# sumitsk/algp

Hardware: AMD Instinct MI355X
Metric: GP-fit+MI-score throughput (N train x M candidates) (higher is better)
Workload: dtype f64

## Files before the change

### algp_amd/csrc/api.hip

```cpp
#include "api_impl.h"

using namespace algp;

namespace algp {

int fail(algp_ctx* c, int code, const std::string& msg) {
    if (c) c->err = msg;
    return code;
}

int ensure(algp_ctx* c, DevBuf& b, size_t bytes) {
    if (bytes <= b.cap && b.p) return ALGP_OK;
    if (bytes == 0) bytes = 256;
    if (b.p) {
        hipStreamSynchronize(c->stream);
        hipFree(b.p);
        c->dev_bytes -= (int64_t)b.cap;
        b.p = nullptr;
        b.cap = 0;
    }
    const size_t want = (bytes + 255) / 256 * 256;
    hipError_t e = hipMalloc(&b.p, want);
    if (e != hipSuccess) {
        b.p = nullptr;
        (void)hipGetLastError();
        return fail(c, ALGP_ERR_OOM, std::string("hipMalloc(") + std::to_string(want) + "): " + hipGetErrorString(e));
    }
    b.cap = want;
    c->dev_bytes += (int64_t)want;
    return ALGP_OK;
}

void release(algp_ctx* c, DevBuf& b) {
    if (b.p) {
        hipFree(b.p);
        c->dev_bytes -= (int64_t)b.cap;
    }
    b.p = nullptr;
    b.cap = 0;
}

static hipEvent_t get_event(algp_ctx* c) {
    if (!c->event_pool.empty()) {
        hipEvent_t e = c->event_pool.back();
        c->event_pool.pop_back();
        return e;
    }
    hipEvent_t e;
    hipEventCreate(&e);
    return e;
}

static thread_local int prof_depth = 0;
void prof_begin(algp_ctx* c, int klass, double flops, double bytes) {
    if (!c->prof_on) return;
    if (prof_depth++ > 0) return;
    PendingEvent pe;
    pe.a = get_event(c);
    pe.b = get_event(c);
    pe.klass = klass;
    c->prof[klass].flops += flops;
    c->prof[klass].bytes += bytes;
    c->prof[klass].launches += 1;
    hipEventRecord(pe.a, c->cur);
    c->pending.push_back(pe);
}
void prof_end(algp_ctx* c) {
    if (!c->prof_on) return;
    if (--prof_depth > 0) return;
    hipEventRecord(c->pending.back().b, c->cur);
}
bool prof_launch_events(algp_ctx* c, int klass, double flops, double bytes, hipEvent_t* a, hipEvent_t* b) {
    if (!c->prof_on || prof_depth > 0) return false;
    PendingEvent pe;
    pe.a = get_event(c);
    pe.b = get_event(c);
    pe.klass = klass;
    c->prof[klass].flops += flops;
    c->prof[klass].bytes += bytes;
    c->prof[klass].launches += 1;
    c->pending.push_back(pe);
    *a = pe.a;
    *b = pe.b;
    return true;
}
static thread_local int span_index = -1;
void prof_span_begin(algp_ctx* c, int klass, double flops, double bytes) {
    if (!c->prof_on) return;
    PendingEvent pe;
    pe.a = get_event(c);
    pe.b = get_event(c);
    pe.klass = klass;
    c->prof[klass].flops += flops;
    c->prof[klass].bytes += bytes;
    c->prof[klass].launches += 1;
    hipEventRecord(pe.a, c->stream);
    span_index = (int)c->pending.size();
    c->pending.push_back(pe);
}
void prof_span_end_on(algp_ctx* c, hipStream_t st) {
    if (!c->prof_on || span_index < 0) return;
    hipEventRecord(c->pending[span_index].b, st);
    span_index = -1;
}
void prof_span_end(algp_ctx* c) { prof_span_end_on(c, c->stream); }
static thread_local int span2_index = -1;
void prof_span_begin2(algp_ctx* c, int klass, double flops, double bytes) {
    if (!c->prof_on) return;
    PendingEvent pe;
    pe.a = get_event(c);
    pe.b = get_event(c);
    pe.klass = klass;
    c->prof[klass].flops += flops;
    c->prof[klass].bytes += bytes;
    c->prof[klass].launches += 1;
    hipEventRecord(pe.a, c->cur);
    span2_index = (int)c->pending.size();
    c->pending.push_back(pe);
}
void prof_span_end2(algp_ctx* c) {
    if (!c->prof_on || span2_index < 0) return;
    hipEventRecord(c->pending[span2_index].b, c->stream);
    span2_index = -1;
}
void prof_collect(algp_ctx* c) {
    for (auto& pe : c->pending) {
        hipEventSynchronize(pe.b);
        float ms = 0;
        hipEventElapsedTime(&ms, pe.a, pe.b);
        c->prof[pe.klass].ms += ms;
        c->event_pool.push_back(pe.a);
        c->event_pool.push_back(pe.b);
    }
    c->pending.clear();
}


hipEvent_t sync_event_api(algp_ctx* c, size_t i) {
    while (c->sync_events.size() <= i) {
        hipEvent_t e;
        hipEventCreateWithFlags(&e, hipEventDisableTiming);
        c->sync_events.push_back(e);
    }
    return c->sync_events[i];
}


KmatSrc make_src(algp_ctx* c) {
    KmatSrc s;
    s.Xs = c->Xs.p;
    s.Cp = c->pool_is_cov ? c->Cp.p : nullptr;
    s.n_pool = c->n_pool;
    s.DP = c->hyp.DP;
    s.kernel = c->hyp.kernel;
    s.outputscale = c->hyp.outputscale;
    s.noise = c->hyp.noise;
    return s;
}

int sync(algp_ctx* c) {
    ALGP_HIP(hipStreamSynchronize(c->stream));
    c->n_syncs++;
    return ALGP_OK;
}

int sync_checked(algp_ctx* c, const char* what) {
    int stall = 0;
    int* d = (int*)((double*)c->scal.p + SC_STALL);
    ALGP_HIP(hipMemcpyAsync(&stall, d, sizeof(int), hipMemcpyDeviceToHost, c->stream));
    ALGP_HIP(hipStreamSynchronize(c->stream));
    c->n_syncs++;
    if (stall != 0) {
        hipMemsetAsync(d, 0, sizeof(double), c->stream);
        return fail(c, ALGP_ERR_HIP, std::string(what) + ": a one-launch kernel stalled (a hand-off between its workgroups never "
                                     "arrived within the spin limit); the result is incomplete");
    }
    return ALGP_OK;
}

}


namespace algp {


template <typename T>
int Impl<T>::rescale_pool(algp_ctx* c) {
    if (c->pool_is_cov || c->n_pool == 0 || !c->hyp.set) return ALGP_OK;
    ALGP_TRY(ensure(c, c->Xs, sizeof(T) * c->n_pool * c->hyp.DP));
    return scale_coords_launch<T>(c, (const T*)c->Xraw.p, c->n_pool, p(c->Xs));
}


template <typename T>
int Impl<T>::kernel_matrix(algp_ctx* c, const void* x1, int64_t n1, const void* x2, int64_t n2, const void* diag_add,
                             int add_lik, void* out) {
    const int D = c->hyp.D, DP = c->hyp.DP;
    const bool sym = (x2 == nullptr);
    if (sym) n2 = n1;
    if (n1 == 0 || n2 == 0) return ALGP_OK;
    const int64_t ldo = round_up(n2, 4);
    DevBuf raw1, raw2, s1, s2, dv, o;
    int rc = ALGP_OK;
    auto cleanup = [&]() { release(c, raw1); release(c, raw2); release(c, s1); release(c, s2); release(c, dv); release(c, o); };
#define KM_TRY(x) do { rc = (x); if (rc != ALGP_OK) { cleanup(); return rc; } } while (0)
#define KM_HIP(x) do { hipError_t e_ = (x); if (e_ != hipSuccess) { cleanup(); return fail(c, ALGP_ERR_HIP, hipGetErrorString(e_)); } } while (0)
    KM_TRY(ensure(c, raw1, sizeof(T) * n1 * D));
    KM_TRY(ensure(c, s1, sizeof(T) * n1 * DP));
    KM_HIP(hipMemcpyAsync(raw1.p, x1, sizeof(T) * n1 * D, hipMemcpyHostToDevice, c->stream));
    KM_TRY(scale_coords_launch<T>(c, (const T*)raw1.p, n1, (T*)s1.p));
    if (!sym) {
        KM_TRY(ensure(c, raw2, sizeof(T) * n2 * D));
        KM_TRY(ensure(c, s2, sizeof(T) * n2 * DP));
        KM_HIP(hipMemcpyAsync(raw2.p, x2, sizeof(T) * n2 * D, hipMemcpyHostToDevice, c->stream));
        KM_TRY(scale_coords_launch<T>(c, (const T*)raw2.p, n2, (T*)s2.p));
    }
    if (sym && diag_add) {
        KM_TRY(ensure(c, dv, sizeof(T) * n1));
        KM_HIP(hipMemcpyAsync(dv.p, diag_add, sizeof(T) * n1, hipMemcpyHostToDevice, c->stream));
    }
    KM_TRY(ensure(c, o, sizeof(T) * n1 * ldo));
    KM_TRY(kmat_xy_launch<T>(c, (const T*)s1.p, n1, sym ? nullptr : (const T*)s2.p, n2, sym ? 1 : 0,
                             (sym && diag_add) ? (const T*)dv.p : nullptr, (sym && add_lik) ? c->hyp.noise : 0.0,
                             (T*)o.p, ldo));
    KM_HIP(hipMemcpy2DAsync(out, sizeof(T) * n2, o.p, sizeof(T) * ldo, sizeof(T) * n2, n1, hipMemcpyDeviceToHost,
                            c->stream));
    KM_HIP(hipStreamSynchronize(c->stream));
    cleanup();
#undef KM_TRY
#undef KM_HIP
    return ALGP_OK;
}


template <typename T>
int Impl<T>::set_pool(algp_ctx* c, const void* x, int64_t n) {
    const int D = c->hyp.D;
    ALGP_TRY(ensure(c, c->Xraw, sizeof(T) * n * D));
    ALGP_HIP(hipMemcpyAsync(c->Xraw.p, x, sizeof(T) * n * D, hipMemcpyHostToDevice, c->stream));
    c->n_pool = n;
    c->pool_is_cov = false;
    c->site_hash.assign((size_t)n, 0);
    const unsigned char* bytes = (const unsigned char*)x;
    const size_t stride = sizeof(T) * (size_t)D;
    for (int64_t i = 0; i < n; ++i) {
        uint64_t h = 1469598103934665603ull;
        for (size_t b = 0; b < stride; ++b) h = (h ^ bytes[(size_t)i * stride + b]) * 1099511628211ull;
        c->site_hash[(size_t)i] = h;
    }
    ALGP_TRY(rescale_pool(c));
    return sync(c);
}

template <typename T>
uint64_t Impl<T>::train_sites_hash(const algp_ctx* c, const std::vector<int64_t>& idx) {
    if (c->pool_is_cov || c->site_hash.empty()) return 0;
    uint64_t h = 1469598103934665603ull;
    for (int64_t i : idx) h = (h ^ c->site_hash[(size_t)i]) * 1099511628211ull;
    return h;
}


template <typename T>
int Impl<T>::set_pool_cov(algp_ctx* c, const void* cov, int64_t n) {
    ALGP_TRY(ensure(c, c->Cp, sizeof(T) * n * n));
    ALGP_HIP(hipMemcpyAsync(c->Cp.p, cov, sizeof(T) * n * n, hipMemcpyHostToDevice, c->stream));
    c->n_pool = n;
    c->pool_is_cov = true;
    c->site_hash.clear();
    return sync(c);
}


template <typename T>
int Impl<T>::set_train(algp_ctx* c, const int64_t* idx, int64_t N, const void* y, const void* var) {
    const int64_t Npad = round_up(std::max<int64_t>(N, 1), NB);
    c->N = N;
    c->Npad = Npad;
    c->train_idx.assign(idx, idx + N);
    c->pos_in_train.assign(c->n_pool, -1);
    c->train_has_repeats = false;
    for (int64_t i = 0; i < N; ++i) {
        if (c->pos_in_train[idx[i]] < 0) c->pos_in_train[idx[i]] = i;
        else c->train_has_repeats = true;
    }
    double ybar = 0;
    const T* yt = (const T*)y;
    for (int64_t i = 0; i < N; ++i) ybar += (double)yt[i];
    ybar = N > 0 ? ybar / (double)N : 0.0;
    if (c->mean_override) ybar = c->mean_value;
    c->ybar = ybar;
    std::vector<T> y0(Npad, (T)0), vv(Npad, (T)0);
    for (int64_t i = 0; i < N; ++i) y0[i] = (T)((double)yt[i] - ybar);
    if (var)
        for (int64_t i = 0; i < N; ++i) vv[i] = ((const T*)var)[i];
    ALGP_TRY(ensure(c, c->Aidx, sizeof(int64_t) * Npad));
    ALGP_TRY(ensure(c, c->y0, sizeof(T) * Npad));
    ALGP_TRY(ensure(c, c->varA, sizeof(T) * Npad));
    if (N > 0) ALGP_HIP(hipMemcpyAsync(c->Aidx.p, idx, sizeof(int64_t) * N, hipMemcpyHostToDevice, c->stream));
    ALGP_HIP(hipMemcpyAsync(c->y0.p, y0.data(), sizeof(T) * Npad, hipMemcpyHostToDevice, c->stream));
    std::vector<T> yr(Npad, (T)0);
    for (int64_t i = 0; i < N; ++i) yr[i] = yt[i];
    ALGP_TRY(ensure(c, c->yraw, sizeof(T) * Npad));
    ALGP_HIP(hipMemcpyAsync(c->yraw.p, yr.data(), sizeof(T) * Npad, hipMemcpyHostToDevice, c->stream));
    c->train_y_host.assign(N, 0.0);
    for (int64_t i = 0; i < N; ++i) c->train_y_host[i] = (double)yt[i];
    ALGP_HIP(hipMemcpyAsync(c->varA.p, vv.data(), sizeof(T) * Npad, hipMemcpyHostToDevice, c->stream));
    ALGP_TRY(sync(c));
    c->train_var_host.assign(N, 0.0);
    if (var)
        for (int64_t i = 0; i < N; ++i) c->train_var_host[i] = (double)((const T*)var)[i];
    c->train_dirty = true;
    c->solved = false;
    if (c->comm || c->host_gather) ALGP_TRY(comm_reserve(c));
    return ALGP_OK;
}


template <typename T>
int Impl<T>::build_set_matrix(algp_ctx* c, const int64_t* idx, int64_t m, const void* var, int64_t* mpad_out, T* dst) {
    const int64_t mpad = round_up(std::max<int64_t>(m, 1), NB);
    *mpad_out = mpad;
    if (!dst) ALGP_TRY(ensure(c, c->auxA, sizeof(T) * mpad * mpad));
    ALGP_TRY(ensure(c, c->auxInv, sizeof(T) * mpad * NB));
    ALGP_TRY(ensure(c, c->auxIdx, sizeof(int64_t) * mpad));
    ALGP_TRY(ensure(c, c->auxVar, sizeof(T) * mpad));
    if (m > 0) ALGP_HIP(hipMemcpyAsync(c->auxIdx.p, idx, sizeof(int64_t) * m, hipMemcpyHostToDevice, c->stream));
    if (var && m > 0)
        ALGP_HIP(hipMemcpyAsync(c->auxVar.p, var, sizeof(T) * m, hipMemcpyHostToDevice, c->stream));
    KmatSrc s = make_src(c);
// ... 35 lines not shown
    double ld = 0;
    ALGP_TRY(factor_resident(c, p(c->auxA), m, mpad, p(c->auxInv), SC_AUXLOGDET, SC_AUXINFO, &ld));
    if (H) *H = (double)m * ENT_CONST + 0.5 * ld;
    return inverse_diag_resident(c, m, mpad, diag_out);
}


template <typename T>
int Impl<T>::upload_padded(algp_ctx* c, DevBuf& b, const void* A, int64_t rows, int64_t cols, int64_t rpad,
                             int64_t cpad) {
    ALGP_TRY(ensure(c, b, sizeof(T) * rpad * cpad));
    ALGP_HIP(hipMemsetAsync(b.p, 0, sizeof(T) * rpad * cpad, c->stream));
    if (rows > 0 && cols > 0)
        ALGP_HIP(hipMemcpy2DAsync(b.p, sizeof(T) * cpad, A, sizeof(T) * cols, sizeof(T) * cols, rows,
                                  hipMemcpyHostToDevice, c->stream));
    return ALGP_OK;
}


template <typename T>
int Impl<T>::entropy_from_cov(algp_ctx* c, const void* cov, int64_t k, double* H, void* L_out, double* logdet) {
    if (k == 0) { if (H) *H = 0.0; if (logdet) *logdet = 0.0; return ALGP_OK; }
    const int64_t kpad = round_up(k, NB);
    ALGP_TRY(upload_padded(c, c->auxA, cov, k, k, kpad, kpad));
    ALGP_TRY(pad_identity_launch<T>(c, p(c->auxA), k, kpad, kpad));
    ALGP_TRY(ensure(c, c->auxInv, sizeof(T) * kpad * NB));
    double ld = 0;
    ALGP_TRY(factor_resident(c, p(c->auxA), k, kpad, p(c->auxInv), SC_AUXLOGDET, SC_AUXINFO, &ld));
    if (H) *H = (double)k * ENT_CONST + 0.5 * ld;
    if (logdet) *logdet = ld;
    if (L_out) {
        ALGP_HIP(hipMemcpy2DAsync(L_out, sizeof(T) * k, c->auxA.p, sizeof(T) * kpad, sizeof(T) * k, k,
                                  hipMemcpyDeviceToHost, c->stream));
        ALGP_TRY(sync(c));
        T* Lh = (T*)L_out;
        for (int64_t i = 0; i < k; ++i)
            for (int64_t j = i + 1; j < k; ++j) Lh[i * k + j] = (T)0;
    }
    return ALGP_OK;
}


template <typename T>
int Impl<T>::gemm_host(algp_ctx* c, int64_t m, int64_t n, int64_t k, double alpha, const void* A, const void* B,
                         double beta, const void* C, void* D) {
    const int64_t mp = round_up(std::max<int64_t>(m, 1), NB), np = round_up(std::max<int64_t>(n, 1), NB),
                  kp = round_up(std::max<int64_t>(k, 1), NB);
    DevBuf a, b, cc;
    int rc = upload_padded(c, a, A, m, k, mp, kp);
    if (rc == ALGP_OK) rc = upload_padded(c, b, B, n, k, np, kp);
    if (rc == ALGP_OK) rc = upload_padded(c, cc, (beta != 0.0 && C) ? C : nullptr, (beta != 0.0 && C) ? m : 0, n, mp, np);
    if (rc == ALGP_OK)
        rc = gemm_nt_launch<T>(c, ALGP_PROF_GEMM_OTHER, mp, np, kp, (T)alpha, (const T*)a.p, kp, (const T*)b.p, kp,
                               (T)beta, (const T*)cc.p, np, (T*)cc.p, np, 0);
    if (rc == ALGP_OK) {
        hipError_t e = hipMemcpy2DAsync(D, sizeof(T) * n, cc.p, sizeof(T) * np, sizeof(T) * n, m,
                                        hipMemcpyDeviceToHost, c->stream);
        if (e != hipSuccess) rc = fail(c, ALGP_ERR_HIP, hipGetErrorString(e));
    }
    hipStreamSynchronize(c->stream);
    release(c, a); release(c, b); release(c, cc);
    return rc;
}


template <typename T>
int Impl<T>::trsm_host(algp_ctx* c, const void* L, int64_t n, const void* B, int64_t m, void* X) {
    const int64_t np = round_up(std::max<int64_t>(n, 1), NB), mp = round_up(std::max<int64_t>(m, 1), NB);
    DevBuf l, b, inv;
    int rc = upload_padded(c, l, L, n, n, np, np);
    if (rc == ALGP_OK) rc = pad_identity_launch<T>(c, (T*)l.p, n, np, np);
    if (rc == ALGP_OK) rc = upload_padded(c, b, B, m, n, mp, np);
    if (rc == ALGP_OK) rc = ensure(c, inv, sizeof(T) * np * NB);
    for (int64_t kb = 0; rc == ALGP_OK && kb < np / NB; ++kb)
        rc = trinv_diag_launch<T>(c, (const T*)l.p + kb * NB * np + kb * NB, np, (T*)inv.p + kb * NB * NB);
    if (rc == ALGP_OK) rc = trsm_blocked<T>(c, ALGP_PROF_GEMM_OTHER, (T*)b.p, mp, np, (const T*)l.p, np, np, (const T*)inv.p);
    if (rc == ALGP_OK) {
        hipError_t e = hipMemcpy2DAsync(X, sizeof(T) * n, b.p, sizeof(T) * np, sizeof(T) * n, m,
                                        hipMemcpyDeviceToHost, c->stream);
        if (e != hipSuccess) rc = fail(c, ALGP_ERR_HIP, hipGetErrorString(e));
    }
    hipStreamSynchronize(c->stream);
    release(c, l); release(c, b); release(c, inv);
    return rc;
}

template <typename T>
int Impl<T>::selftest(algp_ctx* c, int* mism) {
    double* sc = (double*)c->scal.p;
    int* d = (int*)(sc + SC_PROBE);
    ALGP_HIP(hipMemsetAsync(d, 0, sizeof(double), c->stream));
    ALGP_TRY(test_mfma_launch<double>(c, d));
    ALGP_TRY(test_mfma_launch<float>(c, d));
    ALGP_HIP(hipMemcpyAsync(mism, d, sizeof(int), hipMemcpyDeviceToHost, c->stream));
    return sync(c);
}

template struct Impl<float>;
template struct Impl<double>;

}

extern "C" {

int algp_version(void) { return 100; }

int algp_device_count(void) {
    int n = 0;
    if (hipGetDeviceCount(&n) != hipSuccess) { (void)hipGetLastError(); return 0; }
    return n;
}

int algp_create(int device_id, int dtype, algp_ctx** out) {
    if (!out || (dtype != ALGP_F32 && dtype != ALGP_F64)) return ALGP_ERR_BAD_ARG;
    *out = nullptr;
    setenv("GPU_MAX_HW_QUEUES", "8", 0);
    int n = 0;
    if (hipGetDeviceCount(&n) != hipSuccess || n <= 0) { (void)hipGetLastError(); return ALGP_ERR_NO_DEVICE; }
    if (device_id < 0 || device_id >= n) return ALGP_ERR_BAD_ARG;
    if (hipSetDevice(device_id) != hipSuccess) return ALGP_ERR_HIP;
    algp_ctx* c = new algp_ctx();
    c->device = device_id;
    c->dtype = dtype;
    c->es = dtype == ALGP_F64 ? 8 : 4;
    if (hipStreamCreateWithFlags(&c->stream, hipStreamNonBlocking) != hipSuccess) { delete c; return ALGP_ERR_HIP; }
    if (hipStreamCreateWithFlags(&c->stream2, hipStreamNonBlocking) != hipSuccess) { hipStreamDestroy(c->stream); delete c; return ALGP_ERR_HIP; }
    if (hipStreamCreateWithFlags(&c->stream3, hipStreamNonBlocking) != hipSuccess) c->stream3 = nullptr;
    if (hipStreamCreateWithFlags(&c->stream4, hipStreamNonBlocking) != hipSuccess) c->stream4 = nullptr;
    c->trsm_chunks = env_int("ALGP_TRSM_CHUNKS", c->trsm_chunks);
    c->trsm_chunks_explicit = env_int("ALGP_TRSM_CHUNKS", 0) != 0;
    if (hipDeviceGetAttribute(&c->cu_count, hipDeviceAttributeMultiprocessorCount, device_id) != hipSuccess) { (void)hipGetLastError(); c->cu_count = 0; }
    c->cur = c->stream;
    if (ensure(c, c->scal, sizeof(double) * SC_COUNT) != ALGP_OK) { hipStreamDestroy(c->stream); delete c; return ALGP_ERR_OOM; }
    hipMemsetAsync(c->scal.p, 0, sizeof(double) * SC_COUNT, c->stream);
    hipStreamSynchronize(c->stream);
    *out = c;
    return ALGP_OK;
}

void algp_destroy(algp_ctx* c) {
    if (!c) return;
    hipSetDevice(c->device);
    hipStreamSynchronize(c->stream);
    prof_collect(c);
    DevBuf* bufs[] = {&c->Xs, &c->Xraw, &c->Cp, &c->Aidx, &c->yA, &c->varA, &c->y0, &c->L, &c->invD, &c->z, &c->alpha,
                      &c->scal, &c->Cidx, &c->ckind, &c->cextra, &c->Vt, &c->dstat, &c->mu, &c->alive, &c->scores,
                      &c->lrow, &c->remote, &c->commbuf, &c->tvec, &c->amax, &c->prevrows, &c->fresh, &c->lazypicks, &c->yraw, &c->uvec, &c->wvec, &c->acc3, &c->rowstat, &c->inv512, &c->inv512_scr, &c->trsm_tmp, &c->gemm_part, &c->rhs_rx, &c->rhs_cx, &c->rhs_rk, &c->splitk, &c->dag_state, &c->dag_stats, &c->trsv_ctrl, &c->auxA, &c->auxInv, &c->auxW, &c->auxIdx,
                      &c->auxVar, &c->auxD, &c->hostStage, &c->rowx, &c->tailE, &c->tailPart, &c->ldpart, &c->tw, &c->smp, &c->grp};
    for (DevBuf* b : bufs) release(c, *b);
    release(c, c->mi);
    release(c, c->vr);
    dag_release(c);
    comm_destroy(c);
    for (hipEvent_t e : c->event_pool) hipEventDestroy(e);
    for (hipEvent_t e : c->sync_events) hipEventDestroy(e);
    hipStreamSynchronize(c->stream2);
    hipStreamDestroy(c->stream2);
    if (c->stream3) { hipStreamSynchronize(c->stream3); hipStreamDestroy(c->stream3); }
    if (c->stream4) { hipStreamSynchronize(c->stream4); hipStreamDestroy(c->stream4); }
    hipStreamDestroy(c->stream);
    delete c;
}

const char* algp_last_error(const algp_ctx* c) { return c ? c->err.c_str() : "null context"; }

int64_t algp_last_pivot(const algp_ctx* c) { return c ? c->pivot : 0; }

double algp_last_jitter(const algp_ctx* c) { return c ? c->last_jitter : 0.0; }

int algp_dtype(const algp_ctx* c) { return c ? c->dtype : -1; }

int algp_set_hypers(algp_ctx* c, int kernel, int D, const double* log_ls, double log_os, double log_noise) {
    CHECK_CTX(c);
    if (D < 1 || D > MAXD || !log_ls) return fail(c, ALGP_ERR_BAD_ARG, "set_hypers: 1 <= D <= 8 required");
    if (kernel < ALGP_KERNEL_RBF || kernel > ALGP_KERNEL_MATERN25) return fail(c, ALGP_ERR_BAD_ARG, "set_hypers: unknown kernel");
    if (c->hyp.set && c->hyp.D != D && c->n_pool > 0 && !c->pool_is_cov) {
        c->n_pool = 0;
        c->N = 0;
        c->pos_in_train.clear();
    }
    c->hyp.kernel = kernel;
    c->hyp.D = D;
    c->hyp.DP = D <= 2 ? 2 : (D <= 4 ? 4 : 8);
    for (int d = 0; d < MAXD; ++d) c->hyp.inv_ls[d] = d < D ? exp(-log_ls[d]) : 0.0;
    c->hyp.outputscale = exp(log_os);
    c->hyp.noise = exp(log_noise);
    c->hyp.set = true;
    c->hyp_stamp++;
    c->factored = false;
    c->solved = false;
    FINISH(c, DISPATCH(c, rescale_pool(c)));
}

int algp_kernel_matrix(algp_ctx* c, const void* x1, int64_t n1, const void* x2, int64_t n2, const void* diag_add,
                       int add_lik, void* out) {
    CHECK_CTX(c);
    NEED_HYPERS(c);
    if (!x1 || n1 < 0 || n2 < 0 || !out) return fail(c, ALGP_ERR_BAD_ARG, "kernel_matrix: bad arguments");
    FINISH(c, DISPATCH(c, kernel_matrix(c, x1, n1, x2, n2, diag_add, add_lik, out)));
}

int algp_set_pool(algp_ctx* c, const void* x, int64_t n) {
    CHECK_CTX(c);
    NEED_HYPERS(c);
    if (!x || n <= 0) return fail(c, ALGP_ERR_BAD_ARG, "set_pool: bad arguments");
    c->factored = c->solved = false;
    c->hyp_stamp++;
    c->pos_in_train.clear();
    c->N = 0;
    c->site_owner.clear();
    c->site_owner_hash = 0;
    c->has_tw = false;
    c->vr.drop();
    FINISH(c, DISPATCH(c, set_pool(c, x, n)));
}

int algp_set_pool_cov(algp_ctx* c, const void* cov, int64_t n) {
    CHECK_CTX(c);
    NEED_HYPERS(c);
    if (!cov || n <= 0) return fail(c, ALGP_ERR_BAD_ARG, "set_pool_cov: bad arguments");
    c->factored = c->solved = false;
    c->hyp_stamp++;
    c->pos_in_train.clear();
    c->N = 0;
    c->site_owner.clear();
    c->site_owner_hash = 0;
    c->has_tw = false;
    c->vr.drop();
    FINISH(c, DISPATCH(c, set_pool_cov(c, cov, n)));
}

int algp_set_train(algp_ctx* c, const int64_t* idx, int64_t N, const void* y, const void* var) {
    CHECK_CTX(c);
    if (c->n_pool <= 0) return fail(c, ALGP_ERR_STATE, "set_train: set a pool first");
    if (N < 0 || (N > 0 && (!idx || !y))) return fail(c, ALGP_ERR_BAD_ARG, "set_train: bad arguments");
    for (int64_t i = 0; i < N; ++i)
        if (idx[i] < 0 || idx[i] >= c->n_pool) return fail(c, ALGP_ERR_BAD_ARG, "set_train: index outside the pool");
    FINISH(c, DISPATCH(c, set_train(c, idx, N, y, var)));
}

int algp_set_constant_mean(algp_ctx* c, int enable, double value) {
    CHECK_CTX(c);
    if (enable && !(value == value)) return fail(c, ALGP_ERR_BAD_ARG, "set_constant_mean: NaN");
    c->mean_override = enable != 0;
    c->mean_value = value;
    return ALGP_OK;
}

#if ALGP_TEST_HOOKS
int64_t algp_debug_counter(algp_ctx* c, int which) {
    if (!c) return -1;
    switch (which) {
        case 0: return c->n_syncs;
        case 1: return c->factor_rows_from_vt;
        case 2: return c->rows_from_peers;
        case 3: return c->row_exchanges;
        case 4: return c->row_fallbacks;
        default: return -1;
    }
}
#endif

#if ALGP_TEST_HOOKS
int algp_debug_set_trsm_chunks(algp_ctx* c, int chunks) {
    CHECK_CTX(c);
    if (chunks < 0 || chunks > 4) return fail(c, ALGP_ERR_BAD_ARG, "debug_set_trsm_chunks: 0 (default) .. 4");
    hipStreamSynchronize(c->stream);
    c->trsm_chunks_explicit = chunks != 0 || env_int("ALGP_TRSM_CHUNKS", 0) != 0;
    if (chunks == 0) chunks = env_int("ALGP_TRSM_CHUNKS", 3);
    c->trsm_chunks = chunks;
    return ALGP_OK;
}
#endif

#if ALGP_TEST_HOOKS
int algp_debug_trsv_stall(algp_ctx* c, int block) {
    CHECK_CTX(c);
    if (block < -1) return fail(c, ALGP_ERR_BAD_ARG, "debug_trsv_stall: a block >= 0, or -1 to disarm");
    c->debug_trsv_stall_block = block;
    return ALGP_OK;
}
#endif

#if ALGP_TEST_HOOKS
int algp_debug_dag_stall(algp_ctx* c, int ticket) {
    CHECK_CTX(c);
    if (ticket < -1) return fail(c, ALGP_ERR_BAD_ARG, "debug_dag_stall: a ticket >= 0, or -1 to disarm");
    c->debug_dag_stall_ticket = ticket;
    return ALGP_OK;
}
#endif

int algp_entropy_from_cov(algp_ctx* c, const void* cov, int64_t k, double* H) {
    CHECK_CTX(c);
    if (k < 0 || !H || (k > 0 && !cov)) return fail(c, ALGP_ERR_BAD_ARG, "entropy_from_cov: bad arguments");
    FINISH(c, DISPATCH(c, entropy_from_cov(c, cov, k, H, nullptr, nullptr)));
}

int algp_set_entropy(algp_ctx* c, const int64_t* idx, int64_t m, const void* var, double* H) {
    CHECK_CTX(c);
    NEED_HYPERS(c);
    if (m < 0 || !H || (m > 0 && !idx)) return fail(c, ALGP_ERR_BAD_ARG, "set_entropy: bad arguments");
    for (int64_t i = 0; i < m; ++i)
        if (idx[i] < 0 || idx[i] >= c->n_pool) return fail(c, ALGP_ERR_BAD_ARG, "set_entropy: index outside the pool");
    FINISH(c, DISPATCH(c, set_entropy(c, idx, m, var, H)));
}
// ... 108 lines not shown
```

### algp_amd/csrc/api_candidates.hip

```cpp
#include "api_impl.h"

using namespace algp;

namespace algp {


template <typename T>
int Impl<T>::set_candidates(algp_ctx* c, const int64_t* idx, int64_t M, int prior_noise, const void* extra) {
    if (c->pool_is_cov && !prior_noise)
        return fail(c, ALGP_ERR_BAD_ARG, "an explicit pool covariance carries sigma_n^2 on its diagonal: prior_includes_noise must be 1");
    const int64_t Mpad = round_up(std::max<int64_t>(M, 1), NB);
    c->M = M;
    c->Mpad = Mpad;
    c->prior_noise = prior_noise;
    c->cand_idx.assign(idx, idx + M);
    c->cand_pos.assign(c->n_pool, -1);
    for (int64_t j = 0; j < M; ++j) c->cand_pos[idx[j]] = j;
    ALGP_TRY(ensure(c, c->Cidx, sizeof(int64_t) * Mpad));
    if (M > 0) ALGP_HIP(hipMemcpyAsync(c->Cidx.p, idx, sizeof(int64_t) * M, hipMemcpyHostToDevice, c->stream));
    if (extra) {
        ALGP_TRY(ensure(c, c->cextra, sizeof(T) * Mpad));
        ALGP_HIP(hipMemcpyAsync(c->cextra.p, extra, sizeof(T) * M, hipMemcpyHostToDevice, c->stream));
    } else {
        release(c, c->cextra);
    }
    ALGP_TRY(sync(c));
    c->solved = false;
    return ALGP_OK;
}

template <typename T>
void Impl<T>::plan_route(algp_ctx* c, int incremental, bool allow_fold, typename Impl<T>::SolvePlan& pl) {
    const bool tail_on = env_switch("ALGP_TAIL_COLS", true), solve_dag_on = env_switch("ALGP_SOLVE_DAG", true),
               stats_on = env_switch("ALGP_ROW_STATS", true), fold_on = allow_fold && env_switch("ALGP_FOLD", true);
    const int64_t N = c->N, Npad = c->Npad, M = c->M, Mpad = c->Mpad;
    pl.carried_sums = incremental && c->uw_rows == N && c->uvec.p && c->wvec.p;
    int64_t keep = 0;
    if (incremental && c->Vt.p && c->vt_hyp_stamp == c->hyp_stamp && c->vt_prior_noise == c->prior_noise &&
        !c->vt_has_extra && !c->cextra.p && c->vt_cand_idx == c->cand_idx) {
        const int64_t lim = std::min<int64_t>((int64_t)c->vt_fact_idx.size(), N);
        int64_t p0 = 0;
        while (p0 < lim && c->vt_fact_idx[p0] == c->fact_idx[p0] && c->vt_fact_var[p0] == c->fact_var[p0]) ++p0;
        keep = p0 / NB * NB;
        if (tail_on && p0 >= 2048 && Mpad >= 2048 && c->cur == c->stream) {
            const bool exact = N > p0 && N - p0 <= 64;
            const int64_t k16 = exact ? p0 : p0 / 16 * 16, c1 = exact ? N : round_up(N, 16);
            int n = 0;
            bool ok = c1 > k16;
            if (exact) {
                pl.seg_c0[0] = p0;
                pl.seg_w[0] = (int)(N - p0);
                pl.seg_window = true;
                n = 1;
            }
            if (ok && !exact && c1 - k16 <= 64 && k16 / NB != (c1 - 1) / NB && k16 + NB <= Npad) {
                pl.seg_c0[0] = k16;
                pl.seg_w[0] = (int)(c1 - k16);
                pl.seg_window = true;
                n = 1;
            }
            for (int64_t a = k16; a < c1 && ok && !pl.seg_window;) {
                const int64_t b = std::min<int64_t>(c1, (a / NB + 1) * NB);
                if (b - a > 64 || n == 2) { ok = false; break; }
                pl.seg_c0[n] = a;
                pl.seg_w[n] = (int)(b - a);
                ++n;
                a = b;
            }
            if (ok && n > 0) {
                pl.nseg = n;
                keep = k16;
            }
        }
    }
    std::vector<int>& kind = pl.kind;
    kind.assign(Mpad, -1);
    if (c->prior_noise)
        for (int64_t j = 0; j < M; ++j) kind[j] = (int)c->pos_in_train[c->cand_idx[j]];
    std::vector<int64_t>& became_unit = pl.became_unit;
    became_unit.clear();
    if (keep > 0) {
        for (int64_t j = 0; j < M && keep > 0; ++j) {
            const int was = c->vt_kind[j], now = kind[j];
            if (was == now) continue;
            if (was < 0 && now >= keep) became_unit.push_back(j);
            else if (!(was >= keep && now >= keep)) keep = 0;
        }
        if (keep == 0) became_unit.clear();
    }
    if (keep == 0) { pl.nseg = 0; pl.seg_window = false; }
    pl.keep = keep;
    if (pl.nseg > 0) { pl.route = SolveRoute::Segments; return; }
    if (fold_on && M > 0 && panel_fits(Npad, Mpad)) pl.route = SolveRoute::Folded;
    else if (solve_dag_on && keep == 0 && Mpad / NB > 32 && panel_fits(Npad, Mpad) && c->cur == c->stream) pl.route = SolveRoute::TaskList;
    else pl.route = SolveRoute::Sweep;
    const int64_t r = N % NB, N1 = Npad - NB;
    const bool narrow = r > 0 && r <= 64 && N1 >= 2048 && Mpad >= 2048 && tail_on &&
                        (pl.route != SolveRoute::Sweep || (keep == 0 && c->cur == c->stream && Mpad / NB > SWEEP_PUSH_TILES));
    if (narrow) {
        pl.narrow_r = (int)r;
        pl.short_rows = pl.route == SolveRoute::Sweep ? Mpad : M < Mpad ? Mpad - NB : Mpad;
    }
    pl.row_stats = pl.route == SolveRoute::Sweep && stats_on && keep == 0 && !pl.carried_sums;
    pl.sweep_end = pl.narrow_r ? Npad - NB : Npad;
    pl.rhs_fused = pl.route == SolveRoute::Sweep && keep == 0 && M > 0 && env_switch("ALGP_RHS_FUSED", true) &&
                   trsm_sched_wanted(c, Mpad, pl.sweep_end, keep) && rhs_gen_supported(c->hyp.DP, c->pool_is_cov);
}

template <typename T>
int Impl<T>::rhs_window(algp_ctx* c, int64_t c0, int64_t w, void* out, int64_t ldo) {
    const int64_t live = std::max<int64_t>(0, std::min<int64_t>(c->N - c0, w));
    KmatSrc s = make_src(c);
    return kmat_launch<T>(c, s, (const int64_t*)c->Cidx.p, c->M, c->Mpad, (const int64_t*)c->Aidx.p + c0, live, w, nullptr, 0,
                          c->prior_noise ? (const int*)c->ckind.p : nullptr, 0, (T*)out, ldo, 0, c0);
}

template <typename T>
int Impl<T>::solve_prepare(algp_ctx* c, int incremental, typename Impl<T>::SolvePlan& pl) {
    const int64_t N = c->N, Npad = c->Npad, M = c->M, Mpad = c->Mpad, keep = pl.keep;
    const int64_t ldv = Npad + MAX_APPEND;
    c->solved = false;
    c->vr.drop();
    if (!c->Vt.p || c->ldv_cap < ldv || (keep == 0 && !incremental && c->ldv_cap != ldv) ||
        c->Vt.cap < sizeof(T) * Mpad * c->ldv_cap) {
        const int64_t newcap = incremental ? round_up(ldv + ldv / 8, NB) : ldv;
        DevBuf nv;
        ALGP_TRY(ensure(c, nv, sizeof(T) * Mpad * newcap));
        if (keep > 0) {
            hipError_t e = hipMemcpy2DAsync(nv.p, sizeof(T) * newcap, c->Vt.p, sizeof(T) * c->ldv_cap, sizeof(T) * keep,
                                            Mpad, hipMemcpyDeviceToDevice, c->stream);
            if (e != hipSuccess) { release(c, nv); return fail(c, ALGP_ERR_HIP, hipGetErrorString(e)); }
            hipStreamSynchronize(c->stream);
        }
        release(c, c->Vt);
        c->Vt = nv;
        c->ldv_cap = newcap;
    }
    const int64_t ldc = c->ldv_cap;
    c->ldv = ldc;
    ALGP_TRY(ensure(c, c->dstat, sizeof(T) * Mpad));
    ALGP_TRY(ensure(c, c->mu, sizeof(T) * Mpad));
    ALGP_TRY(ensure(c, c->tvec, sizeof(T) * 2 * Mpad));
    ALGP_TRY(ensure(c, c->alive, Mpad));
    ALGP_TRY(ensure(c, c->scores, sizeof(double) * Mpad));
    ALGP_TRY(ensure(c, c->lrow, sizeof(T) * ldc));
    ALGP_TRY(ensure(c, c->prevrows, sizeof(T) * MAX_APPEND * ldc));
    {
        ALGP_TRY(ensure(c, c->ckind, sizeof(int) * Mpad));
        ALGP_HIP(hipMemcpyAsync(c->ckind.p, pl.kind.data(), sizeof(int) * Mpad, hipMemcpyHostToDevice, c->stream));
        if (!pl.became_unit.empty() && keep > 0) {
            const size_t nb = pl.became_unit.size();
            ALGP_TRY(ensure(c, c->auxIdx, sizeof(int64_t) * nb));
            ALGP_HIP(hipMemcpyAsync(c->auxIdx.p, pl.became_unit.data(), sizeof(int64_t) * nb, hipMemcpyHostToDevice, c->stream));
            ALGP_TRY(zero_listed_rows_launch<T>(c, p(c->Vt), ldc, (const int64_t*)c->auxIdx.p, (int64_t)nb, keep));
        }
        ALGP_TRY(sync(c));
    }
    KmatSrc s = make_src(c);
    if (pl.rhs_fused) {
        const int DP = c->hyp.DP;
        ALGP_TRY(ensure(c, c->rhs_rx, sizeof(T) * (size_t)Mpad * DP));
        ALGP_TRY(ensure(c, c->rhs_cx, sizeof(T) * (size_t)Npad * DP));
        ALGP_TRY(ensure(c, c->rhs_rk, sizeof(int) * (size_t)Mpad));
        ALGP_TRY(rhs_gather_launch<T>(c, (const T*)c->Xs.p, DP, (const int64_t*)c->Cidx.p, M, Mpad,
                                      c->prior_noise ? (const int*)c->ckind.p : nullptr, (const int64_t*)c->Aidx.p, N, Npad,
                                      p(c->rhs_rx), p(c->rhs_cx), (int*)c->rhs_rk.p));
        pl.gen.rx = c->rhs_rx.p;
        pl.gen.cx = c->rhs_cx.p;
        pl.gen.rk = (const int*)c->rhs_rk.p;
        pl.gen.ncols = N;
        pl.gen.DP = DP;
        pl.gen.kernel = s.kernel;
        pl.gen.outputscale = s.outputscale;
        pl.gen.window = &Impl<T>::rhs_window;
        return rhs_window(c, pl.sweep_end, ldv - pl.sweep_end, p(c->Vt) + pl.sweep_end, ldc);
    }
    return kmat_launch<T>(c, s, (const int64_t*)c->Cidx.p, M, Mpad, (const int64_t*)c->Aidx.p + keep, N - keep,
                          ldv - keep, nullptr, 0, c->prior_noise ? (const int*)c->ckind.p : nullptr, 0,
                          p(c->Vt) + keep, ldc, 0, keep);
}


template <typename T>
int Impl<T>::solve_run(algp_ctx* c, typename Impl<T>::SolvePlan& pl) {
    const int64_t Npad = c->Npad, Mpad = c->Mpad, ldc = c->ldv, keep = pl.keep;
    prof_span_begin(c, ALGP_PROF_TRSM, (double)(Npad - keep) * (double)(Npad + keep) * (double)Mpad,
                    sizeof(T) * (double)Mpad * (double)Npad);
    int trc = ALGP_OK;
    if (pl.route == SolveRoute::Segments && pl.seg_window) {
        const int64_t w0 = std::min<int64_t>(pl.seg_c0[0], Npad - NB), o = pl.seg_c0[0] - w0;
        trc = ensure(c, c->tailE, sizeof(T) * NB * NB);
        if (trc == ALGP_OK) trc = trinv_diag_launch<T>(c, p(c->L) + w0 * c->Lld + w0, c->Lld, p(c->tailE));
        if (trc == ALGP_OK)
            trc = tail_cols_launch<T>(c, ALGP_PROF_TAIL_COLS, p(c->Vt), Mpad, ldc, p(c->L), c->Lld, Npad, (const T*)nullptr,
                                      pl.seg_c0[0], pl.seg_w[0], p(c->tailE) + o * NB + o);
    } else if (pl.route == SolveRoute::Segments) {
        for (int q = 0; q < pl.nseg && trc == ALGP_OK; ++q)
            trc = tail_cols_launch<T>(c, ALGP_PROF_TAIL_COLS, p(c->Vt), Mpad, ldc, p(c->L), c->Lld, Npad,
                                      p(c->invD) + (pl.seg_c0[q] / NB) * NB * NB, pl.seg_c0[q], pl.seg_w[q]);
    } else if (pl.route == SolveRoute::TaskList) {
        trc = solve_dag_panel<T>(c, p(c->L), Npad, c->Lld, p(c->invD), (int*)((double*)c->scal.p + SC_STALL), p(c->Vt), ldc, Mpad, 1,
                                 (int)(pl.short_rows / NB));
    } else if (pl.route == SolveRoute::Sweep) {
        T* stat = nullptr;
        if (pl.row_stats && ensure(c, c->rowstat, sizeof(T) * 2 * (size_t)(Npad / NB) * (size_t)Mpad) == ALGP_OK)
            stat = p(c->rowstat);
        trc = trsm_blocked<T>(c, ALGP_PROF_GEMM_TRSM, p(c->Vt), Mpad, ldc, p(c->L), pl.sweep_end, c->Lld, p(c->invD),
                              keep, p(c->z), stat, Mpad, &pl.rowstat_done, pl.rhs_fused ? &pl.gen : nullptr);
    } else {
        trc = fail(c, ALGP_ERR_STATE, "internal: the folded route is solved by the factorisation's launch (fit_and_solve)");
    }
    if (trc == ALGP_OK) trc = solve_narrow_tile(c, pl);
    prof_span_end(c);
    return trc;
}


template <typename T>
int Impl<T>::solve_narrow_tile(algp_ctx* c, const typename Impl<T>::SolvePlan& pl) {
    if (pl.narrow_r == 0) return ALGP_OK;
    const int64_t Mpad = c->Mpad, ldc = c->ldv, N1 = c->Npad - NB;
    ALGP_TRY(tail_cols_launch<T>(c, ALGP_PROF_TAIL_COLS, p(c->Vt), pl.short_rows, ldc, p(c->L), c->Lld, c->Npad,
                                 p(c->invD) + (N1 / NB) * NB * NB, N1, (int)round_up(pl.narrow_r, 16)));
    if (!pl.rowstat_done) return ALGP_OK;
    T* stat = p(c->rowstat);
    return rows_reduce_launch<T>(c, p(c->Vt) + N1, Mpad, ldc, NB, p(c->z) + N1, stat + 2 * (N1 / NB) * Mpad,
                                 stat + (2 * (N1 / NB) + 1) * Mpad);
}


template <typename T>
int Impl<T>::solve_finish(algp_ctx* c, int incremental, const unsigned char* alive_host, const typename Impl<T>::SolvePlan& pl) {
    const int64_t N = c->N, Npad = c->Npad, M = c->M, Mpad = c->Mpad, ldc = c->ldv, keep = pl.keep;
    T* ss = p(c->tvec);
    T* dot = ss + Mpad;
    if (pl.carried_sums) {
        const size_t need = sizeof(T) * 6 * (size_t)Mpad;
        bool ok = keep > 0 && c->acc3.p && c->acc3.cap >= need && c->acc_M == M && c->acc_cols > 0 &&
                  c->acc_cols <= keep && c->acc_cols <= c->uw_stable;
        if (!ok) {
            ALGP_TRY(ensure(c, c->acc3, need));
            ALGP_HIP(hipMemsetAsync(c->acc3.p, 0, sizeof(T) * 3 * (size_t)Mpad, c->stream));
            c->acc_cols = 0;
        }
        T* acc = p(c->acc3);
        T* tmp = acc + 3 * Mpad;
        if (!pl.became_unit.empty()) {
            const size_t nb = pl.became_unit.size();
            ALGP_TRY(ensure(c, c->auxIdx, sizeof(int64_t) * nb));
            ALGP_HIP(hipMemcpyAsync(c->auxIdx.p, pl.became_unit.data(), sizeof(int64_t) * nb, hipMemcpyHostToDevice, c->stream));
            ALGP_TRY(zero_rows3_launch<T>(c, acc, Mpad, (const int64_t*)c->auxIdx.p, (int64_t)nb));
        }
        const int64_t fin = N / NB * NB;
        if (fin > c->acc_cols)
            ALGP_TRY(rows_reduce3_launch<T>(c, p(c->Vt), M, ldc, c->acc_cols, fin, p(c->uvec), p(c->wvec), acc, Mpad, 1));
        ALGP_TRY(rows_reduce3_launch<T>(c, p(c->Vt), M, ldc, fin, Npad, p(c->uvec), p(c->wvec), tmp, Mpad, 0));
        ALGP_TRY(combine3_launch<T>(c, M, acc, tmp, Mpad, (T)c->ybar, ss, dot));
        c->acc_cols = fin;
        c->acc_M = M;
        c->uw_stable = N;
    } else {
        c->acc_cols = 0;
        if (pl.rowstat_done) ALGP_TRY(rowstat_combine_launch<T>(c, p(c->rowstat), Mpad, (int)(Npad / NB), M, ss, dot));
        else ALGP_TRY(rows_reduce_launch<T>(c, p(c->Vt), M, ldc, Npad, p(c->z), ss, dot));
    }
    const T prior = (T)(c->hyp.outputscale + (c->prior_noise ? c->hyp.noise : 0.0));
    ALGP_TRY(cand_finalize_launch<T>(c, M, (const int*)c->ckind.p, (const int64_t*)c->Cidx.p,
                                     c->pool_is_cov ? (const T*)c->Cp.p : nullptr, c->n_pool, prior,
                                     c->cextra.p ? (const T*)c->cextra.p : nullptr, ss, dot, (T)c->ybar, p(c->dstat),
                                     p(c->mu), (unsigned char*)c->alive.p));
    if (alive_host) ALGP_HIP(hipMemcpyAsync(c->alive.p, alive_host, M, hipMemcpyHostToDevice, c->stream));
    ALGP_TRY(sync_checked(c, "solve_candidates"));
    c->ncols = Npad;
    c->picks.clear();
    c->mi.valid = false;
    c->vr.drop();
    ALGP_TRY(reset_lazy(c));
    c->solved = true;
    c->vt_fact_idx = c->fact_idx;
    c->vt_fact_var = c->fact_var;
    c->vt_cand_idx = c->cand_idx;
    c->vt_kind.assign(pl.kind.begin(), pl.kind.begin() + M);
    c->vt_hyp_stamp = c->hyp_stamp;
    c->vt_prior_noise = c->prior_noise;
    c->vt_has_extra = c->cextra.p != nullptr;
    c->kept_cols_last = keep;
    return ALGP_OK;
}


template <typename T>
int Impl<T>::solve_candidates(algp_ctx* c, int incremental, const unsigned char* alive_host) {
    if (!c->factored || c->train_dirty) return fail(c, ALGP_ERR_STATE, "solve_candidates: call algp_factorize first");
    SolvePlan pl;
    plan_route(c, incremental, false, pl);
    ALGP_TRY(solve_prepare(c, incremental, pl));
    ALGP_TRY(solve_run(c, pl));
    return solve_finish(c, incremental, alive_host, pl);
}


template <typename T>
int Impl<T>::fit_and_solve(algp_ctx* c) {
    SolvePlan pl;
    plan_route(c, 0, true, pl);
    if (pl.route != SolveRoute::Folded) {
        ALGP_TRY(factorize(c, 0));
        ALGP_TRY(solve_prepare(c, 0, pl));
        ALGP_TRY(solve_run(c, pl));
        return solve_finish(c, 0, nullptr, pl);
    }
    c->factored = false;
    ALGP_TRY(solve_prepare(c, 0, pl));
    Panel pn{p(c->Vt), c->ldv, c->Mpad, 1};
    if (c->M < c->Mpad) {
        pn.z_row = c->M;
        ALGP_HIP(hipMemcpyAsync(p(c->Vt) + c->M * c->ldv, c->y0.p, sizeof(T) * c->Npad, hipMemcpyDeviceToDevice, c->stream));
    }
    pn.short_rows = pl.short_rows;
    ALGP_TRY(factorize(c, 0, &pn));
    ALGP_TRY(solve_narrow_tile(c, pl));
    return solve_finish(c, 0, nullptr, pl);
}


template <typename T>
int Impl<T>::get_posterior(algp_ctx* c, void* mu, void* var) {
    if (!c->solved) return fail(c, ALGP_ERR_STATE, "get_posterior: call algp_solve_candidates first");
    ALGP_TRY(flush_lazy(c));
    if (mu) ALGP_HIP(hipMemcpyAsync(mu, c->mu.p, sizeof(T) * c->M, hipMemcpyDeviceToHost, c->stream));
    if (var) ALGP_HIP(hipMemcpyAsync(var, c->dstat.p, sizeof(T) * c->M, hipMemcpyDeviceToHost, c->stream));
    return sync(c);
}


template <typename T>
int Impl<T>::get_posterior_cov(algp_ctx* c, void* cov_out, double* mi_out) {
    if (!c->solved) return fail(c, ALGP_ERR_STATE, "get_posterior_cov: call algp_solve_candidates first");
    if (c->pool_is_cov) return fail(c, ALGP_ERR_BAD_ARG, "get_posterior_cov needs a coordinate pool");
    const int64_t M = c->M, Mpad = c->Mpad;
    if (c->prior_noise)
        for (int64_t j = 0; j < M; ++j)
            if (c->vt_kind[j] >= 0)
                return fail(c, ALGP_ERR_STATE,
                            "get_posterior_cov: candidate " + std::to_string(j) + " (pool index " + std::to_string(c->cand_idx[j]) +
                                ") is a train site and was solved as a unit row (prior_includes_noise = 1): set the "
                                "candidates with prior_includes_noise = 0");
    if (!c->picks.empty())
        return fail(c, ALGP_ERR_STATE, "get_posterior_cov: " + std::to_string(c->picks.size()) +
                                           " pick(s) were committed since the candidate solve, which the covariance would "
                                           "not include: solve the candidates again");
    c->last_jitter = 0.0;
    if (M == 0) {
        if (mi_out) *mi_out = 0.0;
        return ALGP_OK;
    }
    ALGP_TRY(ensure(c, c->auxA, sizeof(T) * Mpad * Mpad));
    ALGP_TRY(ensure(c, c->auxW, sizeof(T) * Mpad * Mpad));
    ALGP_TRY(ensure(c, c->auxInv, sizeof(T) * Mpad * NB));
    KmatSrc s = make_src(c);
    const T* extra = c->cextra.p ? (const T*)c->cextra.p : nullptr;
    c->last_jitter = 0.0;
    const double eps = sizeof(T) == 8 ? 2.220446049250313e-16 : 1.1920928955078125e-07;
    for (int attempt = 0;; ++attempt) {
        const double jitter = attempt == 0 ? 0.0 : 64.0 * eps * c->hyp.outputscale * pow(100.0, attempt - 1);
        ALGP_TRY(kmat_launch<T>(c, s, (const int64_t*)c->Cidx.p, M, Mpad, (const int64_t*)c->Cidx.p, M, Mpad, extra, 0,
                                nullptr, 1, p(c->auxA), Mpad));
        ALGP_TRY(gemm_nt_launch<T>(c, ALGP_PROF_GEMM_OTHER, Mpad, Mpad, c->Npad, (T)-1, p(c->Vt), c->ldv, p(c->Vt),
                                   c->ldv, (T)1, p(c->auxA), Mpad, p(c->auxW), Mpad, 0));
        if (attempt == 0 && cov_out)
            ALGP_HIP(hipMemcpy2DAsync(cov_out, sizeof(T) * M, c->auxW.p, sizeof(T) * Mpad, sizeof(T) * M, M,
                                      hipMemcpyDeviceToHost, c->stream));
        ALGP_TRY(sync(c));
        if (!mi_out) break;
        if (jitter > 0.0) {
            ALGP_TRY(add_diag_launch<T>(c, p(c->auxA), M, Mpad, (T)jitter));
            ALGP_TRY(add_diag_launch<T>(c, p(c->auxW), M, Mpad, (T)jitter));
        }
        double ld_xx = 0, ld_cov = 0;
        int rc = factor_resident(c, p(c->auxA), M, Mpad, p(c->auxInv), SC_AUXLOGDET, SC_AUXINFO, &ld_xx);
        if (rc == ALGP_OK) rc = factor_resident(c, p(c->auxW), M, Mpad, p(c->auxInv), SC_AUXLOGDET, SC_AUXINFO, &ld_cov);
        if (rc == ALGP_OK) {
            *mi_out = 0.5 * (ld_xx - ld_cov);
            c->last_jitter = jitter;
            break;
        }
        if (rc != ALGP_ERR_NOT_PD || attempt >= 5) return rc;
        c->err.clear();
    }
    return ALGP_OK;
}


template <typename T>
int Impl<T>::posterior_mean(algp_ctx* c, const int64_t* idx, int64_t M, void* mu_out) {
    if (!c->factored || c->train_dirty) return fail(c, ALGP_ERR_STATE, "posterior_mean: call algp_factorize first");
    if (c->pool_is_cov) return fail(c, ALGP_ERR_BAD_ARG, "posterior_mean needs a coordinate pool");
    if (M == 0) return ALGP_OK;
    ALGP_TRY(ensure(c, c->auxIdx, sizeof(int64_t) * M));
    ALGP_TRY(ensure(c, c->auxD, sizeof(T) * M));
    ALGP_HIP(hipMemcpyAsync(c->auxIdx.p, idx, sizeof(int64_t) * M, hipMemcpyHostToDevice, c->stream));
    ALGP_TRY(need_alpha(c));
    ALGP_TRY(kgemv_launch<T>(c, M, (const int64_t*)c->auxIdx.p, make_src(c), c->N, (const int64_t*)c->Aidx.p,
                             (const T*)c->alpha.p, (T)c->ybar, p(c->auxD)));
    ALGP_HIP(hipMemcpyAsync(mu_out, c->auxD.p, sizeof(T) * M, hipMemcpyDeviceToHost, c->stream));
    const int rc = sync_checked(c, "posterior_mean");
    if (rc != ALGP_OK) c->alpha_valid = false;
    return rc;
}

template struct Impl<float>;
template struct Impl<double>;

}

extern "C" {

int algp_set_candidates(algp_ctx* c, const int64_t* idx, int64_t M, int prior_noise, const void* extra) {
    CHECK_CTX(c);
    if (c->n_pool <= 0) return fail(c, ALGP_ERR_STATE, "set_candidates: set a pool first");
    if (M < 0 || (M > 0 && !idx)) return fail(c, ALGP_ERR_BAD_ARG, "set_candidates: bad arguments");
    for (int64_t i = 0; i < M; ++i)
        if (idx[i] < 0 || idx[i] >= c->n_pool) return fail(c, ALGP_ERR_BAD_ARG, "set_candidates: index outside the pool");
    FINISH(c, DISPATCH(c, set_candidates(c, idx, M, prior_noise, extra)));
}

int algp_fit_and_solve(algp_ctx* c) {
    CHECK_CTX(c);
    NEED_HYPERS(c);
    if (c->n_pool <= 0) return fail(c, ALGP_ERR_STATE, "fit_and_solve: set a pool first");
    if (!c->y0.p || (int64_t)c->pos_in_train.size() != c->n_pool)
        return fail(c, ALGP_ERR_STATE, "fit_and_solve: call algp_set_train first");
    if ((int64_t)c->cand_pos.size() != c->n_pool) return fail(c, ALGP_ERR_STATE, "fit_and_solve: call algp_set_candidates first");
    FINISH(c, DISPATCH(c, fit_and_solve(c)));
}

int algp_solve_candidates(algp_ctx* c) { CHECK_CTX(c); FINISH(c, DISPATCH(c, solve_candidates(c, 0, nullptr))); }

int algp_solve_candidates_update(algp_ctx* c, const uint8_t* alive, int64_t* kept_cols) {
    CHECK_CTX(c);
    int rc = DISPATCH(c, solve_candidates(c, 1, alive));
    if (kept_cols) *kept_cols = rc == ALGP_OK ? c->kept_cols_last : 0;
    if (c->prof_on) prof_collect(c);
    return rc;
}

int algp_set_candidate_alive(algp_ctx* c, const uint8_t* alive) {
    CHECK_CTX(c);
    if (!c->solved || !alive) return fail(c, ALGP_ERR_STATE, "set_candidate_alive: solve the candidates first");
    if (hipMemcpyAsync(c->alive.p, alive, c->M, hipMemcpyHostToDevice, c->stream) != hipSuccess)
        return fail(c, ALGP_ERR_HIP, "set_candidate_alive: copy failed");
    c->bounds_valid = false;
    return sync(c);
}

int algp_get_posterior(algp_ctx* c, void* mu, void* var) { CHECK_CTX(c); FINISH(c, DISPATCH(c, get_posterior(c, mu, var))); }

int algp_get_posterior_cov(algp_ctx* c, void* cov, double* mi) { CHECK_CTX(c); FINISH(c, DISPATCH(c, get_posterior_cov(c, cov, mi))); }
// ... 11 lines not shown
```

### algp_amd/csrc/api_factor.hip

```cpp
#include "api_impl.h"

using namespace algp;

namespace algp {

template <typename T>
bool Impl<T>::panel_fits(int64_t npad, int64_t mpad) {
    const int64_t nt = npad / NB, mt = mpad / NB;
    return dag_enabled() && nt >= DAG_MIN_TILES && nt <= DAG_MAX_TILES && mt >= 1 && mt <= DAG_MAX_PANEL_TILES;
}


template <typename T>
int Impl<T>::factor_resident(algp_ctx* c, T* A, int64_t n, int64_t npad, T* invD, int slot_logdet, int slot_info,
                               double* logdet, int64_t ld, int64_t pivot_offset, typename Impl<T>::Panel* panel) {
    if (panel && !panel_fits(npad, panel->mpad))
        return fail(c, ALGP_ERR_STATE, "internal: factor_resident was given a panel that does not fit the task list");
    if (ld == 0) ld = npad;
    double* sc = (double*)c->scal.p;
    ALGP_HIP(hipMemsetAsync(sc + slot_logdet, 0, 2 * sizeof(double), c->stream));
    if (panel) {
        ALGP_TRY(cholesky_dag_panel<T>(c, A, npad, ld, invD, sc + slot_logdet, (int*)(sc + slot_info), panel->P, panel->ldp,
                                       panel->mpad, panel->mode, (int)(panel->short_rows / NB)));
        if (panel->mode == 2 && panel->inv_out && c->stream2 && c->cur == c->stream) {
            hipEvent_t ready = sync_event_api(c, 20), done = sync_event_api(c, 21);
            ALGP_HIP(hipEventRecord(ready, c->stream));
            ALGP_HIP(hipStreamWaitEvent(c->stream2, ready, 0));
            c->cur = c->stream2;
            const int rc = syrk_upper<T>(c, ALGP_PROF_GEMM_OTHER, panel->P, npad, panel->ldp, panel->inv_out, npad);
            c->cur = c->stream;
            ALGP_HIP(hipEventRecord(done, c->stream2));
            ALGP_TRY(rc);
            panel->inv_enqueued = true;
        }
    } else {
        ALGP_TRY(cholesky_blocked<T>(c, A, npad, ld, invD, sc + slot_logdet, (int*)(sc + slot_info)));
    }
    double host[2];
    ALGP_HIP(hipMemcpyAsync(host, sc + slot_logdet, 2 * sizeof(double), hipMemcpyDeviceToHost, c->stream));
    ALGP_TRY(sync(c));
    int info;
    memcpy(&info, &host[1], sizeof(int));
    if (info == INT_MIN)
        return fail(c, ALGP_ERR_HIP, "cholesky: the dependency-driven launch stalled (a task's inputs never arrived)");
    if (info != 0) {
        info += (int)pivot_offset;
        c->pivot = info;
        return fail(c, ALGP_ERR_NOT_PD,
                    "matrix is not positive definite: non-positive pivot at index " + std::to_string(info) +
                        " (1-based) of " + std::to_string(n));
    }
    *logdet = host[0];
    return ALGP_OK;
}


template <typename T>
int Impl<T>::reserve_factor(algp_ctx* c, int64_t npad_need, int64_t keep_rows, int64_t keep_height,
                              bool headroom) {
    if (c->Lld >= npad_need && c->L.p && c->invD.p) return ALGP_OK;
    const int64_t first = headroom ? npad_need + npad_need / 8 : npad_need;
    const int64_t newld = round_up(std::max<int64_t>(first, c->Lld + c->Lld / 4), NB);
    DevBuf nl, ni;
    int rc = ensure(c, nl, sizeof(T) * newld * newld);
    if (rc == ALGP_OK) rc = ensure(c, ni, sizeof(T) * newld * NB);
    if (rc != ALGP_OK) { release(c, nl); release(c, ni); return rc; }
    if (keep_rows > 0 && c->L.p) {
        hipError_t e = hipMemcpy2DAsync(nl.p, sizeof(T) * newld, c->L.p, sizeof(T) * c->Lld, sizeof(T) * keep_rows,
                                        std::max(keep_rows, keep_height), hipMemcpyDeviceToDevice, c->stream);
        if (e == hipSuccess)
            e = hipMemcpyAsync(ni.p, c->invD.p, sizeof(T) * keep_rows * NB, hipMemcpyDeviceToDevice, c->stream);
        if (e != hipSuccess) { release(c, nl); release(c, ni); return fail(c, ALGP_ERR_HIP, hipGetErrorString(e)); }
        hipStreamSynchronize(c->stream);
    }
    release(c, c->L);
    release(c, c->invD);
    c->L = nl;
    c->invD = ni;
    c->Lld = newld;
    return ALGP_OK;
}


template <typename T>
bool Impl<T>::vt_rows_for_new_sites(algp_ctx* c, int64_t Nb, int64_t p0, std::vector<int64_t>& src_row,
                                      std::vector<int64_t>& lrow, std::vector<T>& lscale, bool& any_second) {
    static const bool on = env_switch("ALGP_FACTOR_FROM_VT", true);
    const int64_t N = c->N, Npad = c->Npad;
    if (!on || !c->Vt.p || c->vt_hyp_stamp != c->hyp_stamp || (int64_t)c->vt_fact_idx.size() < Nb || Nb <= 0) return false;
    if (c->vt_cand_idx != c->cand_idx || (int64_t)c->vt_kind.size() != c->M) return false;
    for (int64_t r = 0; r < Nb; ++r)
        if (c->vt_fact_idx[r] != c->train_idx[r] || c->vt_fact_var[r] != c->train_var_host[r]) return false;
    src_row.assign((size_t)(Npad - p0), -1);
    lrow.assign((size_t)(Npad - p0), -1);
    lscale.assign((size_t)(Npad - p0), (T)0);
    any_second = false;
    for (int64_t i = p0; i < N; ++i) {
        const int64_t q = c->train_idx[i], j = c->cand_pos[q];
        if (j < 0) return false;
        const int k = c->vt_kind[j];
        if (k >= 0) {
            if (k >= p0 || c->train_idx[k] != q || (int64_t)c->vt_fact_idx.size() <= k || c->vt_fact_idx[k] != q ||
                c->vt_fact_var[k] != c->train_var_host[k])
                return false;
            lrow[(size_t)(i - p0)] = k;
            lscale[(size_t)(i - p0)] = (T)c->train_var_host[k];
            any_second = true;
        }
        src_row[(size_t)(i - p0)] = j;
    }
    return true;
}


template <typename T>
int Impl<T>::exchange_new_rows(algp_ctx* c, int64_t Nb, int64_t p0, int* placed, int st_in) {
    const int64_t N = c->N, Npad = c->Npad, ld = c->Lld;
    const int nr = c->comm_nranks, me = c->comm_rank;
    const int64_t nnew = N - p0, ntot = Npad - p0;
    *placed = 0;
    std::vector<int> owner((size_t)std::max<int64_t>(nnew, 0)), slot((size_t)std::max<int64_t>(nnew, 0));
    std::vector<int64_t> cnt((size_t)nr, 0);
    int st = st_in;
    uint64_t h = 1469598103934665603ull;
    auto mix = [&h](uint64_t v) { h = (h ^ v) * 1099511628211ull; };
    mix((uint64_t)Nb);
    mix(c->site_owner_hash);
    for (int64_t i = 0; i < nnew; ++i) {
        const int64_t q = c->train_idx[(size_t)(p0 + i)];
        const int o = c->site_owner[(size_t)q];
        mix((uint64_t)q);
        mix((uint64_t)(int64_t)o);
        if (o < 0 || o >= nr) { st = 1; owner[(size_t)i] = -1; continue; }
        owner[(size_t)i] = o;
        slot[(size_t)i] = (int)cnt[(size_t)o]++;
    }
    int64_t cap = 0;
    for (int r = 0; r < nr; ++r) cap = std::max(cap, cnt[(size_t)r]);
    std::vector<int64_t> src_row((size_t)std::max<int64_t>(cap, 1), -1), lrow((size_t)std::max<int64_t>(cap, 1), -1);
    std::vector<T> lscale((size_t)std::max<int64_t>(cap, 1), (T)0);
    bool second = false;
    if (st == 0 && Nb > 0 && cnt[(size_t)me] > 0) {
        bool ok = c->Vt.p && c->vt_hyp_stamp == c->hyp_stamp && (int64_t)c->vt_fact_idx.size() >= Nb &&
                  c->vt_cand_idx == c->cand_idx && (int64_t)c->vt_kind.size() == c->M;
        for (int64_t r = 0; ok && r < Nb; ++r)
            ok = c->vt_fact_idx[(size_t)r] == c->train_idx[(size_t)r] && c->vt_fact_var[(size_t)r] == c->train_var_host[(size_t)r];
        for (int64_t i = 0; ok && i < nnew; ++i) {
            if (owner[(size_t)i] != me) continue;
            const int64_t q = c->train_idx[(size_t)(p0 + i)], j = c->cand_pos[(size_t)q];
            if (j < 0) { ok = false; break; }
            const int k = c->vt_kind[(size_t)j];
            if (k >= 0) {
                if (k >= p0 || c->train_idx[(size_t)k] != q || (int64_t)c->vt_fact_idx.size() <= k ||
                    c->vt_fact_idx[(size_t)k] != q || c->vt_fact_var[(size_t)k] != c->train_var_host[(size_t)k]) { ok = false; break; }
                lrow[(size_t)slot[(size_t)i]] = k;
                lscale[(size_t)slot[(size_t)i]] = (T)c->train_var_host[(size_t)k];
                second = true;
            }
            src_row[(size_t)slot[(size_t)i]] = j;
        }
        if (!ok) st = 1;
    }
    const size_t rowbytes = sizeof(T) * (size_t)Nb;
    if (st <= 1 && cap > 0 && Nb > 0) {
        const int rc = comm_rows_reserve(c, sizeof(T) * (size_t)c->Lld * (size_t)std::max<int64_t>(16, round_up(cap, 8)));
        if (rc != ALGP_OK) st = rc;
    }
    if (st <= 1 && Nb > 0) {
        int rc = ensure(c, c->auxIdx, sizeof(int64_t) * 2 * (size_t)std::max<int64_t>(std::max(ntot, cap), 1));
        if (rc == ALGP_OK) rc = ensure(c, c->auxVar, sizeof(T) * (size_t)std::max<int64_t>(cap, 1) + 256);
        if (rc != ALGP_OK) st = rc;
    }
    if (c->debug_fail_next_rowx) {
        st = c->debug_fail_next_rowx;
        c->debug_fail_next_rowx = 0;
        c->err = "factorize_update: failure injected by algp_debug_fail_at";
    }
    const std::string local_err = c->err;
    double mine[4] = {(double)st, (double)p0, (double)N, 0.0};
    memcpy(&mine[3], &h, sizeof(h));
    std::vector<double> all;
    ALGP_TRY(comm_agree(c, mine, all));
    int worst = 0, bad_rank = -1;
    bool same = true;
    for (int r = 0; r < nr; ++r) {
        const double* t = &all[(size_t)r * 4];
        const int s_r = (t[0] == t[0] && t[0] >= 0 && t[0] <= 64) ? (int)t[0] : ALGP_ERR_HIP;
        if (s_r > worst) { worst = s_r; bad_rank = r; }
        if (t[1] != mine[1] || t[2] != mine[2] || memcmp(&t[3], &mine[3], 8) != 0) same = false;
    }
    if (worst >= 2) {
        if (st >= 2) return fail(c, st, local_err);
        return fail(c, worst, "factorize_update: rank " + std::to_string(bad_rank) + " failed with error " + std::to_string(worst) +
                                  " before the row exchange; no rank updated its factor");
    }
    if (worst == 1 || !same) {
        bool any_kept = false;
        for (int r = 0; r < nr; ++r) any_kept = any_kept || all[(size_t)r * 4 + 1] >= (double)NB;
        if (any_kept) c->row_fallbacks += 1;
        return ALGP_OK;
    }
    if (cap > 0) {
        T* own = (T*)c->rowx.p;
        const size_t bytes = rowbytes * (size_t)cap;
        T* gathered = (T*)((char*)c->rowx.p + bytes);
        int64_t* d_src = (int64_t*)c->auxIdx.p;
        int64_t* d_lrow = d_src + std::max<int64_t>(std::max(ntot, cap), 1);
        ALGP_HIP(hipMemcpyAsync(d_src, src_row.data(), sizeof(int64_t) * (size_t)cap, hipMemcpyHostToDevice, c->stream));
        if (second) {
            ALGP_HIP(hipMemcpyAsync(d_lrow, lrow.data(), sizeof(int64_t) * (size_t)cap, hipMemcpyHostToDevice, c->stream));
            ALGP_HIP(hipMemcpyAsync(c->auxVar.p, lscale.data(), sizeof(T) * (size_t)cap, hipMemcpyHostToDevice, c->stream));
        }
        ALGP_TRY(gather_rows_launch<T>(c, p(c->Vt), c->ldv, d_src, own, Nb, cap, Nb, second ? d_lrow : nullptr,
                                       second ? (const T*)c->auxVar.p : nullptr, p(c->L), ld));
        ALGP_TRY(sync(c));
        std::vector<size_t> used((size_t)nr);
        for (int r = 0; r < nr; ++r) used[(size_t)r] = rowbytes * (size_t)cnt[(size_t)r];
        ALGP_TRY(comm_rows_gather(c, bytes, used.data()));
        std::vector<int64_t> from((size_t)ntot, -1);
        int64_t peers = 0;
        for (int64_t i = 0; i < nnew; ++i) {
            from[(size_t)i] = (int64_t)owner[(size_t)i] * cap + slot[(size_t)i];
            peers += owner[(size_t)i] != me;
        }
        ALGP_HIP(hipMemcpyAsync(d_src, from.data(), sizeof(int64_t) * (size_t)ntot, hipMemcpyHostToDevice, c->stream));
        ALGP_TRY(gather_rows_launch<T>(c, gathered, Nb, d_src, p(c->L) + p0 * ld, ld, ntot, Nb));
        ALGP_TRY(sync(c));
        c->rows_from_peers = peers;
        c->row_exchanges += 1;
    } else if (ntot > 0) {
        ALGP_HIP(hipMemset2DAsync(p(c->L) + p0 * ld, sizeof(T) * (size_t)ld, 0, rowbytes, (size_t)ntot, c->stream));
        c->rows_from_peers = 0;
    }
    *placed = 1;
    return ALGP_OK;
}


template <typename T>
int Impl<T>::factorize(algp_ctx* c, int incremental, typename Impl<T>::Panel* panel) {
    if (panel && incremental) return fail(c, ALGP_ERR_STATE, "internal: a panel rides along with a from-scratch factorisation only");
    const int64_t N = c->N, Npad = c->Npad;
    int64_t keep = 0, p0 = 0;
    if (incremental && c->factored && c->fact_hyp_stamp == c->hyp_stamp && c->Lld > 0) {
        const int64_t lim = std::min<int64_t>(N, c->Nfact);
        while (p0 < lim && c->fact_idx[p0] == c->train_idx[p0] && c->fact_var[p0] == c->train_var_host[p0]) ++p0;
        keep = p0 / NB * NB;
    }
    c->factored = false;
    c->solved = false;
    const bool sharded = incremental && (c->comm || c->host_gather) && c->comm_nranks > 1 && !c->site_owner.empty() &&
                         (int64_t)c->site_owner.size() == c->n_pool;
    int pre = reserve_factor(c, Npad, keep, p0, incremental != 0);
    if (pre == ALGP_OK) pre = ensure(c, c->z, sizeof(T) * Npad);
    if (pre == ALGP_OK) pre = ensure(c, c->alpha, sizeof(T) * Npad);
    if (sharded && (pre != ALGP_OK || keep == 0)) {
        int placed_unused = 0;
        const int arc = exchange_new_rows(c, 0, p0, &placed_unused, pre != ALGP_OK ? pre : 1);
        if (arc != ALGP_OK) return arc;
    }
    ALGP_TRY(pre);
    const int64_t ld = c->Lld;
    KmatSrc s = make_src(c);
    double ld_total = 0;
    prof_span_begin(c, ALGP_PROF_CHOLESKY, keep == 0 ? (double)N * N * N / 3.0 : (double)(N - keep) * N * N,
                    sizeof(T) * (double)N * N);
    int frc = ALGP_OK;
    if (keep == 0) {
        frc = kmat_launch<T>(c, s, (const int64_t*)c->Aidx.p, N, Npad, (const int64_t*)c->Aidx.p, N, Npad,
                             (const T*)c->varA.p, c->pool_is_cov ? 0 : 1, nullptr, 1, p(c->L), ld);
        if (frc == ALGP_OK)
            frc = factor_resident(c, p(c->L), N, Npad, p(c->invD), SC_LOGDET, SC_INFO, &ld_total, ld, 0, panel);
    } else {
        const int64_t Nb = keep, R = Npad - Nb;
        T* rows = p(c->L) + Nb * ld;
        std::vector<int64_t> src_row, lrow;
        std::vector<T> lscale;
        bool second = false;
        int placed = 0;
        c->rows_from_peers = 0;
        if (sharded) {
            frc = exchange_new_rows(c, Nb, p0, &placed);
            if (frc != ALGP_OK) { prof_span_end(c); return frc; }
        }
        if (placed) {
            frc = kmat_launch<T>(c, s, (const int64_t*)c->Aidx.p + Nb, N - Nb, R, (const int64_t*)c->Aidx.p + Nb, N - Nb, R,
                                 (const T*)c->varA.p + Nb, c->pool_is_cov ? 0 : 1, nullptr, 1, rows + Nb, ld);
            c->factor_rows_from_vt = Npad - p0;
        } else if (!sharded && vt_rows_for_new_sites(c, Nb, p0, src_row, lrow, lscale, second)) {
            frc = kmat_launch<T>(c, s, (const int64_t*)c->Aidx.p + Nb, N - Nb, R, (const int64_t*)c->Aidx.p + Nb, N - Nb, R,
                                 (const T*)c->varA.p + Nb, c->pool_is_cov ? 0 : 1, nullptr, 1, rows + Nb, ld);
            const size_t nr = src_row.size();
            if (frc == ALGP_OK) frc = ensure(c, c->auxIdx, sizeof(int64_t) * 2 * std::max<size_t>(nr, 1));
            if (frc == ALGP_OK) frc = ensure(c, c->auxVar, sizeof(T) * std::max<size_t>(nr, 1) + 256);
            if (frc == ALGP_OK && nr > 0) {
                int64_t* d_src = (int64_t*)c->auxIdx.p;
                int64_t* d_lrow = d_src + nr;
                hipMemcpyAsync(d_src, src_row.data(), sizeof(int64_t) * nr, hipMemcpyHostToDevice, c->stream);
                if (second) {
                    hipMemcpyAsync(d_lrow, lrow.data(), sizeof(int64_t) * nr, hipMemcpyHostToDevice, c->stream);
                    hipMemcpyAsync(c->auxVar.p, lscale.data(), sizeof(T) * nr, hipMemcpyHostToDevice, c->stream);
                }
                frc = gather_rows_launch<T>(c, p(c->Vt), c->ldv, d_src, p(c->L) + p0 * ld, ld, (int64_t)nr, Nb,
                                            second ? d_lrow : nullptr, second ? (const T*)c->auxVar.p : nullptr,
                                            p(c->L), ld);
                if (frc == ALGP_OK) frc = sync(c);
            }
            c->factor_rows_from_vt = (int64_t)src_row.size();
        } else {
            c->factor_rows_from_vt = 0;
            frc = kmat_launch<T>(c, s, (const int64_t*)c->Aidx.p + Nb, N - Nb, R, (const int64_t*)c->Aidx.p, N, Npad,
                                 (const T*)c->varA.p + Nb, c->pool_is_cov ? 0 : 1, nullptr, 1, rows, ld, Nb);
            if (frc == ALGP_OK)
                frc = trsm_blocked<T>(c, ALGP_PROF_GEMM_CHOL, rows, R, ld, p(c->L), Nb, ld, p(c->invD));
        }
        if (frc == ALGP_OK)
            frc = syrk_skinny_sub<T>(c, ALGP_PROF_GEMM_CHOL, rows, R, Nb, ld, rows + Nb, ld, c->auxW);
        double ld_tail = 0;
        if (frc == ALGP_OK)
            frc = factor_resident(c, rows + Nb, N - Nb, R, p(c->invD) + Nb * NB, SC_LOGDET, SC_INFO, &ld_tail, ld, Nb);
        if (frc == ALGP_OK) {
            double* sc = (double*)c->scal.p;
            hipMemsetAsync(sc + SC_AUXLOGDET, 0, sizeof(double), c->stream);
            frc = logdiag_launch<T>(c, p(c->L), ld, N, sc + SC_AUXLOGDET);
            if (frc == ALGP_OK) {
                hipMemcpyAsync(&ld_total, sc + SC_AUXLOGDET, sizeof(double), hipMemcpyDeviceToHost, c->stream);
                frc = sync(c);
                ld_total *= 2.0;
            }
        }
    }
    prof_span_end(c);
    ALGP_TRY(frc);
    T* z_src = (panel && panel->z_row >= 0) ? panel->P + panel->z_row * panel->ldp : nullptr;
    return finish_factor(c, keep, p0, ld_total, z_src);
}


template <typename T>
int Impl<T>::finish_factor(algp_ctx* c, int64_t keep, int64_t p0, double ld_total, T* z_src) {
    const int64_t N = c->N, Npad = c->Npad, ld = c->Lld;
    c->logdet = ld_total;
    if (keep > 0) {
        int64_t pu = 0;
        const int64_t lim = std::min<int64_t>(std::min<int64_t>(p0, c->uw_rows), (int64_t)c->fact_y.size());
        while (pu < lim && c->fact_y[pu] == c->train_y_host[pu]) ++pu;
        int64_t ku = std::min<int64_t>(keep, pu / NB * NB);
        const size_t need = sizeof(T) * (size_t)ld;
        if (!c->uvec.p || c->uvec.cap < need || !c->wvec.p || c->wvec.cap < need) {
            ALGP_TRY(ensure(c, c->uvec, need));
            ALGP_TRY(ensure(c, c->wvec, need));
            ku = 0;
        }
        T* u = p(c->uvec);
        T* w = p(c->wvec);
        ALGP_TRY(uw_init_launch<T>(c, u, w, (const T*)c->yraw.p, ku, N, Npad));
        ALGP_TRY(tail_gemv2_launch<T>(c, p(c->L), ld, ku, Npad, u, w));
        ALGP_TRY(trsv_forward2<T>(c, p(c->L), Npad, ld, p(c->invD), u, w, ku / NB));
        ALGP_TRY(uw_combine_launch<T>(c, p(c->z), u, w, (T)c->ybar, Npad));
        c->uw_rows = N;
        c->uw_stable = std::min(c->uw_stable, ku);
        c->fact_y = c->train_y_host;
    } else if (z_src) {
        ALGP_HIP(hipMemcpyAsync(c->z.p, z_src, sizeof(T) * Npad, hipMemcpyDeviceToDevice, c->stream));
        ALGP_HIP(hipMemsetAsync(z_src, 0, sizeof(T) * Npad, c->stream));
        c->uw_rows = 0;
        c->uw_stable = 0;
    } else {
        ALGP_HIP(hipMemcpyAsync(c->z.p, c->y0.p, sizeof(T) * Npad, hipMemcpyDeviceToDevice, c->stream));
        ALGP_TRY(trsv_forward<T>(c, p(c->L), Npad, ld, p(c->invD), p(c->z)));
        c->uw_rows = 0;
        c->uw_stable = 0;
    }
    c->alpha_valid = false;
    std::vector<T> zh(Npad);
    ALGP_HIP(hipMemcpyAsync(zh.data(), c->z.p, sizeof(T) * Npad, hipMemcpyDeviceToHost, c->stream));
    ALGP_TRY(sync_checked(c, "factorize: forward substitution"));
    double q = 0;
    for (int64_t i = 0; i < N; ++i) q += (double)zh[i] * (double)zh[i];
    c->yalpha = q;
    c->factored = true;
    c->train_dirty = false;
    c->Nfact = N;
    c->fact_idx = c->train_idx;
    c->fact_var = c->train_var_host;
    c->fact_hyp_stamp = c->hyp_stamp;
    c->kept_rows_last = keep;
    return ALGP_OK;
}


template <typename T>
int Impl<T>::factorize_from(algp_ctx* c, algp_ctx* src) {
    const int64_t N = c->N, Npad = c->Npad;
    if (src == c) return fail(c, ALGP_ERR_BAD_ARG, "factorize_from: source and destination are the same context");
    if (src->dtype != c->dtype || src->device != c->device)
        return fail(c, ALGP_ERR_BAD_ARG, "factorize_from: contexts differ in dtype or device");
    if (!src->factored || src->train_dirty) return fail(c, ALGP_ERR_STATE, "factorize_from: the source holds no factor");
    const Hypers &a = c->hyp, &b = src->hyp;
    bool same = a.D == b.D && a.kernel == b.kernel && a.outputscale == b.outputscale && a.noise == b.noise;
    for (int d = 0; same && d < a.D; ++d) same = a.inv_ls[d] == b.inv_ls[d];
    if (!same) return fail(c, ALGP_ERR_STATE, "factorize_from: hyper-parameters differ");
    if (src->N != N || src->fact_idx != c->train_idx || src->fact_var != c->train_var_host)
        return fail(c, ALGP_ERR_STATE, "factorize_from: the source factor belongs to a different train set");
    if (c->pool_is_cov || src->pool_is_cov)
        return fail(c, ALGP_ERR_STATE, "factorize_from: needs coordinate pools on both sides (an explicit covariance cannot be compared)");
    if (train_sites_hash(src, src->fact_idx) != train_sites_hash(c, c->train_idx))
        return fail(c, ALGP_ERR_STATE, "factorize_from: the two pools hold different coordinates at the train indices");
    int64_t keep = 0, p0 = 0;
    if (c->factored && c->fact_hyp_stamp == c->hyp_stamp && c->Lld > 0) {
        const int64_t lim = std::min<int64_t>(N, c->Nfact);
        while (p0 < lim && c->fact_idx[p0] == c->train_idx[p0] && c->fact_var[p0] == c->train_var_host[p0]) ++p0;
        keep = p0 / NB * NB;
    }
    c->factored = false;
    c->solved = false;
    ALGP_TRY(reserve_factor(c, Npad, keep, 0));
    ALGP_TRY(ensure(c, c->z, sizeof(T) * Npad));
    ALGP_TRY(ensure(c, c->alpha, sizeof(T) * Npad));
    hipStreamSynchronize(src->stream);
    if (Npad > keep) {
        ALGP_HIP(hipMemcpy2DAsync(p(c->L) + keep * c->Lld, sizeof(T) * c->Lld, (const T*)src->L.p + keep * src->Lld,
                                  sizeof(T) * src->Lld, sizeof(T) * Npad, Npad - keep, hipMemcpyDeviceToDevice, c->stream));
        ALGP_HIP(hipMemcpyAsync(p(c->invD) + keep * NB, (const T*)src->invD.p + keep * NB, sizeof(T) * (Npad - keep) * NB,
                                hipMemcpyDeviceToDevice, c->stream));
    }
    return finish_factor(c, keep, p0, src->logdet);
}


template <typename T>
int Impl<T>::need_alpha(algp_ctx* c) {
    if (c->alpha_valid) return ALGP_OK;
    ALGP_HIP(hipMemcpyAsync(c->alpha.p, c->z.p, sizeof(T) * c->Npad, hipMemcpyDeviceToDevice, c->stream));
    ALGP_TRY(trsv_backward<T>(c, p(c->L), c->Npad, c->Lld, p(c->invD), p(c->alpha)));
    c->alpha_valid = true;
    return ALGP_OK;
}


template <typename T>
int Impl<T>::get_alpha(algp_ctx* c, void* out) {
    if (!c->factored || c->train_dirty) return fail(c, ALGP_ERR_STATE, "get_alpha: call algp_factorize first");
    ALGP_TRY(need_alpha(c));
    ALGP_HIP(hipMemcpyAsync(out, c->alpha.p, sizeof(T) * c->N, hipMemcpyDeviceToHost, c->stream));
    const int rc = sync_checked(c, "get_alpha");
    if (rc != ALGP_OK) c->alpha_valid = false;
    return rc;
}

template <typename T>
int Impl<T>::get_factor(algp_ctx* c, void* out) {
    if (!c->factored || c->train_dirty) return fail(c, ALGP_ERR_STATE, "get_factor: call algp_factorize first");
    const int64_t N = c->N;
    ALGP_HIP(hipMemcpy2DAsync(out, sizeof(T) * N, c->L.p, sizeof(T) * c->Lld, sizeof(T) * N, N, hipMemcpyDeviceToHost, c->stream));
    ALGP_TRY(sync(c));
    T* Lh = (T*)out;
    for (int64_t i = 0; i < N; ++i)
        for (int64_t j = i + 1; j < N; ++j) Lh[i * N + j] = (T)0;
    return ALGP_OK;
}

template struct Impl<float>;
template struct Impl<double>;

}

extern "C" {

int algp_factorize(algp_ctx* c) {
    CHECK_CTX(c);
    NEED_HYPERS(c);
    if (c->n_pool <= 0) return fail(c, ALGP_ERR_STATE, "factorize: set a pool first");
    if (!c->y0.p || (int64_t)c->pos_in_train.size() != c->n_pool)
        return fail(c, ALGP_ERR_STATE, "factorize: call algp_set_train first");
    FINISH(c, DISPATCH(c, factorize(c, 0)));
}

int algp_factorize_update(algp_ctx* c, int64_t* kept_rows) {
    CHECK_CTX(c);
    NEED_HYPERS(c);
    if (c->n_pool <= 0) return fail(c, ALGP_ERR_STATE, "factorize_update: set a pool first");
    if (!c->y0.p || (int64_t)c->pos_in_train.size() != c->n_pool)
        return fail(c, ALGP_ERR_STATE, "factorize_update: call algp_set_train first");
    int rc = DISPATCH(c, factorize(c, 1));
    if (kept_rows) *kept_rows = rc == ALGP_OK ? c->kept_rows_last : 0;
    if (c->prof_on) prof_collect(c);
    return rc;
}

int algp_get_logdet(algp_ctx* c, double* logdet) {
    CHECK_CTX(c);
    if (!c->factored || c->train_dirty || !logdet) return fail(c, ALGP_ERR_STATE, "get_logdet: call algp_factorize first");
    *logdet = c->logdet;
    return ALGP_OK;
}

int algp_get_entropy(algp_ctx* c, double* H) {
    CHECK_CTX(c);
    if (!c->factored || c->train_dirty || !H) return fail(c, ALGP_ERR_STATE, "get_entropy: call algp_factorize first");
    *H = (double)c->N * ENT_CONST + 0.5 * c->logdet;
    return ALGP_OK;
}

int algp_get_mll(algp_ctx* c, double* mll) {
    CHECK_CTX(c);
    if (!c->factored || c->train_dirty || !mll) return fail(c, ALGP_ERR_STATE, "get_mll: call algp_factorize first");
    *mll = -0.5 * c->yalpha - 0.5 * c->logdet - 0.5 * (double)c->N * 1.8378770664093453;
    return ALGP_OK;
}

int algp_get_alpha(algp_ctx* c, void* out) { CHECK_CTX(c); FINISH(c, DISPATCH(c, get_alpha(c, out))); }

int algp_get_factor(algp_ctx* c, void* out) { CHECK_CTX(c); FINISH(c, DISPATCH(c, get_factor(c, out))); }

int algp_factorize_from(algp_ctx* c, algp_ctx* src, int64_t* kept_rows) {
    CHECK_CTX(c);
    if (!src) return fail(c, ALGP_ERR_BAD_ARG, "factorize_from: null source");
    NEED_HYPERS(c);
    if (c->n_pool <= 0) return fail(c, ALGP_ERR_STATE, "factorize_from: set a pool first");
    if (!c->y0.p || (int64_t)c->pos_in_train.size() != c->n_pool)
        return fail(c, ALGP_ERR_STATE, "factorize_from: call algp_set_train first");
    int rc = DISPATCH(c, factorize_from(c, src));
    if (kept_rows) *kept_rows = rc == ALGP_OK ? c->kept_rows_last : 0;
    if (c->prof_on) prof_collect(c);
    return rc;
}

#if ALGP_TEST_HOOKS
int algp_debug_get_factor_rows(algp_ctx* c, int64_t row0, int64_t nrows, int64_t ncols, void* out) {
    CHECK_CTX(c);
    if (!c->factored || c->train_dirty) return fail(c, ALGP_ERR_STATE, "debug_get_factor_rows: call algp_factorize first");
    if (row0 < 0 || nrows < 0 || ncols < 0 || row0 + nrows > c->Npad || ncols > c->Npad || (nrows > 0 && ncols > 0 && !out))
        return fail(c, ALGP_ERR_BAD_ARG, "debug_get_factor_rows: rows / columns outside the factor");
    if (nrows == 0 || ncols == 0) return ALGP_OK;
    ALGP_HIP(hipMemcpy2DAsync(out, c->es * (size_t)ncols, (const char*)c->L.p + (size_t)row0 * c->Lld * c->es, c->es * (size_t)c->Lld,
                              c->es * (size_t)ncols, (size_t)nrows, hipMemcpyDeviceToHost, c->stream));
    return sync(c);
}
#endif
// ... 3 lines not shown
```

### algp_amd/csrc/api_greedy.hip

```cpp
#include "api_impl.h"

using namespace algp;

namespace algp {


template <typename T>
int Impl<T>::scores_enqueue(algp_ctx* c, int criterion, double static_std, double mobile_std, double* dst) {
    if (!c->solved) return fail(c, ALGP_ERR_STATE, "scores: call algp_solve_candidates first");
    if (!c->prior_noise) return fail(c, ALGP_ERR_STATE, "scores: candidates were set with predictive semantics");
    ALGP_TRY(flush_lazy(c));
    const double ss = static_std * static_std, sm = mobile_std * mobile_std;
    const double delta = 1.0 / (1.0 / ss + 1.0 / sm) - sm;
    if (!dst) dst = (double*)c->scores.p;
    if (criterion == ALGP_CRIT_MUTUAL_INFORMATION) {
        ALGP_TRY(mi_scores_enqueue(c, ss, sm, delta, dst));
    } else if (criterion == ALGP_CRIT_VARIANCE_REDUCTION) {
        ALGP_TRY(vr_scores_enqueue(c, ss, delta, dst));
    } else if (criterion == ALGP_CRIT_ENTROPY) {
        ALGP_TRY(score_launch<T>(c, c->M, (const int*)c->ckind.p, (const unsigned char*)c->alive.p, (const T*)c->dstat.p,
                                 ss, delta, (const double*)nullptr, dst));
    } else {
        return fail(c, ALGP_ERR_BAD_ARG, "unknown criterion");
    }
// ... 3 lines not shown
    if (dst != (double*)c->scores.p)
        ALGP_HIP(hipMemcpyAsync(c->scores.p, dst, sizeof(double) * c->M, hipMemcpyDeviceToDevice, c->stream));
    return ALGP_OK;
}

template <typename T>
int Impl<T>::scores(algp_ctx* c, int criterion, double static_std, double mobile_std, void* out, int out_is_device) {
    if (criterion == ALGP_CRIT_VARIANCE_REDUCTION && vr_over_ranks(c)) ALGP_TRY(vr_shard_step(c, ALGP_OK, true));
    ALGP_TRY(scores_enqueue(c, criterion, static_std, mobile_std, out_is_device ? (double*)out : nullptr));
    if (!out_is_device && out)
        ALGP_HIP(hipMemcpyAsync(out, c->scores.p, sizeof(double) * c->M, hipMemcpyDeviceToHost, c->stream));
    return sync(c);
}


template <typename T>
int Impl<T>::argmax(algp_ctx* c, int64_t* local_pos, int64_t* pool_idx, double* value) {
    if (!c->solved) return fail(c, ALGP_ERR_STATE, "argmax: no scores");
    if (c->M == 0) return fail(c, ALGP_ERR_BAD_ARG, "argmax: empty candidate set");
    double* sc = (double*)c->scal.p;
    ALGP_TRY(argmax_launch(c, (const double*)c->scores.p, c->M, sc + SC_AMAXV, (int64_t*)(sc + SC_AMAXI)));
    double host[2];
    ALGP_HIP(hipMemcpyAsync(host, sc + SC_AMAXV, 2 * sizeof(double), hipMemcpyDeviceToHost, c->stream));
    ALGP_TRY(sync(c));
    int64_t pos;
    memcpy(&pos, &host[1], sizeof(int64_t));
    if (local_pos) *local_pos = pos;
    if (pool_idx) *pool_idx = pos >= 0 ? c->cand_idx[pos] : -1;
    if (value) *value = host[0];
    return ALGP_OK;
}

template <typename T>
typename Impl<T>::RemoteSlots Impl<T>::remote_slots(algp_ctx* c) {
    char* b = (char*)c->remote.p;
    RemoteSlots r;
    r.cidx = (int64_t*)(b + 0);
    r.ckind = (int*)(b + 64);
    r.ss = (T*)(b + 128);
    r.dot = (T*)(b + 192);
    r.dstat = (T*)(b + 256);
    r.mu = (T*)(b + 320);
    r.alive = (unsigned char*)(b + 384);
    r.fresh = (int*)(b + 448);
    r.score = (double*)(b + 512);
    return r;
}

template <typename T>
int Impl<T>::remote_row(algp_ctx* c, int64_t pool_idx, int in_train) {
    const int64_t N = c->N, Npad = c->Npad, ldv = c->ldv;
    T* l = p(c->lrow);
    ALGP_TRY(ensure(c, c->remote, 640));
    RemoteSlots r = remote_slots(c);
    ALGP_HIP(hipMemsetAsync(l, 0, sizeof(T) * ldv, c->stream));
    ALGP_HIP(hipMemsetAsync(c->remote.p, 0, 640, c->stream));
    const int unit_host = in_train ? (int)c->pos_in_train[pool_idx] : -1;
    ALGP_HIP(hipMemcpyAsync(r.cidx, &pool_idx, sizeof(int64_t), hipMemcpyHostToDevice, c->stream));
    ALGP_HIP(hipMemcpyAsync(r.ckind, &unit_host, sizeof(int), hipMemcpyHostToDevice, c->stream));
    KmatSrc s = make_src(c);
    ALGP_TRY(kmat_launch<T>(c, s, r.cidx, 1, 1, (const int64_t*)c->Aidx.p, N, Npad, nullptr, 0, r.ckind, 0, l, ldv));
    ALGP_TRY(trsv_forward<T>(c, p(c->L), Npad, c->Lld, p(c->invD), l));
    ALGP_TRY(rows_reduce_launch<T>(c, l, 1, ldv, Npad, (const T*)nullptr, r.ss, (T*)nullptr));
    const T prior = (T)(c->hyp.outputscale + (c->prior_noise ? c->hyp.noise : 0.0));
    ALGP_TRY(cand_finalize_launch<T>(c, 1, r.ckind, r.cidx, c->pool_is_cov ? (const T*)c->Cp.p : nullptr, c->n_pool, prior,
                                     (const T*)nullptr, r.ss, r.dot, (T)0, r.dstat, r.mu, r.alive));
    if (!c->picks.empty())
        ALGP_TRY(lazy_refresh_launch<T>(c, 1, 2, 0, (const LazyPick*)c->lazypicks.p, (int)c->picks.size(), r.ckind, r.cidx,
                                        s, p(c->prevrows), ldv, l, r.dstat, r.fresh, r.alive, r.score, c->lazy_ss, c->lazy_delta));
    return ALGP_OK;
}


template <typename T>
int Impl<T>::commit_enqueue(algp_ctx* c, int64_t pool_idx, double ss, double delta, const char* winner_payload) {
    if (c->debug_fail_next_commit) {
        const int code = c->debug_fail_next_commit;
        c->debug_fail_next_commit = 0;
        return fail(c, code, "commit_pick: failure injected by algp_debug_fail_at");
    }
    if (!c->solved) return fail(c, ALGP_ERR_STATE, "commit_pick: call algp_solve_candidates first");
    if (pool_idx < 0 || pool_idx >= c->n_pool) return fail(c, ALGP_ERR_BAD_ARG, "commit_pick: index outside the pool");
    if ((int64_t)c->picks.size() >= MAX_APPEND) return fail(c, ALGP_ERR_STATE, "commit_pick: append capacity exhausted; re-factorize");
    for (auto& pk : c->picks)
        if (pk.pool_idx == pool_idx) return fail(c, ALGP_ERR_BAD_ARG, "commit_pick: site already static-sampled");
    const int in_train = c->pos_in_train[pool_idx] >= 0 ? 1 : 0;
    const int64_t local = c->cand_pos[pool_idx];
    const int64_t ldv = c->ldv, ncols = c->ncols;
    const size_t q = c->picks.size();
    const T* dsrc;
    if (local >= 0) {
        if (c->lazy_stale) ALGP_TRY(lazy_launch(c, 0, local, ss, delta));
        ALGP_HIP(hipMemsetAsync(c->lrow.p, 0, sizeof(T) * ldv, c->stream));
        ALGP_HIP(hipMemcpyAsync(c->lrow.p, p(c->Vt) + local * ldv, sizeof(T) * ncols, hipMemcpyDeviceToDevice, c->stream));
        dsrc = p(c->dstat) + local;
    } else if (winner_payload) {
        ALGP_HIP(hipMemsetAsync(c->lrow.p, 0, sizeof(T) * ldv, c->stream));
        ALGP_HIP(hipMemcpyAsync(c->lrow.p, winner_payload + 32, sizeof(T) * ncols, hipMemcpyDeviceToDevice, c->stream));
        dsrc = (const T*)(winner_payload + 24);
    } else {
        ALGP_TRY(remote_row(c, pool_idx, in_train));
        dsrc = remote_slots(c).dstat;
    }
    double* sc = (double*)c->scal.p;
    ALGP_HIP(hipMemcpyAsync(p(c->prevrows) + (int64_t)q * ldv, c->lrow.p, sizeof(T) * ldv, hipMemcpyDeviceToDevice, c->stream));
    ALGP_TRY(commit_finalize_launch<T>(c, dsrc, in_train, ss, delta, (LazyPick*)c->lazypicks.p + q, pool_idx, ncols,
                                       local >= 0 ? (unsigned char*)c->alive.p + local : nullptr,
                                       local >= 0 ? (double*)c->scores.p + local : nullptr, sc + SC_COMMIT));
    PickRec pr;
    pr.pool_idx = pool_idx;
    pr.in_train = in_train;
    c->picks.push_back(pr);
    c->ncols = ncols + 1;
    c->lazy_stale = true;
    return ALGP_OK;
}

template <typename T>
int Impl<T>::commit_pick(algp_ctx* c, int64_t pool_idx, double static_std, double mobile_std) {
    const double ss = static_std * static_std, sm = mobile_std * mobile_std;
    const double delta = 1.0 / (1.0 / ss + 1.0 / sm) - sm;
    const bool was_stale = c->lazy_stale;
    ALGP_TRY(commit_enqueue(c, pool_idx, ss, delta));
    double host[2];
    ALGP_HIP(hipMemcpyAsync(host, (double*)c->scal.p + SC_COMMIT, 2 * sizeof(double), hipMemcpyDeviceToHost, c->stream));
    const int src = sync_checked(c, "commit_pick");
    if (src != ALGP_OK) {
        c->picks.pop_back();
        c->ncols -= 1;
        c->lazy_stale = was_stale;
        c->bounds_valid = false;
        return src;
    }
    const double scale = host[1];
    if (!(scale == scale) || isinf(scale)) {
        c->picks.pop_back();
        c->ncols -= 1;
        c->lazy_stale = was_stale;
        return fail(c, ALGP_ERR_NOT_PD, "commit_pick: posterior variance of the pick is not positive");
    }
    return ALGP_OK;
}


template <typename T>
int Impl<T>::lazy_launch(algp_ctx* c, int mode, int64_t pos, double ss, double delta, const int64_t* pos_dev) {
    return lazy_refresh_launch<T>(c, c->M, mode, pos, (const LazyPick*)c->lazypicks.p, (int)c->picks.size(),
                                  (const int*)c->ckind.p, (const int64_t*)c->Cidx.p, make_src(c), p(c->prevrows), c->ldv, p(c->Vt),
                                  p(c->dstat), (int*)c->fresh.p, (const unsigned char*)c->alive.p,
                                  (double*)c->scores.p, ss, delta, pos_dev);
}

template <typename T>
int Impl<T>::reset_lazy(algp_ctx* c) {
    ALGP_TRY(ensure(c, c->fresh, sizeof(int) * std::max<int64_t>(c->Mpad, 1)));
    ALGP_TRY(ensure(c, c->lazypicks, sizeof(LazyPick) * MAX_APPEND));
    ALGP_HIP(hipMemsetAsync(c->fresh.p, 0, sizeof(int) * std::max<int64_t>(c->Mpad, 1), c->stream));
    c->lazy_stale = false;
    c->bounds_valid = false;
    return ALGP_OK;
}

template <typename T>
int Impl<T>::flush_lazy(algp_ctx* c) {
    if (!c->lazy_stale) return ALGP_OK;
    ALGP_TRY(lazy_launch(c, 2, 0, c->lazy_ss, c->lazy_delta));
    c->lazy_stale = false;
    return ALGP_OK;
}


template <typename T>
int Impl<T>::enqueue_local_best(algp_ctx* c, double ss, double delta) {
    double* sc = (double*)c->scal.p;
    int64_t* pos_dev = (int64_t*)(sc + SC_AMAXI);
    if (c->lazy_stale) {
        ALGP_TRY(argmax_launch(c, (const double*)c->scores.p, c->M, sc + SC_AMAXV, pos_dev));
        ALGP_TRY(lazy_launch(c, 0, 0, ss, delta, pos_dev));
        ALGP_TRY(lazy_launch(c, 1, 0, ss, delta, pos_dev));
    }
    return argmax_launch(c, (const double*)c->scores.p, c->M, sc + SC_AMAXV, pos_dev);
}

template <typename T>
int Impl<T>::ensure_bounds(algp_ctx* c, int criterion, double static_std, double mobile_std, double ss, double delta) {
    static const bool lazy_on = env_switch("ALGP_LAZY_GREEDY", true);
    if (criterion != ALGP_CRIT_ENTROPY || !lazy_on || !c->bounds_valid || c->lazy_ss != ss || c->lazy_delta != delta)
        return scores_enqueue(c, criterion, static_std, mobile_std, nullptr);
    return ALGP_OK;
}


template <typename T>
int Impl<T>::best_candidate(algp_ctx* c, int criterion, double static_std, double mobile_std, int64_t* local_pos,
                              int64_t* pool_idx, double* value) {
    if (!c->solved) return fail(c, ALGP_ERR_STATE, "best_candidate: call algp_solve_candidates first");
    if (c->M == 0) return fail(c, ALGP_ERR_BAD_ARG, "best_candidate: empty candidate set");
    const double ss = static_std * static_std, sm = mobile_std * mobile_std;
    const double delta = 1.0 / (1.0 / ss + 1.0 / sm) - sm;
    ALGP_TRY(ensure_bounds(c, criterion, static_std, mobile_std, ss, delta));
    double* sc = (double*)c->scal.p;
    int64_t pos = -1;
    double val = -INFINITY;
    for (int round = 0; round < 8; ++round) {
        ALGP_TRY(enqueue_local_best(c, ss, delta));
        ALGP_TRY(fresh_at_launch(c, (const int*)c->fresh.p, (const int64_t*)(sc + SC_AMAXI), sc + SC_AMAXF));
        double host[3];
        ALGP_HIP(hipMemcpyAsync(host, sc + SC_AMAXV, 2 * sizeof(double), hipMemcpyDeviceToHost, c->stream));
        ALGP_HIP(hipMemcpyAsync(host + 2, sc + SC_AMAXF, sizeof(double), hipMemcpyDeviceToHost, c->stream));
        ALGP_TRY(sync(c));
        memcpy(&pos, &host[1], sizeof(int64_t));
        val = host[0];
        if (pos < 0 || !c->lazy_stale) break;
        if ((int)host[2] >= (int)c->picks.size()) break;
    }
    if (local_pos) *local_pos = pos;
    if (pool_idx) *pool_idx = pos >= 0 ? c->cand_idx[pos] : -1;
    if (value) *value = val;
    return ALGP_OK;
}


template <typename T>
int Impl<T>::greedy_picks(algp_ctx* c, int criterion, double static_std, double mobile_std, int k, int64_t* picks_out,
                           double* ut_out) {
    const double ss = static_std * static_std, sm = mobile_std * mobile_std;
    const double delta = 1.0 / (1.0 / ss + 1.0 / sm) - sm;
    double* sc = (double*)c->scal.p;
    for (int pck = 0; pck < k; ++pck) {
        double rec[5];
        const char* winner = nullptr;
        for (int round = 0;; ++round) {
            int st = ALGP_OK;
            if (c->debug_fail_next_pick) {
                st = fail(c, c->debug_fail_next_pick, "greedy: failure injected by algp_debug_fail_next_pick");
                c->debug_fail_next_pick = 0;
            } else if (!c->solved) {
                st = fail(c, ALGP_ERR_STATE, "greedy: call algp_solve_candidates first");
            } else if (!c->prior_noise) {
                st = fail(c, ALGP_ERR_STATE, "greedy: candidates were set with predictive semantics");
            }
            if (st == ALGP_OK && c->pending_pick_error) {
                st = fail(c, c->pending_pick_error, c->pending_pick_msg);
                c->pending_pick_error = 0;
            }
            if (criterion == ALGP_CRIT_MUTUAL_INFORMATION && round == 0 && c->comm_nranks > 1) {
                ALGP_TRY(mi_shard_step(c, ss, sm, st, pck == 0));
            }
            if (criterion == ALGP_CRIT_VARIANCE_REDUCTION && round == 0 && vr_over_ranks(c)) {
                ALGP_TRY(vr_shard_step(c, st, pck == 0));
            }
            if (st == ALGP_OK && c->M > 0) st = ensure_bounds(c, criterion, static_std, mobile_std, ss, delta);
            if (st == ALGP_OK && c->M > 0) st = enqueue_local_best(c, ss, delta);
            const bool have = st == ALGP_OK && c->M > 0;
            const std::string local_err = c->err;
            ALGP_TRY(comm_pick_exchange(c, have ? sc + SC_AMAXV : nullptr, have ? (const int64_t*)(sc + SC_AMAXI) : nullptr,
                                        (const int64_t*)c->Cidx.p, c->lazy_stale ? (const int*)c->fresh.p : nullptr,
                                        (int)c->picks.size(), st, rec, &winner));
            if (rec[3] >= 2.0) {
                const int code = (int)rec[3];
                if (st != ALGP_OK) return fail(c, st, local_err);
                if ((int)rec[4] == c->comm_rank || !(c->comm || c->host_gather)) {
                    const int rc2 = sync_checked(c, "greedy");
                    if (rc2 != ALGP_OK) return rc2;
                }
                return fail(c, code, "greedy_sharded: rank " + std::to_string((int)rec[4]) + " failed with error " +
                                         std::to_string(code) + " while resolving its best candidate; no rank committed pick " +
                                         std::to_string(pck));
            }
            if (rec[3] == 0.0) break;
            if (round == 8) return fail(c, ALGP_ERR_STATE, "greedy: the best candidate could not be resolved (NaN utilities)");
        }
        if (rec[1] < 0) return fail(c, ALGP_ERR_STATE, "greedy: no candidate left on any rank");
        if (!(rec[0] > -INFINITY))
            return fail(c, ALGP_ERR_STATE, "greedy: every remaining candidate is already static-sampled (a further pick would "
                                           "re-sample a static site)");
        const int64_t pool_idx = (int64_t)rec[1];
        if (picks_out) picks_out[pck] = pool_idx;
        if (ut_out) ut_out[pck] = rec[0];
        const int crc = commit_enqueue(c, pool_idx, ss, delta, winner);
        if (crc != ALGP_OK) {
            if (!(c->comm || c->host_gather)) return crc;
            c->pending_pick_error = crc;
            c->pending_pick_msg = "greedy: committing pick " + std::to_string(pck) + " failed on this rank: " + c->err;
            if (pck + 1 == k) return crc;
        }
    }
    return ALGP_OK;
}


template <typename T>
int Impl<T>::greedy(algp_ctx* c, int criterion, double static_std, double mobile_std, int k, const int64_t* forced,
                      int64_t* picks_out, double* ut_out) {
    if (!ut_out && !forced && criterion == ALGP_CRIT_ENTROPY && !c->comm && !c->host_gather)
        return greedy_picks(c, criterion, static_std, mobile_std, k, picks_out, nullptr);
    for (int pck = 0; pck < k; ++pck) {
        int64_t pool_idx;
        if (ut_out || forced) {
            ALGP_TRY(scores(c, criterion, static_std, mobile_std, ut_out ? ut_out + (int64_t)pck * c->M : nullptr, 0));
            if (forced) pool_idx = forced[pck];
            else ALGP_TRY(argmax(c, nullptr, &pool_idx, nullptr));
        } else {
            ALGP_TRY(best_candidate(c, criterion, static_std, mobile_std, nullptr, &pool_idx, nullptr));
        }
        if (picks_out) picks_out[pck] = pool_idx;
        ALGP_TRY(commit_pick(c, pool_idx, static_std, mobile_std));
    }
    return ALGP_OK;
// ... 152 lines not shown
```

### algp_amd/csrc/api_impl.h

```cpp
#pragma once
#include <limits.h>
#include <math.h>
#include <string.h>

#include <algorithm>
#include <stdlib.h>

#include "common.h"
#include "vecops.h"

namespace algp {

void release(algp_ctx* c, DevBuf& b);
void release(algp_ctx* c, MiState& mi);
void release(algp_ctx* c, VrState& vr);
hipEvent_t sync_event_api(algp_ctx* c, size_t i);
KmatSrc make_src(algp_ctx* c);
int sync(algp_ctx* c);
int sync_checked(algp_ctx* c, const char* what);
inline bool vr_over_ranks(const algp_ctx* c) { return c->vr.xrows != 0 && c->comm_nranks > 1; }

enum class SolveRoute { Segments, TaskList, Sweep, Folded };

template <typename T>
struct Impl {
    static T* p(DevBuf& b) { return (T*)b.p; }
    static int rescale_pool(algp_ctx* c);
    static int kernel_matrix(algp_ctx* c, const void* x1, int64_t n1, const void* x2, int64_t n2, const void* diag_add,
                             int add_lik, void* out);
    static int set_pool(algp_ctx* c, const void* x, int64_t n);
    static uint64_t train_sites_hash(const algp_ctx* c, const std::vector<int64_t>& idx);
    static int set_pool_cov(algp_ctx* c, const void* cov, int64_t n);
    static int set_train(algp_ctx* c, const int64_t* idx, int64_t N, const void* y, const void* var);

    struct Panel {
        T* P;
        int64_t ldp, mpad;
        int mode;
        T* inv_out = nullptr;
        bool inv_enqueued = false;
        int64_t z_row = -1;
        int64_t short_rows = 0;
    };
    static bool panel_fits(int64_t npad, int64_t mpad);
    static int factor_resident(algp_ctx* c, T* A, int64_t n, int64_t npad, T* invD, int slot_logdet, int slot_info,
                               double* logdet, int64_t ld = 0, int64_t pivot_offset = 0, Panel* panel = nullptr);
    static int reserve_factor(algp_ctx* c, int64_t npad_need, int64_t keep_rows, int64_t keep_height = 0,
                              bool headroom = false);
    static bool vt_rows_for_new_sites(algp_ctx* c, int64_t Nb, int64_t p0, std::vector<int64_t>& src_row,
                                      std::vector<int64_t>& lrow, std::vector<T>& lscale, bool& any_second);
    static int exchange_new_rows(algp_ctx* c, int64_t Nb, int64_t p0, int* placed, int st_in = 0);
    static int factorize(algp_ctx* c, int incremental, Panel* panel = nullptr);
    static int finish_factor(algp_ctx* c, int64_t keep, int64_t p0, double ld_total, T* z_src = nullptr);
    static int factorize_from(algp_ctx* c, algp_ctx* src);
    static int need_alpha(algp_ctx* c);
    static int set_candidates(algp_ctx* c, const int64_t* idx, int64_t M, int prior_noise, const void* extra);

    struct SolvePlan {
        SolveRoute route = SolveRoute::Sweep;
        int64_t keep = 0;
        std::vector<int> kind;
        std::vector<int64_t> became_unit;
        bool carried_sums = false;
        int nseg = 0;
        int64_t seg_c0[2] = {0, 0};
        int seg_w[2] = {0, 0};
        bool seg_window = false;
        int narrow_r = 0;
        int64_t short_rows = 0;
        bool row_stats = false;
        bool rowstat_done = false;
        bool rhs_fused = false;
        int64_t sweep_end = 0;
        RhsGen gen;
    };
    static int rhs_window(algp_ctx* c, int64_t c0, int64_t w, void* out, int64_t ldo);
    static constexpr int64_t SWEEP_PUSH_TILES = 320;
    static void plan_route(algp_ctx* c, int incremental, bool allow_fold, SolvePlan& pl);
    static int solve_prepare(algp_ctx* c, int incremental, SolvePlan& pl);
    static int solve_run(algp_ctx* c, SolvePlan& pl);
    static int solve_narrow_tile(algp_ctx* c, const SolvePlan& pl);
    static int solve_finish(algp_ctx* c, int incremental, const unsigned char* alive_host, const SolvePlan& pl);
    static int solve_candidates(algp_ctx* c, int incremental, const unsigned char* alive_host);
    static int fit_and_solve(algp_ctx* c);
    static int get_posterior(algp_ctx* c, void* mu, void* var);
    static int get_posterior_cov(algp_ctx* c, void* cov_out, double* mi_out);
    static int posterior_mean(algp_ctx* c, const int64_t* idx, int64_t M, void* mu_out);
    static int sample_posterior(algp_ctx* c, int S, int F, const double* omega, const double* phase, const double* weights,
                                const double* prior, const double* eps, void* out);
    static int group_posterior(algp_ctx* c, const int32_t* group, const double* weight, int64_t Q, void* mean_out, void* cov_out,
                               void* cross_out);
    static int build_set_matrix(algp_ctx* c, const int64_t* idx, int64_t m, const void* var, int64_t* mpad_out, T* dst = nullptr);
    static int set_entropy(algp_ctx* c, const int64_t* idx, int64_t m, const void* var, double* H);
    static int inverse_diag_resident(algp_ctx* c, int64_t m, int64_t mpad, void* diag_out);
    static int set_inverse_diag(algp_ctx* c, const int64_t* idx, int64_t m, const void* var, void* diag_out, double* H);
    static int upload_padded(algp_ctx* c, DevBuf& b, const void* A, int64_t rows, int64_t cols, int64_t rpad,
                             int64_t cpad);
    static int entropy_from_cov(algp_ctx* c, const void* cov, int64_t k, double* H, void* L_out, double* logdet);
    static int gemm_host(algp_ctx* c, int64_t m, int64_t n, int64_t k, double alpha, const void* A, const void* B,
                         double beta, const void* C, void* D);
    static int trsm_host(algp_ctx* c, const void* L, int64_t n, const void* B, int64_t m, void* X);
    struct MiPlan {
        std::vector<int64_t> A, Abar, all, posbar;
        std::vector<T> vA, vall;
        int64_t mb = 0, mbpad = 0, npad = 0;
        size_t rbytes = 0, cbytes = 0;
    };
    static int mi_sets(algp_ctx* c, double ss, double sm, MiPlan& pl);
    static int mi_vectors(algp_ctx* c, const MiPlan& pl, int64_t col);
    static int mi_install(algp_ctx* c, MiPlan& pl, const double* Hs, int form, double ss, double sm);
    static int mi_build(algp_ctx* c, double ss, double sm);
    static int mi_apply_pick(algp_ctx* c, int64_t q, double ss, double sm);
    static int mi_shard_plan(algp_ctx* c, double ss, double sm, MiPlan& pl);
    static int mi_shard_build(algp_ctx* c, MiPlan& pl, double* H3);
    static int mi_shard_fold(algp_ctx* c, int st);
    static int mi_shard_step(algp_ctx* c, double ss, double sm, int st, bool first_of_call);
    static int mi_scores_enqueue(algp_ctx* c, double ss, double sm, double delta, double* dst);
    static int vr_product(algp_ctx* c);
    static int vr_fold(algp_ctx* c, int64_t q);
    static int vr_scores_enqueue(algp_ctx* c, double ss, double delta, double* dst);
    static int vr_zero_picks_block(algp_ctx* c, int64_t q);
    static int vr_shard_build(algp_ctx* c, int64_t max_rows, int st = 0);
    static int vr_shard_fold(algp_ctx* c, int st);
    static int vr_shard_step(algp_ctx* c, int st, bool first_of_call);
    static int set_target_weights(algp_ctx* c, const double* w);
    static int target_variance(algp_ctx* c, double* sum);
    static int scores_enqueue(algp_ctx* c, int criterion, double static_std, double mobile_std, double* dst);
    static int scores(algp_ctx* c, int criterion, double static_std, double mobile_std, void* out, int out_is_device);
    static int argmax(algp_ctx* c, int64_t* local_pos, int64_t* pool_idx, double* value);

    struct RemoteSlots {
        int64_t* cidx;
        int* ckind;
        T *ss, *dot, *dstat, *mu;
        unsigned char* alive;
        int* fresh;
        double* score;
    };
    static RemoteSlots remote_slots(algp_ctx* c);
    static int remote_row(algp_ctx* c, int64_t pool_idx, int in_train);
    static int commit_enqueue(algp_ctx* c, int64_t pool_idx, double ss, double delta, const char* winner_payload = nullptr);
    static int commit_pick(algp_ctx* c, int64_t pool_idx, double static_std, double mobile_std);
    static int lazy_launch(algp_ctx* c, int mode, int64_t pos, double ss, double delta, const int64_t* pos_dev = nullptr);
    static int reset_lazy(algp_ctx* c);
    static int flush_lazy(algp_ctx* c);
    static int enqueue_local_best(algp_ctx* c, double ss, double delta);
    static int ensure_bounds(algp_ctx* c, int criterion, double static_std, double mobile_std, double ss, double delta);
    static int best_candidate(algp_ctx* c, int criterion, double static_std, double mobile_std, int64_t* local_pos,
                              int64_t* pool_idx, double* value);
    static int greedy_picks(algp_ctx* c, int criterion, double static_std, double mobile_std, int k, int64_t* picks_out, double* ut_out);
    static int greedy(algp_ctx* c, int criterion, double static_std, double mobile_std, int k, const int64_t* forced,
                      int64_t* picks_out, double* ut_out);
    static int score_paths_big(algp_ctx* c, const std::vector<int64_t>& cpos, const std::vector<int64_t>& lpos, int npaths, int maxlen,
                               int maxused, double mobile_std, double* dH);
    static int score_paths(algp_ctx* c, const int64_t* sites, int npaths, int maxlen, double mobile_std, double* dH);
    static int score_paths_mi(algp_ctx* c, const int64_t* sites, int npaths, int maxlen, double static_std, double mobile_std,
                              double* dMI, double* terms);
    static int score_paths_vr(algp_ctx* c, const int64_t* sites, int npaths, int maxlen, double mobile_std, int64_t max_union, double* dV);
    static int mll_grad(algp_ctx* c, double* grad_out, bool have_X = false, bool inv_enqueued = false);
    static int fit_step(algp_ctx* c, double* mll_out, double* grad_out);
    static int get_alpha(algp_ctx* c, void* out);
    static int get_factor(algp_ctx* c, void* out);
    static int selftest(algp_ctx* c, int* mism);
};

template <typename T>
int factor_blocks_batched(algp_ctx* c, T* G, int ppad, T* inv, T* L21, double* logdet, int* info, int B) {
    ALGP_TRY(potrf_diag_batched_launch<T>(c, G, (int64_t)ppad * ppad, ppad, inv, 2 * NB * NB, logdet, info, B));
    if (ppad > NB) {
        T* G21 = G + (int64_t)NB * ppad;
        T* G22 = G21 + NB;
        ALGP_TRY(gemm_nt<T>(c, {.klass = ALGP_PROF_GEMM_OTHER, .m = NB, .n = NB, .k = NB, .A = {G21, ppad, (int64_t)ppad * ppad},
                                .B = {inv, NB, 2 * NB * NB}, .D = {L21, NB, NB * NB}, .batch = B}));
        ALGP_TRY(gemm_nt<T>(c, {.klass = ALGP_PROF_GEMM_OTHER, .m = NB, .n = NB, .k = NB, .alpha = (T)-1, .beta = (T)1, .A = {L21, NB, NB * NB},
                                .B = {L21, NB, NB * NB}, .D = {G22, ppad, (int64_t)ppad * ppad}, .batch = B}));
        ALGP_TRY(potrf_diag_batched_launch<T>(c, G22, (int64_t)ppad * ppad, ppad, inv + NB * NB, 2 * NB * NB, logdet, info, B));
    }
    return ALGP_OK;
}

}

#define DISPATCH(c, call) ((c)->dtype == ALGP_F64 ? Impl<double>::call : Impl<float>::call)
#define CHECK_CTX(c) do { if (!(c)) return ALGP_ERR_BAD_ARG; (c)->err.clear(); hipSetDevice((c)->device); } while (0)
#define NEED_HYPERS(c) do { if (!(c)->hyp.set) return fail(c, ALGP_ERR_STATE, "call algp_set_hypers first"); } while (0)
#define FINISH(c, expr) do { int rc__ = (expr); if ((c)->prof_on) prof_collect(c); return rc__; } while (0)
```

### algp_amd/csrc/common.h

```cpp
#pragma once
#include <stdlib.h>
#include <hip/hip_runtime.h>
#include <stdint.h>
#include <string>
#include <type_traits>
#include <vector>
#include "../../include/algp_hip.h"

namespace algp {

constexpr int NB = 128;
constexpr int MAXD = 8;
constexpr int MAX_APPEND = 128;
constexpr double ENT_CONST = 1.4189385332046727;

inline int64_t round_up(int64_t v, int64_t m) { return (v + m - 1) / m * m; }

constexpr int SC_LOGDET = 0;
constexpr int SC_INFO = 1;
constexpr int SC_AUXLOGDET = 2;
constexpr int SC_AUXINFO = 3;
constexpr int SC_AMAXV = 4;
constexpr int SC_AMAXI = 5;
constexpr int SC_PROBE = 6;
// ... 175 lines not shown
        }
    }
    return kval<T, FAM>(kernel, os, r2);
}
template <typename T, int DP>
__device__ __forceinline__ T bt_entry(int kernel, T os, const T (&xr)[DP], const T (&xc)[DP], int kind, int64_t gcol, int64_t ncols) {
    const T v = kmat_value<T, DP>(kernel, os, xr, xc);
    const T ordinary = (kind == -1 && gcol < ncols) ? v : (T)0;
    const T unit = gcol == (int64_t)kind ? (T)1 : (T)0;
    return kind >= 0 ? unit : ordinary;
}

template <typename T, typename C = T>
struct CovSrc {
    const T* Xs;
    const T* Cp;
    int64_t n_pool;
    int kernel;
    C os, noise;
};
template <int DP, bool NOISE = true, typename S, typename XA, typename XB>
__device__ __forceinline__ auto pool_cov(const S& s, int64_t pa, int64_t pb, const XA* xa, const XB* xb) {
    using C = decltype(s.os);
    if (s.Cp) return (C)s.Cp[pa * s.n_pool + pb];
    C r2 = (C)0;
#pragma unroll
    for (int d = 0; d < DP; ++d) {
        const C df = (C)xa[d] - (C)xb[d];
        r2 += df * df;
    }
    C v = kval<C>(s.kernel, s.os, r2);
    if (NOISE && pa == pb) v += s.noise;
    return v;
}
template <int DP, bool NOISE = true, typename S, typename XA>
__device__ __forceinline__ auto pool_cov(const S& s, int64_t pa, int64_t pb, const XA* xa) {
    return pool_cov<DP, NOISE>(s, pa, pb, xa, s.Xs + pb * DP);
}
template <int DP, typename S>
__device__ __forceinline__ auto pool_cov(const S& s, int64_t pa, int64_t pb) {
    return pool_cov<DP>(s, pa, pb, s.Xs + pa * DP, s.Xs + pb * DP);
}
}

struct algp_ctx {
    int device = 0;
    int dtype = ALGP_F64;
    size_t es = 8;
    hipStream_t stream = nullptr;
    hipStream_t stream2 = nullptr;
    hipStream_t stream3 = nullptr, stream4 = nullptr;
    int trsm_chunks = 3;
    bool trsm_chunks_explicit = false;
    int cu_count = 0;
    bool gemm_sched = false;
    hipStream_t cur = nullptr;
    std::vector<hipEvent_t> sync_events;
    std::string err;
    int64_t pivot = 0;
    double last_jitter = 0;
    algp::Hypers hyp;

    int64_t n_pool = 0;
    bool pool_is_cov = false;
    algp::DevBuf Xs;
    algp::DevBuf Xraw;
    algp::DevBuf Cp;
    algp::DevBuf tw;
    bool has_tw = false;
    uint64_t tw_hash = 0;
    std::vector<int64_t> pos_in_train;
    std::vector<uint64_t> site_hash;

    int64_t N = 0, Npad = 0;
    int64_t Lld = 0;
    int64_t Nfact = 0;
    std::vector<int64_t> fact_idx;
    std::vector<double> fact_var;
    std::vector<double> train_var_host;
    uint64_t fact_hyp_stamp = 0, hyp_stamp = 1;
    bool train_dirty = false;
    int64_t kept_rows_last = 0;
    std::vector<int64_t> train_idx;
    bool mean_override = false;
    double mean_value = 0;
    bool train_has_repeats = false;
    algp::DevBuf Aidx, yA, varA, y0, L, invD, z, alpha, scal;
    double ybar = 0, logdet = 0, yalpha = 0;
    bool factored = false;
    algp::DevBuf yraw, uvec, wvec;
    std::vector<double> train_y_host, fact_y;
    int64_t uw_rows = 0;
    int64_t uw_stable = 0;
    algp::DevBuf acc3;
    algp::DevBuf rowstat;
    algp::DevBuf splitk;
    algp::DevBuf ldpart;
    algp::DevBuf tailPart;
    algp::DevBuf tailE;
    algp::DevBuf gemm_part;
    algp::DevBuf inv512, inv512_scr, trsm_tmp;
    algp::DevBuf rhs_rx, rhs_cx, rhs_rk;
    std::vector<algp::DagCache> dag_cache;
    algp::DevBuf dag_state;
    algp::DevBuf trsv_ctrl;
    algp::DevBuf dag_stats;
    int64_t acc_cols = 0, acc_M = -1;
    int64_t factor_rows_from_vt = 0;
    bool alpha_valid = false;

    int64_t M = 0, Mpad = 0, ldv = 0;
    int64_t ncols = 0;
    int prior_noise = 1;
    std::vector<int64_t> cand_idx;
    std::vector<int64_t> cand_pos;
    algp::DevBuf Cidx, ckind, cextra, Vt, dstat, mu, alive, scores, lrow, tvec, amax;
    std::vector<algp::PickRec> picks;
    algp::DevBuf prevrows;
    algp::DevBuf remote;
    algp::DevBuf fresh, lazypicks;
    bool lazy_stale = false;
    bool bounds_valid = false;
    double lazy_ss = 0, lazy_delta = 0;
    bool solved = false;
    int64_t ldv_cap = 0;
    std::vector<int64_t> vt_fact_idx, vt_cand_idx;
    std::vector<double> vt_fact_var;
    std::vector<int> vt_kind;
    uint64_t vt_hyp_stamp = 0;
    int vt_prior_noise = -1;
    bool vt_has_extra = false;
    int64_t kept_cols_last = 0;

    algp::MiState mi;
    algp::VrState vr;

    void* comm = nullptr;
    algp_allgather_fn host_gather = nullptr;
    void* host_gather_user = nullptr;
    int comm_nranks = 1, comm_rank = 0;
    algp::DevBuf commbuf;
    void* comm_host = nullptr;
    size_t comm_host_cap = 0;
    std::vector<int32_t> site_owner;
    uint64_t site_owner_hash = 0;
    algp::DevBuf rowx;
    void* rowx_host = nullptr;
    size_t rowx_host_cap = 0;
    int64_t rows_from_peers = 0;
    int64_t row_exchanges = 0, row_fallbacks = 0;
    int debug_fail_next_rowx = 0;
    int pending_pick_error = 0;
    std::string pending_pick_msg;
    int64_t n_syncs = 0;
    int debug_dag_stall_ticket = -1;
    int debug_trsv_stall_block = -1;
    int debug_fail_next_pick = 0;
    int debug_fail_next_commit = 0;
    int debug_fail_next_pack = 0;
    int debug_fail_next_mi = 0;
    int debug_fail_next_vr = 0;
    double xhdr[4] = {0, 0, 0, 0};

    algp::DevBuf auxA, auxInv, auxW, auxIdx, auxVar, auxD, hostStage;
    algp::DevBuf smp;
    algp::DevBuf grp;

    bool prof_on = false;
    algp::ProfSlot prof[ALGP_PROF_COUNT];
    std::vector<algp::PendingEvent> pending;
    std::vector<hipEvent_t> event_pool;
    int64_t dev_bytes = 0;
};

namespace algp {

int fail(algp_ctx* c, int code, const std::string& msg);
int ensure(algp_ctx* c, DevBuf& b, size_t bytes);
void prof_begin(algp_ctx* c, int klass, double flops, double bytes);
void prof_end(algp_ctx* c);
bool prof_launch_events(algp_ctx* c, int klass, double flops, double bytes, hipEvent_t* a, hipEvent_t* b);
void prof_collect(algp_ctx* c);
void prof_span_begin(algp_ctx* c, int klass, double flops, double bytes);
void prof_span_end(algp_ctx* c);
void prof_span_end_on(algp_ctx* c, hipStream_t st);
void prof_span_begin2(algp_ctx* c, int klass, double flops, double bytes);
void prof_span_end2(algp_ctx* c);

inline bool env_switch(const char* name, bool dflt) {
    const char* e = getenv(name);
    return (e && *e) ? atoi(e) != 0 : dflt;
}
inline int env_int(const char* name, int dflt) {
    const char* e = getenv(name);
    return (e && *e) ? atoi(e) : dflt;
}

#define ALGP_HIP(call)                                                                          \
    do {                                                                                        \
        hipError_t e_ = (call);                                                                 \
        if (e_ != hipSuccess)                                                                   \
            return algp::fail(c, ALGP_ERR_HIP, std::string(#call) + ": " + hipGetErrorString(e_)); \
    } while (0)
#define ALGP_TRY(call)          \
    do {                        \
        int r_ = (call);        \
        if (r_ != ALGP_OK) return r_; \
    } while (0)

struct ProfScope {
    algp_ctx* c;
    ProfScope(algp_ctx* c_, int klass, double flops, double bytes) : c(c_) { prof_begin(c, klass, flops, bytes); }
    ~ProfScope() { prof_end(c); }
};

struct KmatSrc {
    const void* Xs;
    const void* Cp;
    int64_t n_pool;
    int DP;
    int kernel;
    double outputscale;
    double noise;
};
template <typename T, typename C = T>
inline CovSrc<T, C> cov_src(const KmatSrc& s) {
    return {(const T*)s.Xs, (const T*)s.Cp, s.n_pool, s.kernel, (C)s.outputscale, (C)(s.Cp ? 0.0 : s.noise)};
}
template <typename F>
inline void with_dp(int DP, F&& f) {
    if (DP == 2) f(std::integral_constant<int, 2>{});
    else if (DP == 4) f(std::integral_constant<int, 4>{});
    else f(std::integral_constant<int, 8>{});
}
#define ALGP_INSTANTIATE(f) \
    template decltype(f<double>) f<double>; \
    template decltype(f<float>) f<float>

struct RhsGen {
    const void* rx = nullptr;
    const void* cx = nullptr;
    const int* rk = nullptr;
    int64_t ncols = 0;
    int DP = 0, kernel = 0;
    double outputscale = 0;
    int (*window)(algp_ctx* c, int64_t c0, int64_t w, void* out, int64_t ldo) = nullptr;
};
template <typename T>
int rhs_gather_launch(algp_ctx* c, const T* Xs, int DP, const int64_t* ridx, int64_t rows, int64_t rows_pad, const int* unit,
                      const int64_t* cidx, int64_t cols, int64_t cols_pad, T* rx, T* cx, int* rk);
template <typename T>
int gemm_nt_launch_gen(algp_ctx* c, int klass, int64_t m, int64_t n, int64_t k, T alpha, const T* A, int64_t lda, const T* B,
                       int64_t ldb, T beta, const RhsGen& gen, int64_t col0, T* D, int64_t ldd);
bool rhs_gen_supported(int DP, bool pool_is_cov);

template <typename T>
int kmat_launch(algp_ctx* c, const KmatSrc& s, const int64_t* ridx, int64_t rows, int64_t rows_pad,
                const int64_t* cidx, int64_t cols, int64_t cols_pad, const T* diag_add,
                int add_noise_on_equal, const int* unit, int identity_pad, T* out, int64_t ldo,
                int64_t ident_shift = 0, int64_t col_shift = 0);

template <typename T>
int kmat_xy_launch(algp_ctx* c, const T* xs1, int64_t n1, const T* xs2, int64_t n2, int symmetric,
                   const T* diag_add, double add_noise, T* out, int64_t ldo);
template <typename T>
int scale_coords_launch(algp_ctx* c, const T* x, int64_t n, T* xs);

#pragma clang diagnostic ignored "-Wc++20-designator"
template <typename P>
struct Mat {
    P* p = nullptr;
    int64_t ld = 0;
    int64_t stride = 0;
};
template <typename T>
struct GemmNt {
    int klass = 0;
    int64_t m = 0, n = 0, k = 0;
    T alpha = (T)1, beta = (T)0;
    Mat<const T> A, B, C;
    Mat<T> D;
    int batch = 1;
    int lower_only = 0;
    int ktri = 0, kcut = 0;
    const T* stat_w = nullptr;
    T* stat_out = nullptr;
    int64_t stat_ld = 0;
};
template <typename T>
int gemm_nt(algp_ctx* c, const GemmNt<T>& p);
template <typename T>
int gemm_nt_launch(algp_ctx* c, int klass, int64_t m, int64_t n, int64_t k, T alpha, const T* A,
                   int64_t lda, const T* B, int64_t ldb, T beta, const T* C, int64_t ldc, T* D,
                   int64_t ldd, int lower_only);
template <typename T>
int gemm_nt_launch_tri(algp_ctx* c, int klass, int64_t m, int64_t n, const T* A, int64_t lda, const T* B, int64_t ldb, T* D,
                       int64_t ldd, const T* w, T* stat_out, int64_t stat_ld);
template <typename T>
int gemm_nt_launch_stats(algp_ctx* c, int klass, int64_t m, int64_t k, T alpha, const T* A, int64_t lda, const T* B, int64_t ldb,
                         T* D, int64_t ldd, const T* w, T* stat_out, int64_t stat_ld);
template <typename T>
int gemm_nt_launch_vr(algp_ctx* c, int klass, int64_t mpad, int64_t n, int64_t k, const T* Vt, int64_t ldv, int64_t ncol0,
                      const KmatSrc& s, const int64_t* cidx, const int* ckind, int64_t M, const T* tw, T* part, int64_t part_ld);
template <typename T>
int gemm_nt_launch_vrx(algp_ctx* c, int klass, int64_t mpad, int64_t n, int64_t k, const T* Vt, int64_t ldv, const T* B, int64_t ldb,
                       const int64_t* cpool, int nslices, int64_t slice_bytes, const KmatSrc& s, const int64_t* cidx, const int* ckind,
                       int64_t M, const T* tw, T* part, int64_t part_ld);
template <typename T>
int gemm_nt_launch_pvr(algp_ctx* c, int klass, int64_t upad, int64_t n, int64_t k, const T* R, int64_t ldr, const T* Vt, int64_t ldv,
                       int64_t ncol0, const KmatSrc& s, const int64_t* uidx, int64_t U, const int64_t* cidx, const int* ckind, int64_t M,
                       const T* tw, T* E, int64_t lde);
template <typename T>
int syrk_skinny_sub(algp_ctx* c, int klass, const T* X, int64_t m, int64_t k, int64_t ldx, T* C, int64_t ldc,
                    algp::DevBuf& scratch);

template <typename T>
int potrf_diag_launch(algp_ctx* c, T* A, int64_t lda, T* inv_out, double* logdet_acc, int* info,
                      int64_t block_row0);

template <typename T>
int potrf_diag_batched_launch(algp_ctx* c, T* A, int64_t sA, int64_t lda, T* inv_out, int64_t sInv, double* logdet, int* info, int batch);

int comm_unique_id(void* out128, std::string* why);
int comm_init(algp_ctx* c, int nranks, int rank, const void* unique_id128);
void comm_destroy(algp_ctx* c);
int comm_init_host(algp_ctx* c, int nranks, int rank, algp_allgather_fn fn, void* user);
int comm_pick_exchange(algp_ctx* c, const double* val_dev, const int64_t* pos_dev, const int64_t* cidx_dev,
                       const int* fresh_dev, int npicks, int status, double* rec5, const char** winner_payload);
int comm_reserve(algp_ctx* c);
int comm_agree(algp_ctx* c, const double* mine, std::vector<double>& all, int nd = 4);
int comm_rows_reserve(algp_ctx* c, size_t bytes_per_rank);
int comm_rows_gather(algp_ctx* c, size_t bytes_per_rank, const size_t* used_bytes = nullptr);
int comm_exchange(algp_ctx* c, size_t bytes, int st, const double* v3, std::vector<double>& hdr, int& code, int& bad);
int comm_agreed_fail(algp_ctx* c, int code, int bad, const std::string& local_err, const char* what, const char* state);
size_t comm_payload_bytes(const algp_ctx* c);
int comm_debug_first_max(algp_ctx* c, const double* triples, int nranks, double* out5);
void dag_release(algp_ctx* c);
template <typename T>
int cholesky_blocked(algp_ctx* c, T* A, int64_t npad, int64_t ld, T* invD, double* logdet_acc,
                     int* info);
constexpr int64_t DAG_MIN_TILES = 8, DAG_MAX_TILES = 192, DAG_MAX_PANEL_TILES = 400;
bool dag_enabled();
template <typename T>
int cholesky_dag_panel(algp_ctx* c, T* A, int64_t npad, int64_t ld, T* invD, double* logdet_acc, int* info, T* P, int64_t ldp,
                       int64_t mpad, int mode, int pshort = 0);
template <typename T>
int solve_dag_panel(algp_ctx* c, const T* L, int64_t npad, int64_t ld, const T* invD, int* info, T* P, int64_t ldp, int64_t mpad,
                    int mode, int pshort = 0);
template <typename T>
int trsm_blocked(algp_ctx* c, int klass, T* X, int64_t mpad, int64_t ldx, const T* L, int64_t npad,
                 int64_t ldl, const T* invD, int64_t col_start = 0, const T* stat_w = nullptr, T* stat_out = nullptr,
                 int64_t stat_ld = 0, bool* stats_done = nullptr, const RhsGen* gen = nullptr);
bool trsm_sched_wanted(const algp_ctx* c, int64_t mpad, int64_t npad, int64_t col_start);
template <typename T>
int tail_cols_launch(algp_ctx* c, int klass, T* X, int64_t mpad, int64_t ldx, const T* L, int64_t ldl, int64_t lrows, const T* invD_blk,
                     int64_t c0, int w, const T* E_window = nullptr);
template <typename T>
int trinv_upper(algp_ctx* c, int klass, T* X, int64_t npad, int64_t ldx, const T* L, int64_t ldl, const T* invD);
template <typename T>
int trinv_upper_inplace(algp_ctx* c, int klass, T* XL, int64_t npad, int64_t ld, const T* invD);
template <typename T>
int syrk_upper(algp_ctx* c, int klass, const T* X, int64_t npad, int64_t ldx, T* C, int64_t ldc);

template <typename T>
int trsv_forward(algp_ctx* c, const T* L, int64_t npad, int64_t ldl, const T* invD, T* b, int64_t kb_start = 0);
template <typename T>
int trsv_forward2(algp_ctx* c, const T* L, int64_t npad, int64_t ldl, const T* invD, T* b0, T* b1, int64_t kb_start = 0);
template <typename T>
int tail_gemv2_launch(algp_ctx* c, const T* L, int64_t ldl, int64_t k, int64_t npad, T* u, T* w);
template <typename T>
int trsv_backward(algp_ctx* c, const T* L, int64_t npad, int64_t ldl, const T* invD, T* b);

template <typename T>
int rows_reduce_launch(algp_ctx* c, const T* Vt, int64_t rows, int64_t ldv, int64_t ncols, const T* w, T* ss, T* dot,
                       int64_t tri_c0 = -1);

template <typename T>
struct SampleEpi {
    T* out;
    int64_t ld, nrows;
    int slive;
    T ybar;
    const T* y0;
    const T* var;
    const T* eps;
    T noise;
};
constexpr int SAMPLE_TILE = 128;
constexpr int SAMPLE_KT = 32;
template <typename T>
int sample_features_launch(algp_ctx* c, const T* Xs, int DP, const int64_t* idx, const T* Wt, const T* om, const T* ph,
                           int64_t Fpad, int64_t flop_f, T scale, const SampleEpi<T>& e);
template <typename T>
int sample_values_launch(algp_ctx* c, const T* prior, int64_t n_pool, const int64_t* idx, const SampleEpi<T>& e);
template <typename T>
int sample_convert_launch(algp_ctx* c, const double* src, int64_t rows, int64_t cols, T* dst, int64_t rows_pad, int64_t cols_pad,
                          int64_t ldd, int transposed);

template <typename T>
int test_mfma_launch(algp_ctx* c, int* mismatches_dev);
template <typename T>
int bench_gemm(algp_ctx* c, int64_t m, int64_t n, int64_t k, int lower_only, int beta_one, int reps,
               double* ms_out, bool gen_c = false);

}
```

### algp_amd/csrc/potrf.hip

```cpp
#include "common.h"
#include "mfma.h"
#include "diag.h"
#include "vecops.h"
#include <stdlib.h>

namespace algp {

template <typename T, bool FACTOR>
__global__ __launch_bounds__(256) void potrf_diag_kernel(T* A, int64_t lda, T* inv_out, double* logdet_acc, int* info,
                                                          int64_t block_row0) {
    __shared__ DiagShared<T> sh;
    diag128_run<T, FACTOR>(sh, A, lda, inv_out, logdet_acc, true, info, block_row0);
}

template <typename T>
int potrf_diag_launch(algp_ctx* c, T* A, int64_t lda, T* inv_out, double* logdet_acc, int* info,
                      int64_t block_row0) {
    ProfScope ps(c, ALGP_PROF_POTRF_DIAG, 128.0 * 128.0 * 128.0, sizeof(T) * 3.0 * 128.0 * 128.0);
    hipLaunchKernelGGL((potrf_diag_kernel<T, true>), dim3(1), dim3(256), 0, c->cur, A, lda, inv_out, logdet_acc,
                       info, block_row0);
    ALGP_HIP(hipGetLastError());
    return ALGP_OK;
}
ALGP_INSTANTIATE(potrf_diag_launch);
// ... 186 lines not shown
            }
            if (j1 >= npad || rc != ALGP_OK) break;
            const int64_t wq = (npad - j1 < PW) ? npad - j1 : PW;
            if (sb) {
                hipEvent_t ea = sync_event(c, 8 + 2 * (size_t)(jb & 3)), eb = sync_event(c, 9 + 2 * (size_t)(jb & 3));
                hipEventRecord(ea, sa);
                if (jb > 0) hipStreamWaitEvent(sa, sync_event(c, 9 + 2 * (size_t)((jb - 1) & 3)), 0);
                rc = gemm_nt_launch<T>(c, klass, mpad, wq, w, (T)-1, Xj, ldx, L + j1 * ldl + j0, ldl, (T)1, X + j1, ldx, X + j1, ldx, 0);
                if (rc == ALGP_OK && j1 + wq < npad) {
                    hipStreamWaitEvent(sb, ea, 0);
                    c->cur = sb;
                    rc = gemm_nt_launch<T>(c, klass, mpad, npad - (j1 + wq), w, (T)-1, Xj, ldx, L + (j1 + wq) * ldl + j0, ldl, (T)1,
                                           X + j1 + wq, ldx, X + j1 + wq, ldx, 0);
                    c->cur = sa;
                }
                hipEventRecord(eb, sb);
            } else {
                rc = gemm_nt_launch<T>(c, klass, mpad, npad - j1, w, (T)-1, Xj, ldx, L + j1 * ldl + j0, ldl, (T)1, X + j1, ldx,
                                       X + j1, ldx, 0);
            }
        }
        if (sb) {
            hipEvent_t done = sync_event(c, 16);
            hipEventRecord(done, sb);
            hipStreamWaitEvent(sa, done, 0);
        }
        return rc;
    }
    const int64_t TWB = WB;
    for (int64_t j0 = 0; j0 < npad; j0 += TWB) {
        const int64_t w = (npad - j0 < TWB) ? npad - j0 : TWB;
        if (j0 + w <= col_start) continue;
        const int64_t cs = j0 > col_start ? j0 : col_start;
        T* Xj = X + j0;
        if (inv512 && tmp512 && w == TWB && col_start == 0) {
            if (j0 > 0 && gen) ALGP_TRY(gemm_nt_launch_gen<T>(c, klass, mpad, TWB, j0, (T)-1, X, ldx, L + j0 * ldl, ldl, (T)1, *gen, j0, tmp512, TWB));
            else if (j0 > 0) ALGP_TRY(gemm_nt_launch<T>(c, klass, mpad, TWB, j0, (T)-1, X, ldx, L + j0 * ldl, ldl, (T)1, Xj, ldx, tmp512, TWB, 0));
            ALGP_TRY(gemm_nt_launch_tri<T>(c, klass, mpad, TWB, tmp512, TWB, inv512 + (j0 / TWB) * TWB * TWB, TWB, Xj, ldx,
                                           stat_w ? stat_w + j0 : nullptr, stat_out ? stat_out + 2 * (j0 / NB) * stat_ld : nullptr, stat_ld));
            continue;
        }
        if (gen && (j0 == 0 || cs != j0)) return fail(c, ALGP_ERR_STATE, "internal: generated right-hand sides outside the scheduled sweep");
        if (j0 > 0 && gen)
            ALGP_TRY(gemm_nt_launch_gen<T>(c, klass, mpad, w, j0, (T)-1, X, ldx, L + j0 * ldl, ldl, (T)1, *gen, j0, Xj, ldx));
        else if (j0 > 0)
            ALGP_TRY(gemm_nt_launch<T>(c, klass, mpad, j0 + w - cs, j0, (T)-1, X, ldx, L + cs * ldl, ldl, (T)1, X + cs,
                                       ldx, X + cs, ldx, 0));
        for (int64_t k0 = cs; k0 < j0 + w; k0 += NB) {
            T* Xk = X + k0;
            if (k0 > j0)
                ALGP_TRY(gemm_nt_launch<T>(c, klass, mpad, NB, k0 - j0, (T)-1, Xj, ldx, L + k0 * ldl + j0, ldl, (T)1,
                                           Xk, ldx, Xk, ldx, 0));
            if (stat_out)
                ALGP_TRY(gemm_nt_launch_stats<T>(c, klass, mpad, NB, (T)1, Xk, ldx, invD + (k0 / NB) * NB * NB, NB, Xk, ldx,
                                                 stat_w + k0, stat_out + 2 * (k0 / NB) * stat_ld, stat_ld));
            else
                ALGP_TRY(gemm_nt_launch<T>(c, klass, mpad, NB, NB, (T)1, Xk, ldx, invD + (k0 / NB) * NB * NB, NB, (T)0,
                                           nullptr, 0, Xk, ldx, 0));
        }
    }
    return ALGP_OK;
}

template <typename T>
int trinv_upper(algp_ctx* c, int klass, T* X, int64_t npad, int64_t ldx, const T* L, int64_t ldl, const T* invD) {
    for (int64_t j0 = 0; j0 < npad; j0 += WB) {
        const int64_t w = (npad - j0 < WB) ? npad - j0 : WB, j1 = j0 + w;
        for (int64_t k0 = j0; k0 < j1; k0 += NB) {
            T* Xk = X + k0;
            const int64_t rows = k0 + NB;
            ALGP_TRY(gemm_nt_launch<T>(c, klass, rows, NB, NB, (T)1, Xk, ldx, invD + (k0 / NB) * NB * NB, NB, (T)0,
                                       nullptr, 0, Xk, ldx, 0));
            if (k0 + NB < j1)
                ALGP_TRY(gemm_nt_launch<T>(c, klass, rows, j1 - (k0 + NB), NB, (T)-1, Xk, ldx, L + (k0 + NB) * ldl + k0,
                                           ldl, (T)1, Xk + NB, ldx, Xk + NB, ldx, 0));
        }
        if (j1 < npad)
            ALGP_TRY(gemm_nt_launch<T>(c, klass, j1, npad - j1, w, (T)-1, X + j0, ldx, L + j1 * ldl + j0, ldl, (T)1,
                                       X + j1, ldx, X + j1, ldx, 0));
    }
    return ALGP_OK;
}

template <typename T>
__global__ __launch_bounds__(256) void tri_prep_kernel(T* A, int64_t ld) {
    const int64_t bi = blockIdx.y, bj = blockIdx.x;
    if (bi > bj) return;
    T* t = A + bi * NB * ld + bj * NB;
    for (int e = threadIdx.x; e < NB * NB; e += 256) {
        const int r = e >> 7, q = e & 127;
        t[(int64_t)r * ld + q] = (bi == bj && r == q) ? (T)1 : (T)0;
    }
}
template <typename T>
int trinv_upper_inplace(algp_ctx* c, int klass, T* XL, int64_t npad, int64_t ld, const T* invD) {
    const unsigned nt = (unsigned)(npad / NB);
    if (nt > 65535) return fail(c, ALGP_ERR_BAD_ARG, "trinv_upper_inplace: matrix too large");
    hipLaunchKernelGGL(tri_prep_kernel<T>, dim3(nt, nt), dim3(256), 0, c->cur, XL, ld);
    ALGP_HIP(hipGetLastError());
    for (int64_t j0 = 0; j0 < npad; j0 += WB) {
        const int64_t w = (npad - j0 < WB) ? npad - j0 : WB, j1 = j0 + w;
        for (int64_t k0 = j0; k0 < j1; k0 += NB) {
            T* Xk = XL + k0;
            const int64_t rows = k0 + NB;
            ALGP_TRY(gemm_nt_launch<T>(c, klass, rows, NB, NB, (T)1, Xk, ld, invD + (k0 / NB) * NB * NB, NB, (T)0, nullptr, 0, Xk, ld, 0));
            if (k0 + NB < j1)
                ALGP_TRY(gemm_nt_launch<T>(c, klass, rows, j1 - (k0 + NB), NB, (T)-1, Xk, ld, XL + (k0 + NB) * ld + k0, ld, (T)1,
                                           Xk + NB, ld, Xk + NB, ld, 0));
        }
        if (j1 >= npad) break;
        if (j0 > 0)
            ALGP_TRY(gemm_nt_launch<T>(c, klass, j0, npad - j1, w, (T)-1, XL + j0, ld, XL + j1 * ld + j0, ld, (T)1, XL + j1, ld, XL + j1, ld, 0));
        for (int64_t r0 = j0; r0 < j1; r0 += NB)
            ALGP_TRY(gemm_nt_launch<T>(c, klass, NB, npad - j1, j1 - r0, (T)-1, XL + r0 * ld + r0, ld, XL + j1 * ld + r0, ld, (T)1,
                                       XL + r0 * ld + j1, ld, XL + r0 * ld + j1, ld, 0));
    }
    return ALGP_OK;
}
ALGP_INSTANTIATE(trinv_upper_inplace);

template <typename T>
int syrk_upper(algp_ctx* c, int klass, const T* X, int64_t npad, int64_t ldx, T* C, int64_t ldc) {
    return gemm_nt<T>(c, {.klass = klass, .m = npad, .n = npad, .k = npad, .A = {X, ldx}, .B = {X, ldx}, .D = {C, ldc}, .lower_only = 1, .ktri = 1});
}
ALGP_INSTANTIATE(syrk_upper);
ALGP_INSTANTIATE(trinv_upper);

template <typename T>
static int trsm_rows(algp_ctx* c, int klass, T* X, int64_t mpad, int64_t ldx, const T* L, int64_t npad,
                     int64_t ldl, const T* invD, int64_t col_start, bool whole_solve, const T* stat_w = nullptr,
                     T* stat_out = nullptr, int64_t stat_ld = 0, const T* inv512 = nullptr, T* tmp512 = nullptr,
                     const RhsGen* gen = nullptr) {
    return trsm_rows_blocked<T>(c, klass, X, mpad, ldx, L, npad, ldl, invD, col_start, whole_solve, stat_w, stat_out, stat_ld, inv512,
                                tmp512, gen);
}

static hipEvent_t sync_event(algp_ctx* c, size_t i) {
    while (c->sync_events.size() <= i) {
        hipEvent_t e;
        hipEventCreateWithFlags(&e, hipEventDisableTiming);
        c->sync_events.push_back(e);
    }
    return c->sync_events[i];
}

static bool trsm_inv512_wanted(const algp_ctx* c, int64_t mpad, int64_t npad, int64_t col_start) {
    return env_switch("ALGP_TRSM_INV512", true) && col_start == 0 && mpad / NB > TRSM_PUSH_TILES && npad / WB >= 1 && c->cur == c->stream;
}
bool trsm_sched_wanted(const algp_ctx* c, int64_t mpad, int64_t npad, int64_t col_start) {
    return trsm_inv512_wanted(c, mpad, npad, col_start) && !c->trsm_chunks_explicit && c->cu_count > 0 && env_switch("ALGP_TRSM_SCHED", true);
}

template <typename T>
int trsm_blocked(algp_ctx* c, int klass, T* X, int64_t mpad, int64_t ldx, const T* L, int64_t npad,
                 int64_t ldl, const T* invD, int64_t col_start, const T* stat_w, T* stat_out, int64_t stat_ld, bool* stats_done,
                 const RhsGen* gen) {
    const int64_t tiles = mpad / NB;
    const bool stats = stat_out && stat_w && col_start == 0 && tiles > TRSM_PUSH_TILES;
    if (stats_done) *stats_done = stats;
    if (!stats) stat_out = nullptr;
    const T* inv512 = nullptr;
    T* tmp512 = nullptr;
    {
        if (trsm_inv512_wanted(c, mpad, npad, col_start) &&
            ensure(c, c->inv512, sizeof(T) * (size_t)(npad / WB) * WB * WB) == ALGP_OK &&
            ensure(c, c->inv512_scr, sizeof(T) * inv512_scratch_elems<T>(npad)) == ALGP_OK &&
            ensure(c, c->trsm_tmp, sizeof(T) * (size_t)mpad * WB) == ALGP_OK) {
            ALGP_TRY(build_inv512<T>(c, klass, L, ldl, invD, npad, (T*)c->inv512.p, (T*)c->inv512_scr.p));
            inv512 = (const T*)c->inv512.p;
            tmp512 = (T*)c->trsm_tmp.p;
        }
    }
    const bool sched = inv512 && trsm_sched_wanted(c, mpad, npad, col_start) &&
                       ensure(c, c->gemm_part, sizeof(T) * 128 * 128 * 2 * (size_t)c->cu_count) == ALGP_OK;
    if (gen && !sched) {
        ALGP_TRY(gen->window(c, 0, npad, X, ldx));
        gen = nullptr;
    }
    if (inv512) {
        if (gen) ALGP_TRY(gen->window(c, 0, WB, tmp512, WB));
        else ALGP_HIP(hipMemcpy2DAsync(tmp512, sizeof(T) * WB, X, sizeof(T) * ldx, sizeof(T) * WB, (size_t)mpad, hipMemcpyDeviceToDevice, c->cur));
    }
    if (sched) {
        c->gemm_sched = true;
        const int rc = trsm_rows<T>(c, klass, X, mpad, ldx, L, npad, ldl, invD, col_start, true, stat_w, stat_out, stat_ld, inv512, tmp512, gen);
        c->gemm_sched = false;
        return rc;
    }
    hipStream_t streams[4] = {c->stream, c->stream2, c->stream3, c->stream4};
    int nch = c->trsm_chunks < 1 ? 1 : (c->trsm_chunks > 4 ? 4 : c->trsm_chunks);
    while (nch > 1 && (!streams[nch - 1] || tiles < 32 * nch)) --nch;
    if (col_start == 0 && tiles <= TRSM_PUSH_TILES) nch = 1;
    if (nch == 1 || c->cur != c->stream)
        return trsm_rows<T>(c, klass, X, mpad, ldx, L, npad, ldl, invD, col_start, true, stat_w, stat_out, stat_ld, inv512, tmp512);
    ALGP_HIP(hipEventRecord(sync_event(c, 0), streams[0]));
    int rc = ALGP_OK;
    int64_t r0 = 0;
    for (int k = nch - 1; k >= 0; --k) {
        const int64_t rows = (k == 0) ? mpad - r0 : (tiles / nch) * NB;
        if (k > 0) ALGP_HIP(hipStreamWaitEvent(streams[k], sync_event(c, 0), 0));
        c->cur = streams[k];
        if (rc == ALGP_OK)
            rc = trsm_rows<T>(c, klass, X + r0 * ldx, rows, ldx, L, npad, ldl, invD, col_start, false, stat_w,
                              stat_out ? stat_out + r0 : nullptr, stat_ld, inv512, tmp512 ? tmp512 + r0 * WB : nullptr);
        r0 += rows;
    }
    c->cur = streams[0];
    for (int k = 1; k < nch; ++k) {
        hipEventRecord(sync_event(c, (size_t)k), streams[k]);
        hipStreamWaitEvent(streams[0], sync_event(c, (size_t)k), 0);
    }
    return rc;
}
ALGP_INSTANTIATE(trsm_blocked);

template <typename T>
__global__ void sub_partials_rect_kernel(T* C, int64_t ldc, int64_t m, int64_t n, const T* P, int nchunks) {
    const int64_t i = (int64_t)blockIdx.y * 16 + (threadIdx.x >> 4), j = (int64_t)blockIdx.x * 16 + (threadIdx.x & 15);
    if (i >= m || j >= n) return;
    T s = (T)0;
    for (int q = 0; q < nchunks; ++q) s += P[(int64_t)q * m * n + i * n + j];
    C[i * ldc + j] -= s;
}

template <typename T>
__global__ void sub_partials_kernel(T* C, int64_t ldc, int64_t m, const T* P, int nchunks) {
    const int64_t i = (int64_t)blockIdx.y * 16 + (threadIdx.x >> 4), j = (int64_t)blockIdx.x * 16 + (threadIdx.x & 15);
    if (i >= m || j > i) return;
    T s = (T)0;
    for (int q = 0; q < nchunks; ++q) s += P[(int64_t)q * m * m + i * m + j];
    C[i * ldc + j] -= s;
}

template <typename T>
int syrk_skinny_sub(algp_ctx* c, int klass, const T* X, int64_t m, int64_t k, int64_t ldx, T* C, int64_t ldc,
                    DevBuf& scratch) {
    if (m <= 0 || k <= 0) return ALGP_OK;
    const int64_t kb = k / NB;
    int64_t per = (kb + 127) / 128;
    if (per < 4) per = 4;
    const int64_t nfull = kb / per, rem = kb - nfull * per;
    if (m > 4 * NB || nfull < 2)
        return gemm_nt_launch<T>(c, klass, m, m, k, (T)-1, X, ldx, X, ldx, (T)1, C, ldc, C, ldc, 1);
    ALGP_TRY(ensure(c, scratch, sizeof(T) * (size_t)(nfull + 1) * m * m));
    T* P = (T*)scratch.p;
    ALGP_TRY(gemm_nt<T>(c, {.klass = klass, .m = m, .n = m, .k = per * NB, .A = {X, ldx, per * NB}, .B = {X, ldx, per * NB},
                            .D = {P, m, m * m}, .batch = (int)nfull, .lower_only = 1}));
    int nch = (int)nfull;
    if (rem > 0) {
        ALGP_TRY(gemm_nt_launch<T>(c, klass, m, m, rem * NB, (T)1, X + nfull * per * NB, ldx, X + nfull * per * NB, ldx,
                                   (T)0, nullptr, m, P + nfull * m * m, m, 1));
        ++nch;
    }
    hipLaunchKernelGGL(sub_partials_kernel<T>, dim3((unsigned)((m + 15) / 16), (unsigned)((m + 15) / 16)), dim3(256), 0,
                       c->cur, C, ldc, m, P, nch);
    ALGP_HIP(hipGetLastError());
    return ALGP_OK;
}
template <typename T>
int gemm_splitk_sub(algp_ctx* c, int klass, int64_t m, int64_t n, int64_t k, const T* A, int64_t lda, const T* B,
                    int64_t ldb, T* C, int64_t ldc, DevBuf& scratch) {
    if (m <= 0 || n <= 0 || k <= 0) return ALGP_OK;
    const int64_t tiles = (m / NB) * (n / NB), kb = k / NB;
    int64_t want = tiles > 0 ? 512 / tiles : 1;
    if (want > 128) want = 128;
    int64_t per = want > 0 ? (kb + want - 1) / want : kb;
    if (per < 4) per = 4;
    const int64_t nfull = kb / per, rem = kb - nfull * per;
    if (tiles > 64 || nfull < 2)
        return gemm_nt_launch<T>(c, klass, m, n, k, (T)-1, A, lda, B, ldb, (T)1, C, ldc, C, ldc, 0);
    ALGP_TRY(ensure(c, scratch, sizeof(T) * (size_t)(nfull + 1) * m * n));
    T* P = (T*)scratch.p;
    ALGP_TRY(gemm_nt<T>(c, {.klass = klass, .m = m, .n = n, .k = per * NB, .A = {A, lda, per * NB}, .B = {B, ldb, per * NB},
                            .D = {P, n, m * n}, .batch = (int)nfull}));
    int nch = (int)nfull;
    if (rem > 0) {
        ALGP_TRY(gemm_nt_launch<T>(c, klass, m, n, rem * NB, (T)1, A + nfull * per * NB, lda, B + nfull * per * NB, ldb,
                                   (T)0, nullptr, n, P + nfull * m * n, n, 0));
        ++nch;
    }
    hipLaunchKernelGGL(sub_partials_rect_kernel<T>, dim3((unsigned)((n + 15) / 16), (unsigned)((m + 15) / 16)), dim3(256), 0,
                       c->cur, C, ldc, m, n, P, nch);
    ALGP_HIP(hipGetLastError());
    return ALGP_OK;
}

ALGP_INSTANTIATE(syrk_skinny_sub);

template <typename T>
__global__ __launch_bounds__(256) void tail_gemv2_kernel(const T* Lrows, int64_t ld, int64_t nrows, int64_t k, const T* u,
                                                         const T* w, T* uo, T* wo) {
    constexpr int VEC = 16 / sizeof(T);
    typedef T vec_t __attribute__((ext_vector_type(VEC)));
    __shared__ T red[2][4];
    const int lane = threadIdx.x & 63, wave = threadIdx.x >> 6;
    const int64_t r = blockIdx.x;
    const T* row = Lrows + r * ld;
    const int64_t nv = k / VEC, per = (nv + 3) / 4;
    const int64_t v0 = wave * per, v1 = v0 + per < nv ? v0 + per : nv;
    T su = (T)0, sw = (T)0;
    int64_t v = v0 + lane;
    for (; v + 192 < v1; v += 256) {
        vec_t x[4], a[4], b[4];
#pragma unroll
        for (int q = 0; q < 4; ++q) {
            x[q] = *reinterpret_cast<const vec_t*>(row + (v + 64 * q) * VEC);
            a[q] = *reinterpret_cast<const vec_t*>(u + (v + 64 * q) * VEC);
            b[q] = *reinterpret_cast<const vec_t*>(w + (v + 64 * q) * VEC);
        }
#pragma unroll
        for (int q = 0; q < 4; ++q)
#pragma unroll
            for (int e = 0; e < VEC; ++e) {
                su += x[q][e] * a[q][e];
                sw += x[q][e] * b[q][e];
            }
    }
    for (; v < v1; v += 64) {
        const vec_t x = *reinterpret_cast<const vec_t*>(row + v * VEC);
        const vec_t a = *reinterpret_cast<const vec_t*>(u + v * VEC);
        const vec_t b = *reinterpret_cast<const vec_t*>(w + v * VEC);
#pragma unroll
        for (int e = 0; e < VEC; ++e) {
            su += x[e] * a[e];
            sw += x[e] * b[e];
        }
    }
    for (int o = 32; o > 0; o >>= 1) {
        su += __shfl_down(su, o, 64);
        sw += __shfl_down(sw, o, 64);
    }
    if (lane == 0) {
        red[0][wave] = su;
        red[1][wave] = sw;
    }
// ... 37 lines not shown
    const T* Xrow = invD + (int64_t)i * 128 * 128 + r * 128 + q * 32;
    if (kb0 < i) {
#pragma unroll
        for (int e = 0; e < 32; ++e) cur[e] = Lrow[(int64_t)kb0 * 128 + e];
    } else {
#pragma unroll
        for (int e = 0; e < 32; ++e) cur[e] = Xrow[e];
    }
    for (int j = kb0; j < i; ++j) {
        if (j + 1 < i) {
#pragma unroll
            for (int e = 0; e < 32; ++e) nxt[e] = Lrow[(int64_t)(j + 1) * 128 + e];
        } else {
#pragma unroll
            for (int e = 0; e < 32; ++e) nxt[e] = Xrow[e];
        }
        if (tid == 0) {
            bool ok = false;
            const unsigned long long t0 = __builtin_amdgcn_s_memrealtime();
            for (unsigned spins = 0;; ++spins) {
                if (__hip_atomic_load(&flags[j], __ATOMIC_RELAXED, __HIP_MEMORY_SCOPE_AGENT) != 0) { ok = true; break; }
                if (__hip_atomic_load(&ctrl[1], __ATOMIC_RELAXED, __HIP_MEMORY_SCOPE_AGENT) != 0) break;
                if ((spins & 255) == 255 && __builtin_amdgcn_s_memrealtime() - t0 > spin_limit) {
                    atomicCAS(&ctrl[1], 0, i + 1);
                    __hip_atomic_store(sticky, 1, __ATOMIC_RELAXED, __HIP_MEMORY_SCOPE_AGENT);
                    break;
                }
                __builtin_amdgcn_s_sleep(1);
            }
            s_ok = ok ? 1 : 0;
        }
        __syncthreads();
        if (!s_ok) return;
        if (tid < 128) {
#pragma unroll
            for (int v = 0; v < NR; ++v) zs[v][tid] = __hip_atomic_load(bs[v] + (int64_t)j * 128 + tid, __ATOMIC_RELAXED, __HIP_MEMORY_SCOPE_AGENT);
        }
        __syncthreads();
#pragma unroll
        for (int e = 0; e < 32; ++e) {
#pragma unroll
            for (int v = 0; v < NR; ++v) acc[v] += cur[e] * zs[v][q * 32 + e];
        }
#pragma unroll
        for (int e = 0; e < 32; ++e) cur[e] = nxt[e];
        __syncthreads();
    }
#pragma unroll
    for (int v = 0; v < NR; ++v) red[v][q][r] = acc[v];
    __syncthreads();
    if (tid < 128) {
#pragma unroll
        for (int v = 0; v < NR; ++v)
            zs[v][tid] = bs[v][(int64_t)i * 128 + tid] - (((red[v][0][tid] + red[v][1][tid]) + red[v][2][tid]) + red[v][3][tid]);
    }
    __syncthreads();
#pragma unroll
    for (int v = 0; v < NR; ++v) {
        T s = (T)0;
#pragma unroll
        for (int e = 0; e < 32; ++e) s += cur[e] * zs[v][q * 32 + e];
        red[v][q][r] = s;
    }
    __syncthreads();
    if (tid < 128) {
#pragma unroll
        for (int v = 0; v < NR; ++v)
            st_wt(bs[v] + (int64_t)i * 128 + tid, ((red[v][0][tid] + red[v][1][tid]) + red[v][2][tid]) + red[v][3][tid]);
    }
    asm volatile("s_waitcnt vmcnt(0)" ::: "memory");
    __syncthreads();
    if (tid == 0 && i != skip_block) __hip_atomic_store(&flags[i], 1, __ATOMIC_RELAXED, __HIP_MEMORY_SCOPE_AGENT);
}

template <typename T>
__global__ __launch_bounds__(512) void trsv_chain_back_kernel(const T* L, int64_t ld, const T* invD, T* b, int nblk, int* ctrl,
                                                              int* sticky, unsigned long long spin_limit, int skip_block) {
    __shared__ T zs[128];
    __shared__ T red[4][128];
    __shared__ int s_i, s_ok;
    const int tid = threadIdx.x, cc = tid & 127, q = tid >> 7;
    if (tid == 0) s_i = nblk - 1 - atomicAdd(&ctrl[0], 1);
    __syncthreads();
    const int i = __builtin_amdgcn_readfirstlane(s_i);
    if (i < 0) return;
    int* flags = ctrl + 8;
    T acc = (T)0;
    const int qs = __builtin_amdgcn_readfirstlane(q);
    const T* Lblk = L + (int64_t)(qs * 32) * ld + (int64_t)i * 128;
#define Lcol_at(row) (Lblk + (int64_t)(row) * ld)[(unsigned)cc]
    T cur[32], nxt[32];
    const T* Xcol = invD + (int64_t)i * 128 * 128 + (int64_t)(qs * 32) * 128 + cc;
    if (i + 1 < nblk) {
#pragma unroll
        for (int e = 0; e < 32; ++e) cur[e] = Lcol_at((int64_t)(nblk - 1) * 128 + e);
    } else {
#pragma unroll
        for (int e = 0; e < 32; ++e) cur[e] = Xcol[e * 128];
    }
    for (int j = nblk - 1; j > i; --j) {
        if (j - 1 > i) {
#pragma unroll
            for (int e = 0; e < 32; ++e) nxt[e] = Lcol_at((int64_t)(j - 1) * 128 + e);
        } else {
#pragma unroll
            for (int e = 0; e < 32; ++e) nxt[e] = Xcol[e * 128];
        }
        if (tid == 0) {
            bool ok = false;
            const unsigned long long t0 = __builtin_amdgcn_s_memrealtime();
            for (unsigned spins = 0;; ++spins) {
                if (__hip_atomic_load(&flags[j], __ATOMIC_RELAXED, __HIP_MEMORY_SCOPE_AGENT) != 0) { ok = true; break; }
                if (__hip_atomic_load(&ctrl[1], __ATOMIC_RELAXED, __HIP_MEMORY_SCOPE_AGENT) != 0) break;
                if ((spins & 255) == 255 && __builtin_amdgcn_s_memrealtime() - t0 > spin_limit) {
                    atomicCAS(&ctrl[1], 0, i + 1);
                    __hip_atomic_store(sticky, 1, __ATOMIC_RELAXED, __HIP_MEMORY_SCOPE_AGENT);
                    break;
                }
                __builtin_amdgcn_s_sleep(1);
            }
            s_ok = ok ? 1 : 0;
        }
        __syncthreads();
        if (!s_ok) return;
        if (tid < 128) zs[tid] = __hip_atomic_load(b + (int64_t)j * 128 + tid, __ATOMIC_RELAXED, __HIP_MEMORY_SCOPE_AGENT);
        __syncthreads();
#pragma unroll
        for (int e = 0; e < 32; ++e) {
            acc += cur[e] * zs[q * 32 + e];
            if ((e & 7) == 7) __builtin_amdgcn_sched_barrier(0);
        }
#pragma unroll
        for (int e = 0; e < 32; ++e) cur[e] = nxt[e];
        __syncthreads();
    }
    red[q][cc] = acc;
    __syncthreads();
    if (tid < 128) zs[tid] = b[(int64_t)i * 128 + tid] - (((red[0][tid] + red[1][tid]) + red[2][tid]) + red[3][tid]);
    __syncthreads();
    {
        T s = (T)0;
#pragma unroll
        for (int e = 0; e < 32; ++e) s += cur[e] * zs[q * 32 + e];
        red[q][cc] = s;
    }
    __syncthreads();
    if (tid < 128) st_wt(b + (int64_t)i * 128 + tid, ((red[0][tid] + red[1][tid]) + red[2][tid]) + red[3][tid]);
    asm volatile("s_waitcnt vmcnt(0)" ::: "memory");
    __syncthreads();
    if (tid == 0 && i != skip_block) __hip_atomic_store(&flags[i], 1, __ATOMIC_RELAXED, __HIP_MEMORY_SCOPE_AGENT);
#undef Lcol_at
}

static int trsv_prepare(algp_ctx* c, int nblk, unsigned long long* spin_limit, int* skip_block) {
    const size_t bytes = sizeof(int) * (size_t)(nblk + 8);
    ALGP_TRY(ensure(c, c->trsv_ctrl, bytes));
    ALGP_HIP(hipMemsetAsync(c->trsv_ctrl.p, 0, bytes, c->cur));
    *spin_limit = 200000000ull;
    *skip_block = -1;
    if (c->debug_trsv_stall_block >= 0) {
        *skip_block = c->debug_trsv_stall_block;
        *spin_limit = 20000000ull;
        c->debug_trsv_stall_block = -1;
    }
    return ALGP_OK;
}

template <typename T>
static int trsv_chain_launch(algp_ctx* c, const T* L, int64_t npad, int64_t ldl, const T* invD, T* b0, T* b1, int64_t kb_start) {
    const int nblk = (int)(npad / NB), kb0 = (int)kb_start;
    if (kb0 >= nblk) return ALGP_OK;
    unsigned long long limit;
    int skip;
    ALGP_TRY(trsv_prepare(c, nblk, &limit, &skip));
    int* sticky = (int*)((double*)c->scal.p + SC_STALL);
    const int nr = b1 ? 2 : 1;
    ProfScope ps(c, ALGP_PROF_TRSV, nr * (double)npad * npad, sizeof(T) * 0.5 * (double)npad * npad);
    if (b1) hipLaunchKernelGGL((trsv_chain_kernel<T, 2>), dim3(nblk - kb0), dim3(512), 0, c->cur, L, ldl, invD, b0, b1, kb0, nblk, (int*)c->trsv_ctrl.p, sticky, limit, skip);
    else hipLaunchKernelGGL((trsv_chain_kernel<T, 1>), dim3(nblk - kb0), dim3(512), 0, c->cur, L, ldl, invD, b0, (T*)nullptr, kb0, nblk, (int*)c->trsv_ctrl.p, sticky, limit, skip);
    ALGP_HIP(hipGetLastError());
    return ALGP_OK;
}

template <typename T>
int trsv_forward(algp_ctx* c, const T* L, int64_t npad, int64_t ldl, const T* invD, T* b, int64_t kb_start) {
    return trsv_chain_launch<T>(c, L, npad, ldl, invD, b, (T*)nullptr, kb_start);
}
template <typename T>
int trsv_forward2(algp_ctx* c, const T* L, int64_t npad, int64_t ldl, const T* invD, T* b0, T* b1, int64_t kb_start) {
    return trsv_chain_launch<T>(c, L, npad, ldl, invD, b0, b1, kb_start);
}
ALGP_INSTANTIATE(trsv_forward2);
template <typename T>
int trsv_backward(algp_ctx* c, const T* L, int64_t npad, int64_t ldl, const T* invD, T* b) {
    const int nblk = (int)(npad / NB);
    if (nblk <= 0) return ALGP_OK;
    unsigned long long limit;
    int skip;
    ALGP_TRY(trsv_prepare(c, nblk, &limit, &skip));
    ProfScope ps(c, ALGP_PROF_TRSV, (double)npad * npad, sizeof(T) * 0.5 * (double)npad * npad);
    hipLaunchKernelGGL(trsv_chain_back_kernel<T>, dim3(nblk), dim3(512), 0, c->cur, L, ldl, invD, b, nblk, (int*)c->trsv_ctrl.p,
                       (int*)((double*)c->scal.p + SC_STALL), limit, skip);
    ALGP_HIP(hipGetLastError());
    return ALGP_OK;
}
ALGP_INSTANTIATE(trsv_forward);
ALGP_INSTANTIATE(trsv_backward);

}
```

Baseline: 652,800.

## Pipeline fit-and-solve sweep: overlap RHS build with forward solve, single readback sync

Adds a dedicated fit_and_solve path for the sweep route. Device buffers are reserved up front, then the Cholesky factor is enqueued and an event is recorded. Candidate RHS generation and the TRSM prelude (inv512 build, first window) run on a second stream alongside the forward substitution for z. The separate host syncs for logdet/info, kind upload and the stall check are folded into one pinned-memory readback at the end. This is meant to remove several host round-trips and to overlap independent work, at the cost of more complex cross-stream ordering and error handling.

```diff
diff --git a/algp_amd/csrc/api.hip b/algp_amd/csrc/api.hip
--- a/algp_amd/csrc/api.hip
+++ b/algp_amd/csrc/api.hip
@@ -38,6 +38,24 @@
     }
     b.p = nullptr;
     b.cap = 0;
+}
+
+int readback_reserve(algp_ctx* c, size_t bytes) {
+    if (c->readback && c->readback_cap >= bytes) return ALGP_OK;
+    if (c->readback) {
+        hipStreamSynchronize(c->stream);
+        hipHostFree(c->readback);
+    }
+    c->readback = nullptr;
+    c->readback_cap = 0;
+    const size_t want = bytes + bytes / 4;
+    if (hipHostMalloc(&c->readback, want, hipHostMallocDefault) != hipSuccess) {
+        (void)hipGetLastError();
+        c->readback = nullptr;
+        return fail(c, ALGP_ERR_OOM, "hipHostMalloc(" + std::to_string(want) + ") for the read-back staging failed");
+    }
+    c->readback_cap = want;
+    return ALGP_OK;
 }
 
 static hipEvent_t get_event(algp_ctx* c) {
@@ -170,12 +188,13 @@
     ALGP_HIP(hipMemcpyAsync(&stall, d, sizeof(int), hipMemcpyDeviceToHost, c->stream));
     ALGP_HIP(hipStreamSynchronize(c->stream));
     c->n_syncs++;
-    if (stall != 0) {
-        hipMemsetAsync(d, 0, sizeof(double), c->stream);
-        return fail(c, ALGP_ERR_HIP, std::string(what) + ": a one-launch kernel stalled (a hand-off between its workgroups never "
-                                     "arrived within the spin limit); the result is incomplete");
-    }
-    return ALGP_OK;
+    return stall_verdict(c, stall, what);
+}
+int stall_verdict(algp_ctx* c, int stall, const char* what) {
+    if (stall == 0) return ALGP_OK;
+    hipMemsetAsync((double*)c->scal.p + SC_STALL, 0, sizeof(double), c->stream);
+    return fail(c, ALGP_ERR_HIP, std::string(what) + ": a one-launch kernel stalled (a hand-off between its workgroups never "
+                                 "arrived within the spin limit); the result is incomplete");
 }
 
 }
@@ -517,6 +536,7 @@
     release(c, c->vr);
     dag_release(c);
     comm_destroy(c);
+    if (c->readback) hipHostFree(c->readback);
     for (hipEvent_t e : c->event_pool) hipEventDestroy(e);
     for (hipEvent_t e : c->sync_events) hipEventDestroy(e);
     hipStreamSynchronize(c->stream2);
diff --git a/algp_amd/csrc/api_candidates.hip b/algp_amd/csrc/api_candidates.hip
--- a/algp_amd/csrc/api_candidates.hip
+++ b/algp_amd/csrc/api_candidates.hip
@@ -116,11 +116,9 @@
 }
 
 template <typename T>
-int Impl<T>::solve_prepare(algp_ctx* c, int incremental, typename Impl<T>::SolvePlan& pl) {
-    const int64_t N = c->N, Npad = c->Npad, M = c->M, Mpad = c->Mpad, keep = pl.keep;
+int Impl<T>::solve_reserve(algp_ctx* c, int incremental, const typename Impl<T>::SolvePlan& pl) {
+    const int64_t Npad = c->Npad, Mpad = c->Mpad, keep = pl.keep;
     const int64_t ldv = Npad + MAX_APPEND;
-    c->solved = false;
-    c->vr.drop();
     if (!c->Vt.p || c->ldv_cap < ldv || (keep == 0 && !incremental && c->ldv_cap != ldv) ||
         c->Vt.cap < sizeof(T) * Mpad * c->ldv_cap) {
         const int64_t newcap = incremental ? round_up(ldv + ldv / 8, NB) : ldv;
@@ -145,23 +143,46 @@
     ALGP_TRY(ensure(c, c->scores, sizeof(double) * Mpad));
     ALGP_TRY(ensure(c, c->lrow, sizeof(T) * ldc));
     ALGP_TRY(ensure(c, c->prevrows, sizeof(T) * MAX_APPEND * ldc));
-    {
-        ALGP_TRY(ensure(c, c->ckind, sizeof(int) * Mpad));
-        ALGP_HIP(hipMemcpyAsync(c->ckind.p, pl.kind.data(), sizeof(int) * Mpad, hipMemcpyHostToDevice, c->stream));
-        if (!pl.became_unit.empty() && keep > 0) {
-            const size_t nb = pl.became_unit.size();
-            ALGP_TRY(ensure(c, c->auxIdx, sizeof(int64_t) * nb));
-            ALGP_HIP(hipMemcpyAsync(c->auxIdx.p, pl.became_unit.data(), sizeof(int64_t) * nb, hipMemcpyHostToDevice, c->stream));
-            ALGP_TRY(zero_listed_rows_launch<T>(c, p(c->Vt), ldc, (const int64_t*)c->auxIdx.p, (int64_t)nb, keep));
-        }
-        ALGP_TRY(sync(c));
-    }
-    KmatSrc s = make_src(c);
+    ALGP_TRY(ensure(c, c->ckind, sizeof(int) * Mpad));
     if (pl.rhs_fused) {
         const int DP = c->hyp.DP;
         ALGP_TRY(ensure(c, c->rhs_rx, sizeof(T) * (size_t)Mpad * DP));
         ALGP_TRY(ensure(c, c->rhs_cx, sizeof(T) * (size_t)Npad * DP));
         ALGP_TRY(ensure(c, c->rhs_rk, sizeof(int) * (size_t)Mpad));
+    }
+    return ALGP_OK;
+}
+
+template <typename T>
+int Impl<T>::upload_kinds(algp_ctx* c, const typename Impl<T>::SolvePlan& pl) {
+    ALGP_HIP(hipMemcpyAsync(c->ckind.p, pl.kind.data(), sizeof(int) * c->Mpad, hipMemcpyHostToDevice, c->stream));
+    return ALGP_OK;
+}
+
+template <typename T>
+int Impl<T>::solve_prepare(algp_ctx* c, int incremental, typename Impl<T>::SolvePlan& pl) {
+    const int64_t keep = pl.keep;
+    c->solved = false;
+    c->vr.drop();
+    ALGP_TRY(solve_reserve(c, incremental, pl));
+    ALGP_TRY(upload_kinds(c, pl));
+    if (!pl.became_unit.empty() && keep > 0) {
+        const size_t nb = pl.became_unit.size();
+        ALGP_TRY(ensure(c, c->auxIdx, sizeof(int64_t) * nb));
+        ALGP_HIP(hipMemcpyAsync(c->auxIdx.p, pl.became_unit.data(), sizeof(int64_t) * nb, hipMemcpyHostToDevice, c->stream));
+        ALGP_TRY(zero_listed_rows_launch<T>(c, p(c->Vt), c->ldv, (const int64_t*)c->auxIdx.p, (int64_t)nb, keep));
+    }
+    ALGP_TRY(sync(c));
+    return solve_rhs(c, pl);
+}
+
+template <typename T>
+int Impl<T>::solve_rhs(algp_ctx* c, typename Impl<T>::SolvePlan& pl) {
+    const int64_t N = c->N, Npad = c->Npad, M = c->M, Mpad = c->Mpad, keep = pl.keep, ldc = c->ldv;
+    const int64_t ldv = Npad + MAX_APPEND;
+    KmatSrc s = make_src(c);
+    if (pl.rhs_fused) {
+        const int DP = c->hyp.DP;
         ALGP_TRY(rhs_gather_launch<T>(c, (const T*)c->Xs.p, DP, (const int64_t*)c->Cidx.p, M, Mpad,
                                       c->prior_noise ? (const int*)c->ckind.p : nullptr, (const int64_t*)c->Aidx.p, N, Npad,
                                       p(c->rhs_rx), p(c->rhs_cx), (int*)c->rhs_rk.p));
@@ -182,7 +203,13 @@
 
 
 template <typename T>
-int Impl<T>::solve_run(algp_ctx* c, typename Impl<T>::SolvePlan& pl) {
+T* Impl<T>::rowstat_buffer(algp_ctx* c, const typename Impl<T>::SolvePlan& pl) {
+    if (pl.row_stats && ensure(c, c->rowstat, sizeof(T) * 2 * (size_t)(c->Npad / NB) * (size_t)c->Mpad) == ALGP_OK) return p(c->rowstat);
+    return nullptr;
+}
+
+template <typename T>
+int Impl<T>::solve_run(algp_ctx* c, typename Impl<T>::SolvePlan& pl, TrsmSetup* setup) {
     const int64_t Npad = c->Npad, Mpad = c->Mpad, ldc = c->ldv, keep = pl.keep;
     prof_span_begin(c, ALGP_PROF_TRSM, (double)(Npad - keep) * (double)(Npad + keep) * (double)Mpad,
                     sizeof(T) * (double)Mpad * (double)Npad);
@@ -202,11 +229,9 @@
         trc = solve_dag_panel<T>(c, p(c->L), Npad, c->Lld, p(c->invD), (int*)((double*)c->scal.p + SC_STALL), p(c->Vt), ldc, Mpad, 1,
                                  (int)(pl.short_rows / NB));
     } else if (pl.route == SolveRoute::Sweep) {
-        T* stat = nullptr;
-        if (pl.row_stats && ensure(c, c->rowstat, sizeof(T) * 2 * (size_t)(Npad / NB) * (size_t)Mpad) == ALGP_OK)
-            stat = p(c->rowstat);
+        T* stat = rowstat_buffer(c, pl);
         trc = trsm_blocked<T>(c, ALGP_PROF_GEMM_TRSM, p(c->Vt), Mpad, ldc, p(c->L), pl.sweep_end, c->Lld, p(c->invD),
-                              keep, p(c->z), stat, Mpad, &pl.rowstat_done, pl.rhs_fused ? &pl.gen : nullptr);
+                              keep, p(c->z), stat, Mpad, &pl.rowstat_done, pl.rhs_fused ? &pl.gen : nullptr, setup);
     } else {
         trc = fail(c, ALGP_ERR_STATE, "internal: the folded route is solved by the factorisation's launch (fit_and_solve)");
     }
@@ -230,7 +255,7 @@
 
 
 template <typename T>
-int Impl<T>::solve_finish(algp_ctx* c, int incremental, const unsigned char* alive_host, const typename Impl<T>::SolvePlan& pl) {
+int Impl<T>::solve_finish_enqueue(algp_ctx* c, const unsigned char* alive_host, const typename Impl<T>::SolvePlan& pl) {
     const int64_t N = c->N, Npad = c->Npad, M = c->M, Mpad = c->Mpad, ldc = c->ldv, keep = pl.keep;
     T* ss = p(c->tvec);
     T* dot = ss + Mpad;
@@ -270,22 +295,38 @@
                                      c->cextra.p ? (const T*)c->cextra.p : nullptr, ss, dot, (T)c->ybar, p(c->dstat),
                                      p(c->mu), (unsigned char*)c->alive.p));
     if (alive_host) ALGP_HIP(hipMemcpyAsync(c->alive.p, alive_host, M, hipMemcpyHostToDevice, c->stream));
+    return ALGP_OK;
+}
+
+template <typename T>
+int Impl<T>::solve_finish(algp_ctx* c, int incremental, const unsigned char* alive_host, const typename Impl<T>::SolvePlan& pl) {
+    ALGP_TRY(solve_finish_enqueue(c, alive_host, pl));
     ALGP_TRY(sync_checked(c, "solve_candidates"));
-    c->ncols = Npad;
+    note_solve_state(c);
+    ALGP_TRY(reset_lazy(c));
+    c->solved = true;
+    note_solve(c, pl);
+    return ALGP_OK;
+}
+
+template <typename T>
+void Impl<T>::note_solve_state(algp_ctx* c) {
+    c->ncols = c->Npad;
     c->picks.clear();
     c->mi.valid = false;
     c->vr.drop();
-    ALGP_TRY(reset_lazy(c));
-    c->solved = true;
+}
+
+template <typename T>
+void Impl<T>::note_solve(algp_ctx* c, const typename Impl<T>::SolvePlan& pl) {
     c->vt_fact_idx = c->fact_idx;
     c->vt_fact_var = c->fact_var;
     c->vt_cand_idx = c->cand_idx;
-    c->vt_kind.assign(pl.kind.begin(), pl.kind.begin() + M);
+    c->vt_kind.assign(pl.kind.begin(), pl.kind.begin() + c->M);
     c->vt_hyp_stamp = c->hyp_stamp;
     c->vt_prior_noise = c->prior_noise;
     c->vt_has_extra = c->cextra.p != nullptr;
-    c->kept_cols_last = keep;
-    return ALGP_OK;
+    c->kept_cols_last = pl.keep;
 }
 
 
@@ -301,9 +342,84 @@
 
 
 template <typename T>
+int Impl<T>::fit_and_solve_sweep(algp_ctx* c, typename Impl<T>::SolvePlan& pl) {
+    const int64_t N = c->N, Npad = c->Npad, Mpad = c->Mpad;
+    c->factored = false;
+    c->solved = false;
+    c->alpha_valid = false;
+    c->vr.drop();
+    ALGP_TRY(reserve_factor(c, Npad, 0));
+    ALGP_TRY(ensure(c, c->z, sizeof(T) * Npad));
+    ALGP_TRY(ensure(c, c->alpha, sizeof(T) * Npad));
+    ALGP_TRY(trsv_reserve(c, Npad));
+    ALGP_TRY(solve_reserve(c, 0, pl));
+    ALGP_TRY(lazy_reserve(c));
+    rowstat_buffer(c, pl);
+    TrsmSetup pre;
+    trsm_reserve<T>(c, Mpad, pl.sweep_end, 0, pre);
+    constexpr size_t NSC = SC_STALL + 1;
+    ALGP_TRY(readback_reserve(c, sizeof(double) * NSC + sizeof(T) * Npad));
+    double* host = (double*)c->readback;
+    T* zh = (T*)(host + NSC);
+    ALGP_TRY(upload_kinds(c, pl));
+
+    hipEvent_t factored_ev = sync_event_api(c, 22), ready_ev = sync_event_api(c, 23);
+    ALGP_TRY(factor_scratch_enqueue(c, factored_ev));
+    ALGP_HIP(hipStreamWaitEvent(c->stream2, factored_ev, 0));
+    c->cur = c->stream2;
+    int rc = solve_rhs(c, pl);
+    if (rc == ALGP_OK)
+        rc = trsm_prelude<T>(c, ALGP_PROF_GEMM_TRSM, p(c->Vt), Mpad, c->ldv, p(c->L), pl.sweep_end, c->Lld, p(c->invD),
+                             pl.rhs_fused ? &pl.gen : nullptr, pre);
+    c->cur = c->stream;
+    hipEventRecord(ready_ev, c->stream2);
+    hipStreamWaitEvent(c->stream, ready_ev, 0);
+    if (rc == ALGP_OK) rc = solve_run(c, pl, &pre);
+    if (rc == ALGP_OK) rc = solve_finish_enqueue(c, nullptr, pl);
+    if (rc == ALGP_OK) rc = reset_lazy(c);
+    auto disown = [c](int code) {
+        c->vt_fact_idx.clear();
+        c->vt_fact_var.clear();
+        return code;
+    };
+    if (rc != ALGP_OK) {
+        hipStreamSynchronize(c->stream);
+        return disown(rc);
+    }
+    note_factor(c, 0);
+    note_solve(c, pl);
+    static_assert(SC_LOGDET == 0 && SC_INFO == 1 && SC_STALL > SC_INFO, "one copy covers log det, info and the stall word");
+    hipError_t e = hipMemcpyAsync(host, c->scal.p, sizeof(double) * NSC, hipMemcpyDeviceToHost, c->stream);
+    if (e == hipSuccess) e = hipMemcpyAsync(zh, c->z.p, sizeof(T) * Npad, hipMemcpyDeviceToHost, c->stream);
+    if (e == hipSuccess) e = hipStreamSynchronize(c->stream);
+    if (e != hipSuccess) {
+        hipStreamSynchronize(c->stream);
+        return disown(fail(c, ALGP_ERR_HIP, hipGetErrorString(e)));
+    }
+    c->n_syncs++;
+    int stall = 0;
+    memcpy(&stall, host + SC_STALL, sizeof(int));
+    const int src = stall_verdict(c, stall, "factorize: forward substitution");
+    double ld_total = 0;
+    const int frc = factor_verdict(c, host + SC_LOGDET, N, 0, &ld_total);
+    if (frc != ALGP_OK) return disown(frc);
+    if (src != ALGP_OK) return disown(src);
+    c->logdet = ld_total;
+    c->uw_rows = 0;
+    c->uw_stable = 0;
+    c->yalpha = sum_squares(zh, N);
+    c->factored = true;
+    c->train_dirty = false;
+    note_solve_state(c);
+    c->solved = true;
+    return ALGP_OK;
+}
+
+template <typename T>
 int Impl<T>::fit_and_solve(algp_ctx* c) {
     SolvePlan pl;
     plan_route(c, 0, true, pl);
+    if (pl.route == SolveRoute::Sweep && pl.keep == 0 && c->stream2 && c->cur == c->stream) return fit_and_solve_sweep(c, pl);
     if (pl.route != SolveRoute::Folded) {
         ALGP_TRY(factorize(c, 0));
         ALGP_TRY(solve_prepare(c, 0, pl));
diff --git a/algp_amd/csrc/api_factor.hip b/algp_amd/csrc/api_factor.hip
--- a/algp_amd/csrc/api_factor.hip
+++ b/algp_amd/csrc/api_factor.hip
@@ -18,8 +18,8 @@
         return fail(c, ALGP_ERR_STATE, "internal: factor_resident was given a panel that does not fit the task list");
     if (ld == 0) ld = npad;
     double* sc = (double*)c->scal.p;
-    ALGP_HIP(hipMemsetAsync(sc + slot_logdet, 0, 2 * sizeof(double), c->stream));
     if (panel) {
+        ALGP_HIP(hipMemsetAsync(sc + slot_logdet, 0, 2 * sizeof(double), c->stream));
         ALGP_TRY(cholesky_dag_panel<T>(c, A, npad, ld, invD, sc + slot_logdet, (int*)(sc + slot_info), panel->P, panel->ldp,
                                        panel->mpad, panel->mode, (int)(panel->short_rows / NB)));
         if (panel->mode == 2 && panel->inv_out && c->stream2 && c->cur == c->stream) {
@@ -34,11 +34,23 @@
             panel->inv_enqueued = true;
         }
     } else {
-        ALGP_TRY(cholesky_blocked<T>(c, A, npad, ld, invD, sc + slot_logdet, (int*)(sc + slot_info)));
+        ALGP_TRY(factor_enqueue(c, A, npad, invD, slot_logdet, slot_info, ld));
     }
     double host[2];
     ALGP_HIP(hipMemcpyAsync(host, sc + slot_logdet, 2 * sizeof(double), hipMemcpyDeviceToHost, c->stream));
     ALGP_TRY(sync(c));
+    return factor_verdict(c, host, n, pivot_offset, logdet);
+}
+
+template <typename T>
+int Impl<T>::factor_enqueue(algp_ctx* c, T* A, int64_t npad, T* invD, int slot_logdet, int slot_info, int64_t ld) {
+    double* sc = (double*)c->scal.p;
+    ALGP_HIP(hipMemsetAsync(sc + slot_logdet, 0, 2 * sizeof(double), c->stream));
+    return cholesky_blocked<T>(c, A, npad, ld, invD, sc + slot_logdet, (int*)(sc + slot_info));
+}
+
+template <typename T>
+int Impl<T>::factor_verdict(algp_ctx* c, const double* host, int64_t n, int64_t pivot_offset, double* logdet) {
     int info;
     memcpy(&info, &host[1], sizeof(int));
     if (info == INT_MIN)
@@ -238,6 +250,46 @@
 
 
 template <typename T>
+int Impl<T>::build_S(algp_ctx* c) {
+    return kmat_launch<T>(c, make_src(c), (const int64_t*)c->Aidx.p, c->N, c->Npad, (const int64_t*)c->Aidx.p, c->N, c->Npad,
+                          (const T*)c->varA.p, c->pool_is_cov ? 0 : 1, nullptr, 1, p(c->L), c->Lld);
+}
+
+template <typename T>
+int Impl<T>::factor_scratch_enqueue(algp_ctx* c, hipEvent_t factored_ev) {
+    const int64_t N = c->N, Npad = c->Npad;
+    prof_span_begin(c, ALGP_PROF_CHOLESKY, (double)N * N * N / 3.0, sizeof(T) * (double)N * N);
+    int rc = build_S(c);
+    if (rc == ALGP_OK) rc = factor_enqueue(c, p(c->L), Npad, p(c->invD), SC_LOGDET, SC_INFO, c->Lld);
+    prof_span_end(c);
+    ALGP_TRY(rc);
+    ALGP_HIP(hipEventRecord(factored_ev, c->stream));
+    return z_enqueue(c);
+}
+
+template <typename T>
+int Impl<T>::z_enqueue(algp_ctx* c) {
+    ALGP_HIP(hipMemcpyAsync(c->z.p, c->y0.p, sizeof(T) * c->Npad, hipMemcpyDeviceToDevice, c->stream));
+    return trsv_forward<T>(c, p(c->L), c->Npad, c->Lld, p(c->invD), p(c->z));
+}
+
+template <typename T>
+void Impl<T>::note_factor(algp_ctx* c, int64_t keep) {
+    c->Nfact = c->N;
+    c->fact_idx = c->train_idx;
+    c->fact_var = c->train_var_host;
+    c->fact_hyp_stamp = c->hyp_stamp;
+    c->kept_rows_last = keep;
+}
+
+template <typename T>
+double Impl<T>::sum_squares(const T* zh, int64_t n) {
+    double q = 0;
+    for (int64_t i = 0; i < n; ++i) q += (double)zh[i] * (double)zh[i];
+    return q;
+}
+
+template <typename T>
 int Impl<T>::factorize(algp_ctx* c, int incremental, typename Impl<T>::Panel* panel) {
     if (panel && incremental) return fail(c, ALGP_ERR_STATE, "internal: a panel rides along with a from-scratch factorisation only");
     const int64_t N = c->N, Npad = c->Npad;
@@ -267,8 +319,7 @@
                     sizeof(T) * (double)N * N);
     int frc = ALGP_OK;
     if (keep == 0) {
-        frc = kmat_launch<T>(c, s, (const int64_t*)c->Aidx.p, N, Npad, (const int64_t*)c->Aidx.p, N, Npad,
-                             (const T*)c->varA.p, c->pool_is_cov ? 0 : 1, nullptr, 1, p(c->L), ld);
+        frc = build_S(c);
         if (frc == ALGP_OK)
             frc = factor_resident(c, p(c->L), N, Npad, p(c->invD), SC_LOGDET, SC_INFO, &ld_total, ld, 0, panel);
     } else {
@@ -367,8 +418,7 @@
         c->uw_rows = 0;
         c->uw_stable = 0;
     } else {
-        ALGP_HIP(hipMemcpyAsync(c->z.p, c->y0.p, sizeof(T) * Npad, hipMemcpyDeviceToDevice, c->stream));
-        ALGP_TRY(trsv_forward<T>(c, p(c->L), Npad, ld, p(c->invD), p(c->z)));
+        ALGP_TRY(z_enqueue(c));
         c->uw_rows = 0;
         c->uw_stable = 0;
     }
@@ -376,16 +426,10 @@
     std::vector<T> zh(Npad);
     ALGP_HIP(hipMemcpyAsync(zh.data(), c->z.p, sizeof(T) * Npad, hipMemcpyDeviceToHost, c->stream));
     ALGP_TRY(sync_checked(c, "factorize: forward substitution"));
-    double q = 0;
-    for (int64_t i = 0; i < N; ++i) q += (double)zh[i] * (double)zh[i];
-    c->yalpha = q;
+    c->yalpha = sum_squares(zh.data(), N);
     c->factored = true;
     c->train_dirty = false;
-    c->Nfact = N;
-    c->fact_idx = c->train_idx;
-    c->fact_var = c->train_var_host;
-    c->fact_hyp_stamp = c->hyp_stamp;
-    c->kept_rows_last = keep;
+    note_factor(c, keep);
     return ALGP_OK;
 }
 
diff --git a/algp_amd/csrc/api_greedy.hip b/algp_amd/csrc/api_greedy.hip
--- a/algp_amd/csrc/api_greedy.hip
+++ b/algp_amd/csrc/api_greedy.hip
@@ -179,9 +179,13 @@
 }
 
 template <typename T>
+int Impl<T>::lazy_reserve(algp_ctx* c) {
+    ALGP_TRY(ensure(c, c->fresh, sizeof(int) * std::max<int64_t>(c->Mpad, 1)));
+    return ensure(c, c->lazypicks, sizeof(LazyPick) * MAX_APPEND);
+}
+template <typename T>
 int Impl<T>::reset_lazy(algp_ctx* c) {
-    ALGP_TRY(ensure(c, c->fresh, sizeof(int) * std::max<int64_t>(c->Mpad, 1)));
-    ALGP_TRY(ensure(c, c->lazypicks, sizeof(LazyPick) * MAX_APPEND));
+    ALGP_TRY(lazy_reserve(c));
     ALGP_HIP(hipMemsetAsync(c->fresh.p, 0, sizeof(int) * std::max<int64_t>(c->Mpad, 1), c->stream));
     c->lazy_stale = false;
     c->bounds_valid = false;
diff --git a/algp_amd/csrc/api_impl.h b/algp_amd/csrc/api_impl.h
--- a/algp_amd/csrc/api_impl.h
+++ b/algp_amd/csrc/api_impl.h
@@ -17,7 +17,9 @@
 hipEvent_t sync_event_api(algp_ctx* c, size_t i);
 KmatSrc make_src(algp_ctx* c);
 int sync(algp_ctx* c);
+int readback_reserve(algp_ctx* c, size_t bytes);
 int sync_checked(algp_ctx* c, const char* what);
+int stall_verdict(algp_ctx* c, int stall, const char* what);
 inline bool vr_over_ranks(const algp_ctx* c) { return c->vr.xrows != 0 && c->comm_nranks > 1; }
 
 enum class SolveRoute { Segments, TaskList, Sweep, Folded };
@@ -45,6 +47,13 @@
     static bool panel_fits(int64_t npad, int64_t mpad);
     static int factor_resident(algp_ctx* c, T* A, int64_t n, int64_t npad, T* invD, int slot_logdet, int slot_info,
                                double* logdet, int64_t ld = 0, int64_t pivot_offset = 0, Panel* panel = nullptr);
+    static int factor_enqueue(algp_ctx* c, T* A, int64_t npad, T* invD, int slot_logdet, int slot_info, int64_t ld);
+    static int factor_verdict(algp_ctx* c, const double* host, int64_t n, int64_t pivot_offset, double* logdet);
+    static int build_S(algp_ctx* c);
+    static int z_enqueue(algp_ctx* c);
+    static int factor_scratch_enqueue(algp_ctx* c, hipEvent_t factored_ev);
+    static void note_factor(algp_ctx* c, int64_t keep);
+    static double sum_squares(const T* zh, int64_t n);
     static int reserve_factor(algp_ctx* c, int64_t npad_need, int64_t keep_rows, int64_t keep_height = 0,
                               bool headroom = false);
     static bool vt_rows_for_new_sites(algp_ctx* c, int64_t Nb, int64_t p0, std::vector<int64_t>& src_row,
@@ -77,11 +86,19 @@
     static int rhs_window(algp_ctx* c, int64_t c0, int64_t w, void* out, int64_t ldo);
     static constexpr int64_t SWEEP_PUSH_TILES = 320;
     static void plan_route(algp_ctx* c, int incremental, bool allow_fold, SolvePlan& pl);
+    static int solve_reserve(algp_ctx* c, int incremental, const SolvePlan& pl);
+    static int upload_kinds(algp_ctx* c, const SolvePlan& pl);
+    static int solve_rhs(algp_ctx* c, SolvePlan& pl);
     static int solve_prepare(algp_ctx* c, int incremental, SolvePlan& pl);
-    static int solve_run(algp_ctx* c, SolvePlan& pl);
+    static T* rowstat_buffer(algp_ctx* c, const SolvePlan& pl);
+    static int solve_run(algp_ctx* c, SolvePlan& pl, TrsmSetup* setup = nullptr);
     static int solve_narrow_tile(algp_ctx* c, const SolvePlan& pl);
+    static int solve_finish_enqueue(algp_ctx* c, const unsigned char* alive_host, const SolvePlan& pl);
+    static void note_solve_state(algp_ctx* c);
+    static void note_solve(algp_ctx* c, const SolvePlan& pl);
     static int solve_finish(algp_ctx* c, int incremental, const unsigned char* alive_host, const SolvePlan& pl);
     static int solve_candidates(algp_ctx* c, int incremental, const unsigned char* alive_host);
+    static int fit_and_solve_sweep(algp_ctx* c, SolvePlan& pl);
     static int fit_and_solve(algp_ctx* c);
     static int get_posterior(algp_ctx* c, void* mu, void* var);
     static int get_posterior_cov(algp_ctx* c, void* cov_out, double* mi_out);
@@ -142,6 +159,7 @@
     static int commit_enqueue(algp_ctx* c, int64_t pool_idx, double ss, double delta, const char* winner_payload = nullptr);
     static int commit_pick(algp_ctx* c, int64_t pool_idx, double static_std, double mobile_std);
     static int lazy_launch(algp_ctx* c, int mode, int64_t pos, double ss, double delta, const int64_t* pos_dev = nullptr);
+    static int lazy_reserve(algp_ctx* c);
     static int reset_lazy(algp_ctx* c);
     static int flush_lazy(algp_ctx* c);
     static int enqueue_local_best(algp_ctx* c, double ss, double delta);
diff --git a/algp_amd/csrc/common.h b/algp_amd/csrc/common.h
--- a/algp_amd/csrc/common.h
+++ b/algp_amd/csrc/common.h
@@ -351,6 +351,8 @@
     int debug_fail_next_rowx = 0;
     int pending_pick_error = 0;
     std::string pending_pick_msg;
+    void* readback = nullptr;
+    size_t readback_cap = 0;
     int64_t n_syncs = 0;
     int debug_dag_stall_ticket = -1;
     int debug_trsv_stall_block = -1;
@@ -444,6 +446,13 @@
     int DP = 0, kernel = 0;
     double outputscale = 0;
     int (*window)(algp_ctx* c, int64_t c0, int64_t w, void* out, int64_t ldo) = nullptr;
+};
+struct TrsmSetup {
+    bool reserved = false;
+    bool inv512 = false;
+    bool sched = false;
+    bool built = false;
+    bool materialised = false;
 };
 template <typename T>
 int rhs_gather_launch(algp_ctx* c, const T* Xs, int DP, const int64_t* ridx, int64_t rows, int64_t rows_pad, const int* unit,
@@ -549,7 +558,12 @@
 template <typename T>
 int trsm_blocked(algp_ctx* c, int klass, T* X, int64_t mpad, int64_t ldx, const T* L, int64_t npad,
                  int64_t ldl, const T* invD, int64_t col_start = 0, const T* stat_w = nullptr, T* stat_out = nullptr,
-                 int64_t stat_ld = 0, bool* stats_done = nullptr, const RhsGen* gen = nullptr);
+                 int64_t stat_ld = 0, bool* stats_done = nullptr, const RhsGen* gen = nullptr, TrsmSetup* setup = nullptr);
+template <typename T>
+void trsm_reserve(algp_ctx* c, int64_t mpad, int64_t npad, int64_t col_start, TrsmSetup& setup);
+template <typename T>
+int trsm_prelude(algp_ctx* c, int klass, T* X, int64_t mpad, int64_t ldx, const T* L, int64_t npad, int64_t ldl, const T* invD,
+                 const RhsGen* gen, TrsmSetup& setup);
 bool trsm_sched_wanted(const algp_ctx* c, int64_t mpad, int64_t npad, int64_t col_start);
 template <typename T>
 int tail_cols_launch(algp_ctx* c, int klass, T* X, int64_t mpad, int64_t ldx, const T* L, int64_t ldl, int64_t lrows, const T* invD_blk,
@@ -561,6 +575,7 @@
 template <typename T>
 int syrk_upper(algp_ctx* c, int klass, const T* X, int64_t npad, int64_t ldx, T* C, int64_t ldc);
 
+int trsv_reserve(algp_ctx* c, int64_t npad);
 template <typename T>
 int trsv_forward(algp_ctx* c, const T* L, int64_t npad, int64_t ldl, const T* invD, T* b, int64_t kb_start = 0);
 template <typename T>
diff --git a/algp_amd/csrc/potrf.hip b/algp_amd/csrc/potrf.hip
--- a/algp_amd/csrc/potrf.hip
+++ b/algp_amd/csrc/potrf.hip
@@ -362,35 +362,52 @@
 }
 
 template <typename T>
+void trsm_reserve(algp_ctx* c, int64_t mpad, int64_t npad, int64_t col_start, TrsmSetup& s) {
+    s.inv512 = trsm_inv512_wanted(c, mpad, npad, col_start) &&
+               ensure(c, c->inv512, sizeof(T) * (size_t)(npad / WB) * WB * WB) == ALGP_OK &&
+               ensure(c, c->inv512_scr, sizeof(T) * inv512_scratch_elems<T>(npad)) == ALGP_OK &&
+               ensure(c, c->trsm_tmp, sizeof(T) * (size_t)mpad * WB) == ALGP_OK;
+    s.sched = s.inv512 && trsm_sched_wanted(c, mpad, npad, col_start) &&
+              ensure(c, c->gemm_part, sizeof(T) * 128 * 128 * 2 * (size_t)c->cu_count) == ALGP_OK;
+    s.reserved = true;
+}
+ALGP_INSTANTIATE(trsm_reserve);
+
+template <typename T>
+int trsm_prelude(algp_ctx* c, int klass, T* X, int64_t mpad, int64_t ldx, const T* L, int64_t npad, int64_t ldl, const T* invD,
+                 const RhsGen* gen, TrsmSetup& s) {
+    s.built = true;
+    if (s.inv512) ALGP_TRY(build_inv512<T>(c, klass, L, ldl, invD, npad, (T*)c->inv512.p, (T*)c->inv512_scr.p));
+    if (gen && !s.sched) {
+        ALGP_TRY(gen->window(c, 0, npad, X, ldx));
+        s.materialised = true;
+        gen = nullptr;
+    }
+    if (s.inv512) {
+        T* tmp512 = (T*)c->trsm_tmp.p;
+        if (gen) ALGP_TRY(gen->window(c, 0, WB, tmp512, WB));
+        else ALGP_HIP(hipMemcpy2DAsync(tmp512, sizeof(T) * WB, X, sizeof(T) * ldx, sizeof(T) * WB, (size_t)mpad, hipMemcpyDeviceToDevice, c->cur));
+    }
+    return ALGP_OK;
+}
+ALGP_INSTANTIATE(trsm_prelude);
+
+template <typename T>
 int trsm_blocked(algp_ctx* c, int klass, T* X, int64_t mpad, int64_t ldx, const T* L, int64_t npad,
                  int64_t ldl, const T* invD, int64_t col_start, const T* stat_w, T* stat_out, int64_t stat_ld, bool* stats_done,
-                 const RhsGen* gen) {
+                 const RhsGen* gen, TrsmSetup* setup) {
     const int64_t tiles = mpad / NB;
     const bool stats = stat_out && stat_w && col_start == 0 && tiles > TRSM_PUSH_TILES;
     if (stats_done) *stats_done = stats;
     if (!stats) stat_out = nullptr;
-    const T* inv512 = nullptr;
-    T* tmp512 = nullptr;
-    {
-        if (trsm_inv512_wanted(c, mpad, npad, col_start) &&
-            ensure(c, c->inv512, sizeof(T) * (size_t)(npad / WB) * WB * WB) == ALGP_OK &&
-            ensure(c, c->inv512_scr, sizeof(T) * inv512_scratch_elems<T>(npad)) == ALGP_OK &&
-            ensure(c, c->trsm_tmp, sizeof(T) * (size_t)mpad * WB) == ALGP_OK) {
-            ALGP_TRY(build_inv512<T>(c, klass, L, ldl, invD, npad, (T*)c->inv512.p, (T*)c->inv512_scr.p));
-            inv512 = (const T*)c->inv512.p;
-            tmp512 = (T*)c->trsm_tmp.p;
-        }
-    }
-    const bool sched = inv512 && trsm_sched_wanted(c, mpad, npad, col_start) &&
-                       ensure(c, c->gemm_part, sizeof(T) * 128 * 128 * 2 * (size_t)c->cu_count) == ALGP_OK;
-    if (gen && !sched) {
-        ALGP_TRY(gen->window(c, 0, npad, X, ldx));
-        gen = nullptr;
-    }
-    if (inv512) {
-        if (gen) ALGP_TRY(gen->window(c, 0, WB, tmp512, WB));
-        else ALGP_HIP(hipMemcpy2DAsync(tmp512, sizeof(T) * WB, X, sizeof(T) * ldx, sizeof(T) * WB, (size_t)mpad, hipMemcpyDeviceToDevice, c->cur));
-    }
+    TrsmSetup own;
+    TrsmSetup& s = setup ? *setup : own;
+    if (!s.reserved) trsm_reserve<T>(c, mpad, npad, col_start, s);
+    if (!s.built) ALGP_TRY(trsm_prelude<T>(c, klass, X, mpad, ldx, L, npad, ldl, invD, gen, s));
+    if (s.materialised) gen = nullptr;
+    const T* inv512 = s.inv512 ? (const T*)c->inv512.p : nullptr;
+    T* tmp512 = s.inv512 ? (T*)c->trsm_tmp.p : nullptr;
+    const bool sched = s.sched;
     if (sched) {
         c->gemm_sched = true;
         const int rc = trsm_rows<T>(c, klass, X, mpad, ldx, L, npad, ldl, invD, col_start, true, stat_w, stat_out, stat_ld, inv512, tmp512, gen);
@@ -734,8 +751,10 @@
 #undef Lcol_at
 }
 
+static size_t trsv_ctrl_bytes(int nblk) { return sizeof(int) * (size_t)(nblk + 8); }
+int trsv_reserve(algp_ctx* c, int64_t npad) { return ensure(c, c->trsv_ctrl, trsv_ctrl_bytes((int)(npad / NB))); }
 static int trsv_prepare(algp_ctx* c, int nblk, unsigned long long* spin_limit, int* skip_block) {
-    const size_t bytes = sizeof(int) * (size_t)(nblk + 8);
+    const size_t bytes = trsv_ctrl_bytes(nblk);
     ALGP_TRY(ensure(c, c->trsv_ctrl, bytes));
     ALGP_HIP(hipMemsetAsync(c->trsv_ctrl.p, 0, bytes, c->cur));
     *spin_limit = 200000000ull;
```

Result: no change. 653,600, median of 5 (+0.1%).
